# arneschneuing/DiffSBDD

Measured on AMD Instinct MI355X. Metric: sampled ligands/sec (500-step DDPM, fullatom_cond) at 1/2/4/8 MI355X, higher is better.
Workload: dtype f32

## Files before the change

diffsbdd_amd/_lib.py:

```python
from __future__ import annotations

import ctypes as C
import os

_HERE = os.path.dirname(os.path.abspath(__file__))
LIB_PATH = os.environ.get("DSBDD_LIB") or os.path.join(_HERE, "libdiffsbdd_hip.so")
ABI_VERSION = 6

OK, ERR_ARG, ERR_STATE, ERR_CAPACITY, ERR_LAUNCH = 0, -1, -2, -3, -4
STATUS_NAN, STATUS_EDGE_OVERFLOW = 1, 2

G_NAMES = ["ATOM_ENC_W0T", "ATOM_ENC_B0", "ATOM_ENC_W1T", "ATOM_ENC_B1",
           "RES_ENC_W0T", "RES_ENC_B0", "RES_ENC_W1T", "RES_ENC_B1",
           "ATOM_DEC_W0T", "ATOM_DEC_B0", "ATOM_DEC_W1T", "ATOM_DEC_B1",
           "RES_DEC_W0T", "RES_DEC_B0", "RES_DEC_W1T", "RES_DEC_B1",
           "EMB_WT", "EMB_B", "EMBOUT_WT", "EMBOUT_B"]
GCL_NAMES = ["E1_WT", "E1_WD", "E1_WD0", "E1_TAB", "E2_WT", "E2_B", "ATT_W", "ATT_B",
             "N1_WT", "N1_B", "N2_WT", "N2_B"]
EQ_NAMES = ["C1_WT", "C_WD", "C_WD0", "C_TAB", "C_W2T", "C_B2",
            "X_WD", "X_WD0", "X_TAB", "X_W2T", "X_B2", "W3"]
OPT_PRUNE, OPT_CONE, OPT_GRANULE16, OPT_EMU, OPT_SPLITK = 0, 1, 2, 3, 4
(BUF_EDGE_ROW, BUF_EDGE_COL, BUF_EDGE_D0, BUF_ROW_PTR, BUF_H, BUF_X, BUF_NODE_BATCH, BUF_DEG,
 BUF_LEVEL, BUF_LEVEL_LIST, BUF_LEVEL_COUNT, BUF_LEVEL_END, BUF_LROW_PTR, BUF_LEDGE_ROW, BUF_LEDGE_COL,
 BUF_LEDGE_D0, BUF_LEVEL_STATS) = range(17)


class Config(C.Structure):
    _fields_ = [(n, C.c_int32) for n in (
        "atom_nf", "residue_nf", "joint_nf", "hidden_nf", "n_layers", "inv_sublayers",
        "attention", "use_tanh", "update_pocket_coords", "reflection_equivariant",
        "edge_embedding_dim", "has_cutoff_ligand", "has_cutoff_pocket",
        "has_cutoff_interaction")] + [(n, C.c_float) for n in (
            "cutoff_ligand", "cutoff_pocket", "cutoff_interaction",
            "norm_constant", "normalization_factor", "coords_range")]


class TrainGraph(C.Structure):
    _fields_ = [(n, C.c_void_p) for n in ("erow", "ecol", "ed0", "row_ptr", "deg", "rev", "node_batch", "lig_off",
                                          "poc_off")] + [(n, C.c_int64) for n in ("n_lig", "n_nodes", "n_edges", "batch")]


class LossCfg(C.Structure):
    _fields_ = [(n, C.c_int32) for n in ("batch", "n_lig", "n_pocket", "atom_nf", "residue_nf", "timesteps", "remove_com",
                                         "vnode_idx")] + \
               [(n, C.c_float) for n in ("norm_value_x", "norm_value_h", "norm_bias_h")] + \
               [(n, C.c_int32) for n in ("n1_tab", "n2_tab")]


class TrainMlp(C.Structure):
    _fields_ = [("P", C.c_void_p), ("Q", C.c_void_p), ("ldpq", C.c_int32)] + \
               [(n, C.c_void_p) for n in ("wd", "wd0", "tab", "W2", "W2T", "b2", "head", "head_b")]


class TrainMlpGrad(C.Structure):
    _fields_ = [("dP", C.c_void_p), ("dQ", C.c_void_p), ("ldo", C.c_int32), ("d_vec", C.c_void_p), ("d_W2", C.c_void_p),
                ("gd0", C.c_void_p)]


class OptimCfg(C.Structure):
    _fields_ = [(n, C.c_double) for n in ("lr", "beta1", "beta2", "eps", "weight_decay")] + [("clip_grad", C.c_int32)]


_P = C.c_void_p
_I64 = C.c_int64
_I32 = C.c_int32
_F = C.c_float

SIGNATURES = {
    "dsbdd_abi_version": (C.c_int, []),
    "dsbdd_last_error": (C.c_char_p, []),
    "dsbdd_engine_create": (C.c_int, [C.POINTER(Config), C.POINTER(_P)]),
    "dsbdd_engine_destroy": (None, [_P]),
    "dsbdd_engine_weight_slots": (C.c_int, [_P]),
    "dsbdd_engine_set_weights": (C.c_int, [_P, C.POINTER(_P), C.c_int]),
    "dsbdd_engine_workspace_bytes": (C.c_size_t, [_P, _I64, _I64, _I64, _I64]),
    "dsbdd_engine_bind_workspace": (C.c_int, [_P, _P, C.c_size_t, _I64, _I64, _I64, _I64]),
    "dsbdd_engine_set_trace": (C.c_int, [_P, _P, _P]),
    "dsbdd_engine_set_pocket_frame": (C.c_int, [_P, _P, _P, _P, _P, _P, _I64, _I64, _I64, _I64, _I64, _I64]),
    "dsbdd_engine_clear_pocket_frame": (C.c_int, [_P]),
    "dsbdd_dynamics_forward": (C.c_int, [_P, _P, _P, _P, _P, _I64, _P, _P, _I64, _I64, _I64,
                                         _P, _P, _I64, _P, _P, _P]),
    "dsbdd_engine_buffer": (C.c_int, [_P, C.c_int, C.POINTER(_P)]),
    "dsbdd_engine_graph_stats": (C.c_int, [_P, C.POINTER(_I64), C.POINTER(_I64), C.POINTER(_I64)]),
    "dsbdd_engine_last_plan": (C.c_int, [_P, C.POINTER(C.c_int32), C.POINTER(C.c_int32), C.c_int32,
                                         C.POINTER(C.c_int32), C.POINTER(C.c_int32)]),
    "dsbdd_engine_set_option": (C.c_int, [_P, C.c_int, C.c_int]),
    "dsbdd_engine_get_option": (C.c_int, [_P, C.c_int]),
    "dsbdd_engine_profile": (C.c_int, [_P, C.c_int, C.c_int]),
    "dsbdd_engine_profile_read": (C.c_int, [_P, C.POINTER(C.c_double), C.POINTER(_I64)]),
    "dsbdd_cond_reverse_update": (C.c_int, [_P, _P, _P, _P, _P, _P, _P, _I64, _I64, _I64,
                                            _I32, _I32, _F, _F, _F, _I32]),
    "dsbdd_joint_reverse_update": (C.c_int, [_P, _P, _P, _P, _P, _P, _P, _P, _P, _I64, _I64, _I64,
                                             _I32, _I32, _F, _F, _F, _I32]),
    "dsbdd_segment_mean3": (C.c_int, [_P, _P, _I32, _P, _I64, _I64, _P]),
    "dsbdd_cond_affine_noise": (C.c_int, [_P, _P, _P, _P, _P, _P, _I64, _I64, _I64, _I32, _I32, _F, _F, _I32]),
    "dsbdd_joint_affine_noise": (C.c_int, [_P, _P, _P, _P, _P, _P, _P, _I64, _I64, _I64, _I32, _I32, _F, _F,
                                           _I32, _I32]),
    "dsbdd_cond_repaint_update": (C.c_int, [_P, _P, _P, _P, _P, _P, _P, _P, _P, _P, _P, _I64, _I64, _I64,
                                            _I32, _I32, _F, _F, _F, _F, _I32, _I32]),
    "dsbdd_joint_repaint_update": (C.c_int, [_P] * 15 + [_I64, _I64, _I64, _I32, _I32, _F, _F, _F, _F, _I32]),
    "dsbdd_cond_step_keyed": (C.c_int, [_P] * 10 + [_I64, _I64, _I64, _I32, _I32, _F, _F, _F, _I32, _F, _F, _F, _I32,
                                        C.c_uint64, C.c_uint64, _I64, _P, _P, _F]),
    "dsbdd_randn_keyed": (C.c_int, [_P, _P, _P, _I64, _I32, _I64, _I64, _P, C.c_uint64, C.c_uint64,
                                    C.c_uint32]),
    "dsbdd_node_linear": (C.c_int, [_P, _P, _I32, _I32, _P, _I32, _I32, _P, _I32, _P, _P, _I32,
                                    _P, _I32, _I64, _I32, _I32]),
    "dsbdd_build_edges": (C.c_int, [_P, _P, _P, _P, _I64, _I64, _I64, C.POINTER(Config),
                                    _P, _P, _P, _P, _P, _P, _P, _P, _I64, _P]),
    "dsbdd_bond_orders": (C.c_int, [_P, _P, _P, _P, _I64, _I32, _P, _P, _P, C.c_float, C.c_float,
                                    C.c_float, _I32, _P]),
    "dsbdd_pack_ligands": (C.c_int, [_P, _P, _P, _P, _I32, _I64, _P, _P, _P, _I64, _I64, _I32, _P, _P, _P, _P, _P]),
    "dsbdd_train_scratch_bytes": (C.c_size_t, [_I32, _I64, _I64]),
    "dsbdd_train_wgrad_scratch_bytes": (C.c_size_t, [_I64, _I64, _I64]),
    "dsbdd_train_wgrad_plan_bytes": (C.c_size_t, [_I64, _I64, _I64]),
    "dsbdd_train_edge_rev": (C.c_int, [_P, _P, _P]),
    "dsbdd_train_sample_mean": (C.c_int, [_P, _P, _P, _P]),
    "dsbdd_train_gcl_forward": (C.c_int, [_P, _I32, _P, _P, _P, _F, _P, _P, C.c_size_t]),
    "dsbdd_train_gcl_backward": (C.c_int, [_P, _I32, _P, _P, _P, _F, _P, _P, _P, _P, C.c_size_t]),
    "dsbdd_train_coord_forward": (C.c_int, [_P, _I32, _P, _P, _I32, _P, _P, _I64, _F, _F, _I32, _F, _P, _P,
                                            C.c_size_t]),
    "dsbdd_train_coord_backward": (C.c_int, [_P, _I32, _P, _P, _I32, _P, _P, _I64, _I64, _F, _F, _I32, _F, _P, _P, _P,
                                             _P, _P, C.c_size_t]),
    "dsbdd_train_radial_backward": (C.c_int, [_P, _P, _P, _P, _P]),
    "dsbdd_train_wgrad": (C.c_int, [_P, _P, _I32, _P, _I32, _I64, _I32, _I32, _P, _P, C.c_size_t]),
    "dsbdd_train_colsum": (C.c_int, [_P, _P, _I32, _I64, _I32, _P, _P, C.c_size_t]),
    "dsbdd_train_net_create": (C.c_int, [C.POINTER(Config), C.POINTER(_P)]),
    "dsbdd_train_net_destroy": (None, [_P]),
    "dsbdd_train_net_param_count": (C.c_int, [_P]),
    "dsbdd_train_net_pack_bytes": (C.c_size_t, [_P]),
    "dsbdd_train_net_workspace_bytes": (C.c_size_t, [_P, C.POINTER(TrainGraph)]),
    "dsbdd_train_net_forward": (C.c_int, [_P, _P, C.POINTER(TrainGraph), C.POINTER(_P), _P, C.c_size_t, _P, C.c_size_t, _P, _P,
                                          _P, _I64, _I32, _P, _P, _P]),
    "dsbdd_train_net_backward": (C.c_int, [_P, _P, C.POINTER(TrainGraph), C.POINTER(_P), C.POINTER(_P), _P, C.c_size_t, _P,
                                           C.c_size_t, _I64, _P, _P, _P, _P]),
    "dsbdd_train_net_forward_held": (C.c_int, [_P, _P, C.POINTER(TrainGraph), C.POINTER(_P), _P, C.c_size_t, _P, C.c_size_t,
                                               _P, _P, _P, _I64, _I32, _P, _P, _P, _I32]),
    "dsbdd_train_net_backward_acc": (C.c_int, [_P, _P, C.POINTER(TrainGraph), C.POINTER(_P), C.POINTER(_P), _P, _P, C.c_size_t,
                                               _P, C.c_size_t, _I64, _P, _P, _P, _P]),
    "dsbdd_edge_capacity": (C.c_int, [_P, _P, _I64, _P, _I64, _I64, _P]),
    "dsbdd_loss_rows": (C.c_int, []),
    "dsbdd_loss_out_rows": (C.c_int, []),
    "dsbdd_loss_cond_pre": (C.c_int, [_P, C.POINTER(LossCfg)] + [_P] * 17),
    "dsbdd_loss_cond_post": (C.c_int, [_P, C.POINTER(LossCfg)] + [_P] * 8),
    "dsbdd_loss_cond_post_backward": (C.c_int, [_P, C.POINTER(LossCfg)] + [_P] * 9),
    "dsbdd_loss_joint_out_rows": (C.c_int, []),
    "dsbdd_loss_joint_pre": (C.c_int, [_P, C.POINTER(LossCfg)] + [_P] * 20),
    "dsbdd_loss_joint_post": (C.c_int, [_P, C.POINTER(LossCfg)] + [_P] * 10),
    "dsbdd_loss_joint_post_backward": (C.c_int, [_P, C.POINTER(LossCfg)] + [_P] * 14),
    "dsbdd_optim_create": (C.c_int, [C.POINTER(OptimCfg), _I32, C.POINTER(_I64), C.POINTER(_P)]),
    "dsbdd_optim_destroy": (None, [_P]),
    "dsbdd_optim_state_elems": (_I64, [_P]),
    "dsbdd_optim_state_offset": (_I64, [_P, _I32]),
    "dsbdd_optim_workspace_bytes": (C.c_size_t, [_P]),
    "dsbdd_optim_bind": (C.c_int, [_P, _P, _P, _P, _P, _P, C.c_size_t]),
    "dsbdd_optim_set_params": (C.c_int, [_P, _P, C.POINTER(_P)]),
    "dsbdd_optim_step": (C.c_int, [_P, _P, C.POINTER(_P), C.POINTER(_I32), C.c_double]),
    "dsbdd_optim_state_read": (C.c_int, [_P, _P, C.POINTER(C.c_double), _I32]),
    "dsbdd_optim_state_write": (C.c_int, [_P, _P, C.POINTER(C.c_double), _I32, C.c_double, C.c_double]),
    "dsbdd_lj_potential": (C.c_int, [_P, _P, _I32, _I32, _P, _I64, _I64, _P, C.c_double, _I32, _P, _P, _P]),
}

_lib = None


class HipLibraryError(RuntimeError):
    pass


def load():
    global _lib
    if _lib is not None:
        return _lib
    import torch
    if not os.path.isfile(LIB_PATH):
        raise HipLibraryError(
            f"{LIB_PATH} not found: the HIP extension is not built. Run "
            "`python -c 'import __graft_entry__ as g; g.build()'` (needs hipcc). "
            "There is no CPU fallback for the product path.")
    try:
        lib = C.CDLL(LIB_PATH)
    except OSError as exc:
        raise HipLibraryError(f"cannot load {LIB_PATH}: {exc}") from exc
    for name, (res, args) in SIGNATURES.items():
        try:
            fn = getattr(lib, name)
        except AttributeError as exc:
            raise HipLibraryError(f"{LIB_PATH} does not export {name}") from exc
        fn.restype = res
        fn.argtypes = args
    ver = lib.dsbdd_abi_version()
    if ver != ABI_VERSION:
        raise HipLibraryError(f"ABI version mismatch: library {ver}, binding {ABI_VERSION}")
    _lib = lib
    return lib


def check(rc, what=""):
    if rc == OK:
        return
    msg = load().dsbdd_last_error()
    msg = msg.decode() if msg else ""
    raise HipLibraryError(f"{what} failed with code {rc}: {msg}")
```

diffsbdd_amd/csrc/edge_mlp.h:

```cpp
#pragma once
#include "common.h"

namespace dsbdd {

struct EdgeMlpW {
  const float* P;
  const float* Q;
  const float* wd;
  const float* wd0;
  const float* table;
  const float* W2T;
  const float* b2;
  const float* W2TP;
  const float* W2TP16;
  const void* W2E;
  const float* W2SK;
};

struct EdgeArgs {
  const int* erow; const int* ecol; const float* ed0;
  const int* e_count;
  int e_cap;
  const float* x;
  int n_lig;
  int n_nodes;
  int ldpq;
  EdgeMlpW mlp[2];
  const float* att_w; const float* att_b; int attention;
  float* agg;
  float* agg_head;
  const float* w3; const int* node_batch; const float* mean;
  float norm_constant; float coords_range; int use_tanh; int n_mlp;
  float* xagg;
  float* xagg_head;
  size_t xagg_stride;
  size_t xhead_stride;
  float norm_factor;
  int wt_base;
  int* tile_ctr;
  unsigned long long* ts;
  int pass_split;
  const int* erow_b; const int* ecol_b; const float* ed0_b; const int* e_count_b; int e_cap_b; int wt_base_b;
  float* agg_b; float* agg_head_b;
  float* z2_out;
  size_t z2_stride;
};

enum { MODE_GCL = 0, MODE_COORD = 1 };

__global__ __launch_bounds__(kThreads) void agg_complete_kernel(float* agg, const float* agg_head,
                                                                const int* row_ptr, const int* deg,
                                                                int n_rows, int H, int max_tile, int shift) {
  const int row = (blockIdx.x * kThreads + threadIdx.x) >> 6, lane = threadIdx.x & 63;
  if (row >= n_rows) return;
  const int d = deg[row], s = row_ptr[row];
  const int t0 = s >> shift, t1 = min((s + d - 1) >> shift, max_tile);
  if (d > 0 && t1 == t0) return;
  for (int k = 4 * lane; k < H; k += 256) {
    float4 v = make_float4(0.f, 0.f, 0.f, 0.f);
    if (d > 0) {
      v = ld4(agg + (size_t)row * H + k);
      for (int T = t0 + 1; T <= t1; ++T) {
        const float4 h = ld4(agg_head + (size_t)T * H + k);
        v.x += h.x; v.y += h.y; v.z += h.z; v.w += h.w;
      }
    }
    *reinterpret_cast<float4*>(agg + (size_t)row * H + k) = v;
  }
}


__global__ __launch_bounds__(kThreads) void agg_complete2_kernel(
    float* agg, const float* head_a, const int* row_ptr_a, const int* deg_a, const float* agg_b,
    const float* head_b, const int* row_ptr_b, const int* deg_b, const int* twin_local, int twin_base,
    int n_lig, int n_rows, int H, int n_ghost, int max_tile) {
  const int row = (blockIdx.x * kThreads + threadIdx.x) >> 6, lane = threadIdx.x & 63;
  if (row >= n_rows + n_ghost) return;
  const bool ghost = row >= n_rows;
  const int da = ghost ? 0 : deg_a[row], sa = ghost ? 0 : row_ptr_a[row];
  const int a0 = sa >> 5, a1 = min((sa + da - 1) >> 5, max_tile);
  int db = 0, sb = 0, tw = 0;
  if (row >= n_lig) {
    const int tl = ghost ? row - n_rows : twin_local[row - n_lig];
    db = deg_b[tl]; sb = row_ptr_b[tl]; tw = twin_base + tl;
  }
  const int b0 = sb >> 5, b1 = min((sb + db - 1) >> 5, max_tile);
  for (int k = 4 * lane; k < H; k += 256) {
    float4 v = make_float4(0.f, 0.f, 0.f, 0.f);
    if (da > 0) {
      v = ld4(agg + (size_t)row * H + k);
      for (int T = a0 + 1; T <= a1; ++T) {
        const float4 h = ld4(head_a + (size_t)T * H + k);
        v.x += h.x; v.y += h.y; v.z += h.z; v.w += h.w;
      }
    }
    if (db > 0) {
      float4 u = ld4(agg_b + (size_t)tw * H + k);
      for (int T = b0 + 1; T <= b1; ++T) {
        const float4 h = ld4(head_b + (size_t)T * H + k);
        u.x += h.x; u.y += h.y; u.z += h.z; u.w += h.w;
      }
      v.x += u.x; v.y += u.y; v.z += u.z; v.w += u.w;
    }
    *reinterpret_cast<float4*>(agg + (size_t)row * H + k) = v;
  }
}

}
```

diffsbdd_amd/csrc/edge_wave.h:

```cpp
#pragma once
#include "common.h"
#include "edge_mlp.h"
#include "graph.h"

namespace dsbdd {

template <int H, int MODE, int EMU = 0>
struct WaveLayout {
  static constexpr int BK = EMU ? 16 : 32;
  static constexpr int B_BUF = EMU ? 24 * H : BK * H;
  static constexpr int NV = (MODE == MODE_GCL) ? 1 : 2;
  static constexpr int VEC_PER = 7 * H;
  static constexpr int VEC_OFF = 0;
  static constexpr int SCR_OFF = VEC_OFF + NV * VEC_PER;
  static constexpr int SCR_PER = 32 * 3;
  static constexpr int B_OFF = (SCR_OFF + 4 * SCR_PER + 4 + 255) / 256 * 256;
  static constexpr int TOTAL = B_OFF + 2 * B_BUF;
};

__device__ __forceinline__ void wave_lds_fence() {
  __builtin_amdgcn_fence(__ATOMIC_RELEASE, "wavefront");
  __builtin_amdgcn_s_waitcnt(0xc07f);
  __builtin_amdgcn_wave_barrier();
  __builtin_amdgcn_fence(__ATOMIC_ACQUIRE, "wavefront");
}


__device__ __forceinline__ float dpp_xor1(float v) {
  return __int_as_float(__builtin_amdgcn_update_dpp(0, __float_as_int(v), 0xB1, 0xF, 0xF, true));
}
__device__ __forceinline__ float dpp_xor2(float v) {
  return __int_as_float(__builtin_amdgcn_update_dpp(0, __float_as_int(v), 0x4E, 0xF, 0xF, true));
}
__device__ __forceinline__ float dpp_half_mirror(float v) {
  return __int_as_float(__builtin_amdgcn_update_dpp(0, __float_as_int(v), 0x141, 0xF, 0xF, true));
}
__device__ __forceinline__ float dpp_ror8(float v) {
  return __int_as_float(__builtin_amdgcn_update_dpp(0, __float_as_int(v), 0x128, 0xF, 0xF, true));
}
__device__ __forceinline__ float pair_sum_rows16(float p, float q) {
  const auto r = __builtin_amdgcn_permlane16_swap(__float_as_uint(p), __float_as_uint(q), false, false);
  return __uint_as_float(r[0]) + __uint_as_float(r[1]);
}
__device__ __forceinline__ float pair_sum_halves(float p, float q) {
  const auto r = __builtin_amdgcn_permlane32_swap(__float_as_uint(p), __float_as_uint(q), false, false);
  return __uint_as_float(r[0]) + __uint_as_float(r[1]);
}

__device__ __forceinline__ float reduce16_half_wave(const float (&part)[16], int j) {
  float k8[8], k4[4], k2[2];
#pragma unroll
  for (int i = 0; i < 8; ++i) k8[i] = pair_sum_rows16(part[i], part[i + 8]);
  const bool b3 = (j >> 3) & 1, b2 = (j >> 2) & 1, b1 = (j >> 1) & 1;
#pragma unroll
  for (int i = 0; i < 4; ++i) {
    const float send = b3 ? k8[i] : k8[i + 4], keep = b3 ? k8[i + 4] : k8[i];
    k4[i] = keep + dpp_ror8(send);
  }
#pragma unroll
  for (int i = 0; i < 2; ++i) {
    const float send = b2 ? k4[i] : k4[i + 2], keep = b2 ? k4[i + 2] : k4[i];
    k2[i] = keep + dpp_half_mirror(send);
  }
  const float send = b1 ? k2[0] : k2[1], keep = b1 ? k2[1] : k2[0];
  const float k1 = keep + dpp_xor2(send);
  return k1 + dpp_xor1(k1);
}

typedef __bf16 bf16x8 __attribute__((ext_vector_type(8)));
typedef unsigned int u32x4 __attribute__((ext_vector_type(4)));

__device__ __forceinline__ float bf16_rne_f(float x) {
  unsigned u = __float_as_uint(x);
  u += 0x7FFFu + ((u >> 16) & 1u);
  return __uint_as_float(u & 0xFFFF0000u);
}

__global__ __launch_bounds__(256) void pack_w2e_kernel(const float* __restrict__ W2T, unsigned short* __restrict__ out, int H) {
  const int idx = blockIdx.x * 256 + threadIdx.x;
  if (idx >= H * H) return;
  const int CT = H / 32;
  const int i = idx & 7, l = (idx >> 3) & 63, c = (idx >> 9) % CT, ks = (idx >> 9) / CT;
  const int k = 16 * ks + 8 * (l >> 5) + i, col = 32 * c + (l & 31);
  const float w = W2T[(size_t)k * H + col];
  const float hi = bf16_rne_f(w), r1 = w - hi, mid = bf16_rne_f(r1), lo = bf16_rne_f(r1 - mid);
  const size_t base = (((size_t)(ks * CT + c) * 3) * 64 + l) * 8 + i;
  out[base] = (unsigned short)(__float_as_uint(hi) >> 16);
  out[base + 512] = (unsigned short)(__float_as_uint(mid) >> 16);
  out[base + 1024] = (unsigned short)(__float_as_uint(lo) >> 16);
}

template <int H, int MODE, bool BPERM, int EMU = 0, bool STORE = false>
__global__ __launch_bounds__(kThreads, 2) void edge_wave_kernel(EdgeArgs p) {
  using L = WaveLayout<H, MODE, EMU>;
  static_assert(!STORE || (!BPERM && EMU == 0), "z2 is stored by the plain exact kernels only");
  constexpr int BK = L::BK;
  constexpr int CT = H / 32;
  constexpr int NK = H / BK;
  constexpr int NQ = H / 4;
  constexpr int UNIT = EMU ? (((6 * H) % kThreads == 0) ? 4 : 2) : 4;
  constexpr int BI = EMU ? (24 * H) / (kThreads * UNIT) : BK * NQ / kThreads;
  constexpr int NG = EMU ? CT / 2 : BK / 8;
  constexpr int BMW = 32, BMB = 128;
  static_assert(H % 64 == 0 && H <= 256, "hidden_nf must be 64,128,192 or 256");
  static_assert(EMU || (BK * NQ) % kThreads == 0, "B slice split");
  static_assert(!EMU || (24 * H) % (kThreads * UNIT) == 0, "emulated B slice split");
  static_assert(EMU == 0 || EMU == 6 || EMU == 9, "partial products of the emulated path");
  static_assert(!EMU || !BPERM, "the emulated path has its own B layout");
  constexpr bool SETPRIO = true;
  static_assert(!BPERM || CT == 8 || CT == 4, "lane-grouped B reads need 4 or 8 column tiles");
  constexpr bool bperm = BPERM;

  __shared__ __attribute__((aligned(1024))) float smem[L::TOTAL];
  float* sB = smem + L::B_OFF;
  float* sV = smem + L::VEC_OFF;
  const int t = threadIdx.x, lane = t & 63;
  const int w = __builtin_amdgcn_readfirstlane(t >> 6);
  const int half = lane >> 5, j = lane & 31;
  float* s_phi = smem + L::SCR_OFF + w * L::SCR_PER;
  float* s_tr = s_phi;
  const bool split = MODE == MODE_COORD && p.pass_split && p.n_mlp == 2;
  const int qsel = split ? ((blockIdx.x >> 3) & 1) : 0;
  const int n_pass = (MODE == MODE_GCL || split) ? 1 : p.n_mlp;

  for (int q = 0; q < n_pass; ++q) {
    const EdgeMlpW& mw = p.mlp[qsel + q];
    float* v = sV + q * L::VEC_PER;
    for (int i = t; i < H; i += kThreads) {
      v[i] = mw.wd[i];
      v[H + i] = mw.wd0[i];
      v[2 * H + i] = mw.table[i];
      v[3 * H + i] = mw.table[H + i];
      v[4 * H + i] = mw.table[2 * H + i];
      v[5 * H + i] = mw.b2[i];
      v[6 * H + i] = (MODE == MODE_GCL) ? (p.attention ? p.att_w[i] : 0.f) : p.w3[i];
    }
  }
  const float att_b = (MODE == MODE_GCL && p.attention) ? p.att_b[0] : 0.f;
  const float inv_norm = 1.0f / p.norm_factor;

  const int swb = (bperm && CT == 8) ? ((j >> 3) & 1) : 0;
  auto feat = [&](int c) { return ((c ^ (4 * swb)) * 32) + j; };

  const int E = min(*p.e_count, p.e_cap);
  const int nt_a = (E + BMB - 1) / BMB;
  const int E_b = (MODE == MODE_GCL && p.e_count_b) ? min(*p.e_count_b, p.e_cap_b) : 0;
  const int ntiles = nt_a + (E_b + BMB - 1) / BMB;
  const int xcd = blockIdx.x & 7;
  const int kx = split ? (blockIdx.x >> 4) : (blockIdx.x >> 3);
  const int gx = split ? (gridDim.x >> 4) : (gridDim.x >> 3);
  const int tq = ntiles / 8, tr = ntiles % 8;
  const int csize = tq + (xcd < tr ? 1 : 0);
  const int cbase = (xcd < tr) ? xcd * (tq + 1) : tr * (tq + 1) + (xcd - tr) * tq;
  if (kx >= csize) return;


  constexpr int SG = EMU ? BI : (BI + 3) / 4;
  typedef float stg_t __attribute__((ext_vector_type(UNIT)));
  stg_t stg[SG];
  auto stage_lo = [](int g) { return BI * g / NG; };
  auto stage_load = [&](int q, int ks, int g) {
    const char* src = EMU ? reinterpret_cast<const char*>(p.mlp[qsel + q].W2E) + (size_t)ks * (96 * H)
                          : reinterpret_cast<const char*>((bperm ? p.mlp[qsel + q].W2TP : p.mlp[qsel + q].W2T) + (size_t)ks * BK * H);
    const unsigned toff = (unsigned)t * (4u * UNIT);
#pragma unroll
    for (int i = stage_lo(g); i < stage_lo(g + 1); ++i)
      stg[EMU ? i : i - stage_lo(g)] = *reinterpret_cast<const stg_t*>(src + (size_t)(kThreads * 4 * UNIT * i) + toff);
  };
  auto stage_store = [&](int buf, int g) {
    float* dst = sB + buf * L::B_BUF + t * UNIT;
#pragma unroll
    for (int i = stage_lo(g); i < stage_lo(g + 1); ++i)
      *reinterpret_cast<stg_t*>(dst + kThreads * UNIT * i) = stg[EMU ? i : i - stage_lo(g)];
  };

  int my_r = -1, my_c = 0, my_ty = 0;
  float my_d = 0.f, my_d0 = 0.f, xr[3] = {0.f, 0.f, 0.f}, xc[3] = {0.f, 0.f, 0.f};
  int nx_r = -1, nx_c = 0;
  int my_prev = -1, nx_prev = -1;
  int my_wt = 0, nx_wt = 0;
  bool my_lb = false, nx_lb = false;
  float nx_d0 = 0.f, nxr[3] = {0.f, 0.f, 0.f}, nxc[3] = {0.f, 0.f, 0.f};
  int vzero;
  asm volatile("v_mov_b32 %0, 0" : "=v"(vzero));
  auto fetch_idx = [&](int tile) {
    const bool lb = MODE == MODE_GCL && tile >= nt_a;
    const int tl = lb ? tile - nt_a : tile, El = lb ? E_b : E;
    const int* er = lb ? p.erow_b : p.erow;
    const int* ec = lb ? p.ecol_b : p.ecol;
    const float* ed = lb ? p.ed0_b : p.ed0;
    const int e0 = tl * BMB + w * BMW, e = e0 + j;
    nx_r = -1; nx_c = 0; nx_d0 = 0.f; nx_prev = -1; nx_wt = (lb ? p.wt_base_b : p.wt_base) + tl * 4 + w; nx_lb = lb;
    if (e < El) { nx_r = er[e]; nx_c = ec[e]; nx_d0 = ed[e]; }
    if (e0 > 0 && e0 < El) nx_prev = er[e0 - 1 + vzero];
  };
  auto fetch_x = [&]() {
    if ((unsigned)nx_r >= (unsigned)p.n_nodes || (unsigned)nx_c >= (unsigned)p.n_nodes) { nx_r = -1; nx_c = 0; }
    if (nx_r >= 0) {
#pragma unroll
      for (int k = 0; k < 3; ++k) { nxr[k] = p.x[3 * nx_r + k]; nxc[k] = p.x[3 * nx_c + k]; }
    }
  };
  auto commit_edge = [&]() {
    my_r = nx_r; my_c = nx_c; my_d0 = nx_d0; my_d = 0.f; my_ty = 0;
    my_prev = nx_prev; my_wt = nx_wt; my_lb = nx_lb;
#pragma unroll
    for (int k = 0; k < 3; ++k) { xr[k] = nxr[k]; xc[k] = nxc[k]; }
    if (my_r >= 0) {
      const float dx = xr[0] - xc[0], dy = xr[1] - xc[1], dz = xr[2] - xc[2];
      my_d = dx * dx + dy * dy + dz * dz;
      const bool rl = my_r < p.n_lig, cl = my_c < p.n_lig;
      my_ty = (rl && cl) ? 1 : ((!rl && !cl) ? 2 : 0);
    }
  };

  auto read_b = [&](const float* brow, float (&bv)[CT]) {
    if constexpr (BPERM) {
      const float4 lo = *reinterpret_cast<const float4*>(brow);
      bv[0] = lo.x; bv[1] = lo.y; bv[2] = lo.z; bv[3] = lo.w;
      if constexpr (CT == 8) {
        const float4 hi = *reinterpret_cast<const float4*>(brow + 4 - 8 * swb);
        bv[4] = hi.x; bv[5] = hi.y; bv[6] = hi.z; bv[7] = hi.w;
      }
    } else {
#pragma unroll
      for (int c = 0; c < CT; ++c) bv[c] = brow[c * 32];
    }
  };

#pragma unroll
  for (int g = 0; g < NG; ++g) { stage_load(0, 0, g); stage_store(0, g); }
  fetch_idx(cbase + kx);
  fetch_x();
  commit_edge();
  __syncthreads();
  int bslice = 0;

  constexpr int KH = EMU ? 8 : 4;
  const float* Pp = p.mlp[qsel].P + (size_t)(my_r < 0 ? 0 : my_r) * p.ldpq + KH * half;
  const float* Qp = p.mlp[qsel].Q + (size_t)my_c * p.ldpq + KH * half;
  f32x4 pc = ldv4(Pp), qc = ldv4(Qp), pn = pc, qn4 = qc;
  f32x4 pc1 = pc, qc1 = qc;
  if constexpr (EMU != 0) { pc1 = ldv4(Pp + 4); qc1 = ldv4(Qp + 4); }
  float phi0 = 0.f, phi1 = 0.f;

  bf16x8 a_h = {}, a_m = {}, a_l = {};
  (void)a_h; (void)a_m; (void)a_l;
  int li = kx, q = 0, next_li = 0;
  bool has_next = false;
#pragma unroll 1
  for (;;) {
    const float* vq = sV + q * L::VEC_PER;
    const bool tile_ends = q == n_pass - 1;
    const int qn = tile_ends ? 0 : q + 1;

    f32x16 acc[CT];
#pragma unroll
    for (int c = 0; c < CT; ++c) {
      const float bv = vq[5 * H + feat(c)];
#pragma unroll
      for (int r = 0; r < 16; ++r) acc[c][r] = bv;
    }

#pragma unroll 1
    for (int kt = 0; kt < NK; ++kt) {
      const bool more = kt + 1 < NK;
      const int st = q * NK + kt;
      if (st == 0) {
        next_li = li + gx;
        has_next = next_li < csize;
        if (has_next) fetch_idx(cbase + next_li);
      }
      if (st == 1 && has_next) fetch_x();
      const int sq = more ? q : qn, sks = more ? kt + 1 : 0;
      const f32x2 dd = splat2(my_d), dz = splat2(my_d0);
      if constexpr (EMU != 0) {
        constexpr int NG1 = (NG + 1) / 2;
        auto act8 = [&](int ks, bf16x8& o_h, bf16x8& o_m, bf16x8& o_l) {
          const float* vk = vq + ks * 16 + 8 * half;
          const float* vt = vk + (2 + my_ty) * H;
          float av[8];
#pragma unroll
          for (int hh = 0; hh < 2; ++hh) {
            const f32x4 pp = hh ? pc1 : pc, qq = hh ? qc1 : qc;
            const f32x4 wd4 = *reinterpret_cast<const f32x4*>(vk + 4 * hh);
            const f32x4 wz4 = *reinterpret_cast<const f32x4*>(vk + H + 4 * hh);
            const f32x4 tb4 = *reinterpret_cast<const f32x4*>(vt + 4 * hh);
            f32x2 alo = pk_fma(dz, wz4.xy, pk_fma(dd, wd4.xy, pp.xy + qq.xy)) + tb4.xy;
            f32x2 ahi = pk_fma(dz, wz4.zw, pk_fma(dd, wd4.zw, pp.zw + qq.zw)) + tb4.zw;
            alo = silu2(alo);
            ahi = silu2(ahi);
            av[4 * hh] = alo.x; av[4 * hh + 1] = alo.y; av[4 * hh + 2] = ahi.x; av[4 * hh + 3] = ahi.y;
          }
#pragma unroll
          for (int i = 0; i < 8; ++i) {
            const __bf16 h1 = (__bf16)av[i];
            const float r1 = av[i] - (float)h1;
            const __bf16 m1 = (__bf16)r1;
            const float r2 = r1 - (float)m1;
            o_h[i] = h1; o_m[i] = m1; o_l[i] = (__bf16)r2;
          }
        };
        auto load_pq = [&](int ks) {
          pc = ldv4(Pp + 16 * ks); pc1 = ldv4(Pp + 16 * ks + 4);
          qc = ldv4(Qp + 16 * ks); qc1 = ldv4(Qp + 16 * ks + 4);
        };
        act8(kt, a_h, a_m, a_l);
        load_pq(more ? kt + 1 : 0);
#pragma unroll
        for (int g = 0; g < NG1; ++g) stage_load(sq, sks, g);
        const float* bl = sB + (bslice & 1) * L::B_BUF + lane * 4;
        bf16x8 bh[2], bm[2], blo[2];
        auto rdb = [&](int cp, int plane, bf16x8 (&dst)[2]) {
#pragma unroll
          for (int u = 0; u < 2; ++u)
            dst[u] = __builtin_bit_cast(bf16x8, *reinterpret_cast<const u32x4*>(bl + (2 * cp + u) * 768 + plane * 256));
        };
        rdb(0, 2, blo); rdb(0, 1, bm); rdb(0, 0, bh);
#define EMU_MM(a, b) do { _Pragma("unroll") for (int u = 0; u < 2; ++u) \
          acc[2 * cp + u] = __builtin_amdgcn_mfma_f32_32x32x16_bf16(a, b[u], acc[2 * cp + u], 0, 0, 0); } while (0)
        __builtin_amdgcn_s_setprio(1);
#pragma unroll
        for (int cp = 0; cp < CT / 2; ++cp) {
          const bool nxt = cp + 1 < CT / 2;
          if constexpr (EMU == 9) { EMU_MM(a_l, blo); EMU_MM(a_m, blo); }
          EMU_MM(a_h, blo);
          if (nxt) rdb(cp + 1, 2, blo);
          if constexpr (EMU == 9) EMU_MM(a_l, bm);
          EMU_MM(a_m, bm); EMU_MM(a_h, bm);
          if (nxt) rdb(cp + 1, 1, bm);
          EMU_MM(a_l, bh); EMU_MM(a_m, bh); EMU_MM(a_h, bh);
          if (nxt) rdb(cp + 1, 0, bh);
          if (NG > 1 && cp == CT / 4 - 1) {
#pragma unroll
            for (int g = 0; g < NG1; ++g) stage_store((bslice + 1) & 1, g);
#pragma unroll
            for (int g = NG1; g < NG; ++g) stage_load(sq, sks, g);
          }
        }
#undef EMU_MM
        __builtin_amdgcn_s_setprio(0);
#pragma unroll
        for (int g = (NG > 1 ? NG1 : 0); g < NG; ++g) stage_store((bslice + 1) & 1, g);
      } else {
      const float* bcur = sB + (bslice & 1) * L::B_BUF + (4 * half) * H + (bperm ? j * CT + 4 * swb : j);
      const float* vk = vq + kt * BK + 4 * half;
      const float* vt = vk + (2 + my_ty) * H;
#pragma unroll
      for (int g = 0; g < BK / 8; ++g) {
        const int kb = kt * BK + 8 * g;
        if (g > 0) stage_store((bslice + 1) & 1, g - 1);
        stage_load(sq, sks, g);
        if (g + 1 < BK / 8 || more) {
          pn = ldv4(Pp + kb + 8);
          qn4 = ldv4(Qp + kb + 8);
        }
        const f32x4 wd4 = *reinterpret_cast<const f32x4*>(vk + 8 * g);
        const f32x4 wz4 = *reinterpret_cast<const f32x4*>(vk + H + 8 * g);
        const f32x4 tb4 = *reinterpret_cast<const f32x4*>(vt + 8 * g);
        f32x2 alo = pk_fma(dz, wz4.xy, pk_fma(dd, wd4.xy, pc.xy + qc.xy)) + tb4.xy;
        f32x2 ahi = pk_fma(dz, wz4.zw, pk_fma(dd, wd4.zw, pc.zw + qc.zw)) + tb4.zw;
        alo = silu2(alo);
        ahi = silu2(ahi);
        const float a[4] = {alo.x, alo.y, ahi.x, ahi.y};
        if (SETPRIO) __builtin_amdgcn_s_setprio(1);
#pragma unroll
        for (int i = 0; i < 4; ++i) {
          const float* brow = bcur + (8 * g + i) * H;
          float bv[CT];
          read_b(brow, bv);
#pragma unroll
          for (int c = 0; c < CT; ++c) acc[c] = mfma32(a[i], bv[c], acc[c]);
        }
        if (SETPRIO) __builtin_amdgcn_s_setprio(0);
        pc = pn; qc = qn4;
      }
      stage_store((bslice + 1) & 1, BK / 8 - 1);
      }
      ++bslice;
      __syncthreads();
    }

    const bool last_unit = tile_ends && !has_next;
    if (!last_unit) {
      const int r_n = tile_ends ? nx_r : my_r, c_n = tile_ends ? nx_c : my_c;
      Pp = p.mlp[qsel + qn].P + (size_t)(r_n < 0 ? 0 : r_n) * p.ldpq + KH * half;
      Qp = p.mlp[qsel + qn].Q + (size_t)c_n * p.ldpq + KH * half;
      pc = ldv4(Pp); qc = ldv4(Qp);
      if constexpr (EMU != 0) { pc1 = ldv4(Pp + 4); qc1 = ldv4(Qp + 4); }
    }

    if constexpr (STORE) {
      const int e0 = (my_wt - p.wt_base) * BMW;
      float* zb = p.z2_out + (MODE == MODE_COORD ? (size_t)(qsel + q) * p.z2_stride : (size_t)0) + (size_t)e0 * H + j;
#pragma unroll
      for (int r = 0; r < 16; ++r) {
        const int row = 8 * (r >> 2) + 4 * half + (r & 3);
        if (e0 + row < E) {
#pragma unroll
          for (int c = 0; c < CT; ++c) zb[(size_t)row * H + 32 * c] = acc[c][r];
        }
      }
    }
    if (MODE == MODE_GCL) {
#pragma unroll
      for (int c = 0; c < CT; ++c)
#pragma unroll
        for (int r = 0; r < 16; r += 2) {
          const f32x2 m2 = silu2(f32x2{acc[c][r], acc[c][r + 1]});
          acc[c][r] = m2.x; acc[c][r + 1] = m2.y;
        }
      if (p.attention) {
        f32x2 part2[8];
#pragma unroll
        for (int r = 0; r < 8; ++r) part2[r] = splat2(0.f);
#pragma unroll
        for (int c = 0; c < CT; ++c) {
          const f32x2 aw = splat2(vq[6 * H + feat(c)]);
#pragma unroll
          for (int r = 0; r < 8; ++r) part2[r] = pk_fma(f32x2{acc[c][2 * r], acc[c][2 * r + 1]}, aw, part2[r]);
        }
        float part[16];
#pragma unroll
        for (int r = 0; r < 8; ++r) { part[2 * r] = part2[r].x; part[2 * r + 1] = part2[r].y; }
        const float gate = sigmoidf_fast(reduce16_half_wave(part, j) + att_b);
        s_phi[16 * half + (j >> 1)] = gate;
        wave_lds_fence();
#pragma unroll
        for (int q4 = 0; q4 < 4; ++q4) {
          const float4 g4 = *reinterpret_cast<const float4*>(s_phi + 16 * half + 4 * q4);
          part[4 * q4] = g4.x; part[4 * q4 + 1] = g4.y; part[4 * q4 + 2] = g4.z; part[4 * q4 + 3] = g4.w;
        }
        wave_lds_fence();
#pragma unroll
        for (int c = 0; c < CT; ++c)
#pragma unroll
          for (int r = 0; r < 16; ++r) acc[c][r] *= part[r];
      }
      static_assert(CT % 2 == 0, "column tiles are exchanged in pairs");
      f32x2 sum2[CT];
#pragma unroll
      for (int c = 0; c < CT; ++c) sum2[c] = splat2(0.f);
      int cur = -1;
      const int row0 = __builtin_amdgcn_readlane(my_r, 0);
      bool to_head = row0 >= 0 && row0 == __builtin_amdgcn_readfirstlane(my_prev);
      auto flush = [&]() {
        if (cur >= 0) {
          float* dst = to_head ? (my_lb ? p.agg_head_b : p.agg_head) + (size_t)my_wt * H
                               : (my_lb ? p.agg_b : p.agg) + (size_t)cur * H;
#pragma unroll
          for (int c = 0; c < CT / 2; ++c) {
            const float tot = pair_sum_halves(sum2[c].x + sum2[c].y, sum2[c + CT / 2].x + sum2[c + CT / 2].y);
            dst[feat(c + half * (CT / 2))] = tot * inv_norm;
          }
          to_head = false;
        }
#pragma unroll
        for (int c = 0; c < CT; ++c) sum2[c] = splat2(0.f);
      };
#pragma unroll
      for (int gb = 0; gb < 8; ++gb) {
        const int hh = gb & 1;
#pragma unroll
        for (int ip = 0; ip < 4; ip += 2) {
          const int k = 4 * (gb >> 1) + ip;
          const int rn0 = __builtin_amdgcn_readlane(my_r, 4 * gb + ip);
          const int rn1 = __builtin_amdgcn_readlane(my_r, 4 * gb + ip + 1);
          if (rn0 != cur) {
            flush();
            cur = rn0;
          }
          if (half == hh) {
#pragma unroll
            for (int c = 0; c < CT; ++c) sum2[c].x += acc[c][k];
          }
          if (rn1 != rn0) {
            flush();
            cur = rn1;
          }
          if (half == hh) {
#pragma unroll
            for (int c = 0; c < CT; ++c) sum2[c].y += acc[c][k + 1];
          }
        }
      }
      flush();
    } else {
      f32x2 part2[8];
#pragma unroll
      for (int r = 0; r < 8; ++r) part2[r] = splat2(0.f);
#pragma unroll
      for (int c = 0; c < CT; ++c) {
        const f32x2 wv = splat2(vq[6 * H + feat(c)]);
#pragma unroll
        for (int r = 0; r < 8; ++r) part2[r] = pk_fma(silu2(f32x2{acc[c][2 * r], acc[c][2 * r + 1]}), wv, part2[r]);
      }
      float part[16];
#pragma unroll
      for (int r = 0; r < 8; ++r) { part[2 * r] = part2[r].x; part[2 * r + 1] = part2[r].y; }
      s_phi[mfma_row(j >> 1, lane)] = reduce16_half_wave(part, j);
      wave_lds_fence();
      const float ph = s_phi[j];
      wave_lds_fence();
      if (qsel + q == 0) phi0 = ph; else phi1 = ph;

      if (tile_ends) {
        float tx = 0.f, ty = 0.f, tz = 0.f;
        if (my_r >= 0) {
          const float dx = xr[0] - xc[0], dy = xr[1] - xc[1], dz = xr[2] - xc[2];
          const float den = sqrtf(my_d + 1e-8f) + p.norm_constant;
          const float ux = dx / den, uy = dy / den, uz = dz / den;
          if (split && qsel == 1) {
          } else if (p.use_tanh) {
            const float th = tanhf(phi0);
            tx = ux * th * p.coords_range; ty = uy * th * p.coords_range; tz = uz * th * p.coords_range;
          } else {
            tx = ux * phi0; ty = uy * phi0; tz = uz * phi0;
          }
          if (p.n_mlp == 2 && !(split && qsel == 0)) {
            const int b = p.node_batch[my_r];
            const float m0 = p.mean[3 * b], m1 = p.mean[3 * b + 1], m2 = p.mean[3 * b + 2];
            const float a0 = xr[0] - m0, a1 = xr[1] - m1, a2 = xr[2] - m2;
            const float b0 = xc[0] - m0, b1 = xc[1] - m1, b2 = xc[2] - m2;
            const float c0 = a1 * b2 - a2 * b1, c1 = a2 * b0 - a0 * b2, c2 = a0 * b1 - a1 * b0;
            const float cden = sqrtf(c0 * c0 + c1 * c1 + c2 * c2) + p.norm_constant;
            float phx = phi1;
            if (p.use_tanh) phx = tanhf(phx) * p.coords_range;
            tx += c0 / cden * phx; ty += c1 / cden * phx; tz += c2 / cden * phx;
          }
        }
        if (half == 0) { s_tr[3 * j] = tx; s_tr[3 * j + 1] = ty; s_tr[3 * j + 2] = tz; }
        wave_lds_fence();
        float trv[32];
#pragma unroll
        for (int e = 0; e < 32; ++e) trv[e] = s_tr[3 * e + (lane < 3 ? lane : 0)];
        if (lane < 3) {
          const int pop = split ? qsel : 0;
          float* xa = p.xagg + pop * p.xagg_stride;
          float* xh = p.xagg_head + pop * p.xhead_stride;
          const int row0 = __builtin_amdgcn_readlane(my_r, 0);
          bool to_head = row0 >= 0 && row0 == __builtin_amdgcn_readfirstlane(my_prev);
          int cur = -1;
          float sum = 0.f;
          auto put = [&]() {
            if (cur >= 0) {
              const float v = sum / p.norm_factor;
              if (to_head) xh[4 * (size_t)my_wt + lane] = v; else xa[(size_t)cur * 3 + lane] = v;
              to_head = false;
            }
          };
#pragma unroll
          for (int e = 0; e < 32; ++e) {
            const int rn = __builtin_amdgcn_readlane(my_r, e);
            if (rn != cur) {
              put();
              cur = rn;
              sum = 0.f;
            }
            sum += trv[e];
          }
          put();
        }
        wave_lds_fence();
      }
    }

    if (tile_ends) {
      if (last_unit) break;
      commit_edge();
      li = next_li;
      q = 0;
    } else {
      ++q;
    }
  }
}

}
```

diffsbdd_amd/csrc/engine.hip:

```cpp
#include "../../include/diffsbdd_hip.h"

#include <algorithm>
#include <climits>
#include <cmath>
#include <cstdio>
#include <cstdlib>
#include <cstring>
#include <string>
#include <type_traits>
#include <utility>
#include <vector>

#include "common.h"
#include "ddpm.h"
#include "edge_mlp.h"
#include "edge_wave.h"
#include "edge_wave16.h"
#include "edge_splitk.h"
#include "graph.h"
#include "lig_head.h"
#include "ligand_pack.h"
#include "molecule.h"
#include "node_chain.h"
#include "node_linear.h"
#include "train.h"
#include "train_kernels.h"

using namespace dsbdd;

#include "engine_state.h"
#include "launch.h"
#include "forward.h"
#include "graph_cache.h"
#include "capi_kernels.h"
#include "train_blocks.h"
#include "train_net.h"
#include "loss_head.h"
#include "optim.h"
#include "lj_loss.h"
#include "train_api.h"

extern "C" {

int dsbdd_abi_version(void) { return DSBDD_ABI_VERSION; }
const char* dsbdd_last_error(void) { return g_err.c_str(); }

int dsbdd_engine_create(const dsbdd_config* cfg, dsbdd_engine** out) {
  if (!cfg || !out) return fail(DSBDD_ERR_ARG, "null argument");
  if (!hidden_nf_ok(cfg->hidden_nf)) return fail(DSBDD_ERR_ARG, "hidden_nf must be one of 64, 128, 192, 256");
  if (cfg->n_layers < 1 || cfg->inv_sublayers < 1 || cfg->atom_nf < 1 || cfg->residue_nf < 1 ||
      cfg->joint_nf < 1 || cfg->edge_embedding_dim < 0)
    return fail(DSBDD_ERR_ARG, "bad layer/feature counts");
  if (!(cfg->normalization_factor > 0.f)) return fail(DSBDD_ERR_ARG, "normalization_factor must be > 0");
  dsbdd_engine* e = new dsbdd_engine();
  e->cfg = *cfg;
  e->slots.assign(n_slots(*cfg), nullptr);
  e->n_cu = device_cus();
  read_env_switches(e);
  *out = e;
  return DSBDD_OK;
}

void dsbdd_engine_destroy(dsbdd_engine* e) { delete e; }

int dsbdd_engine_weight_slots(const dsbdd_engine* e) { return e ? n_slots(e->cfg) : DSBDD_ERR_ARG; }

int dsbdd_engine_set_weights(dsbdd_engine* e, const float* const* slots_host, int n) {
  if (!e || !slots_host) return fail(DSBDD_ERR_ARG, "null argument");
  if (n != n_slots(e->cfg)) return fail(DSBDD_ERR_ARG, "wrong number of weight slots");
  const dsbdd_config& c = e->cfg;
  for (int i = 0; i < n; ++i) {
    const float* ptr = slots_host[i];
    bool optional = false;
    const int per = c.inv_sublayers * DSBDD_GCL_COUNT + DSBDD_EQ_COUNT;
    if (i >= DSBDD_G_COUNT) {
      const int r = (i - DSBDD_G_COUNT) % per;
      if (r < c.inv_sublayers * DSBDD_GCL_COUNT) {
        const int wch = r % DSBDD_GCL_COUNT;
        if (!c.attention && (wch == DSBDD_GCL_ATT_W || wch == DSBDD_GCL_ATT_B)) optional = true;
      } else {
        const int wch = r - c.inv_sublayers * DSBDD_GCL_COUNT;
        if (c.reflection_equivariant && wch >= DSBDD_EQ_X_WD && wch <= DSBDD_EQ_X_B2) optional = true;
      }
    }
    if (!ptr && !optional) return fail(DSBDD_ERR_ARG, "null weight slot " + std::to_string(i));
    if (ptr && (reinterpret_cast<uintptr_t>(ptr) & 15))
      return fail(DSBDD_ERR_ARG, "weight slot " + std::to_string(i) + " not 16-byte aligned");
    e->slots[i] = ptr;
  }
  e->drop_graphs();
  e->invalidate_derived();
  e->h0_pocket_valid = false;
  e->has_weights = true;
  return DSBDD_OK;
}

size_t dsbdd_engine_workspace_bytes(const dsbdd_engine* e, int64_t nl, int64_t np, int64_t B,
                                    int64_t E) {
  if (!e || nl < 0 || np < 0 || B < 1 || E < 0) return 0;
  return ws_carve(e->cfg, nl, np, B, E, nullptr).total;
}

int dsbdd_engine_bind_workspace(dsbdd_engine* e, void* ws, size_t bytes, int64_t nl, int64_t np,
                                int64_t B, int64_t E) {
  if (!e || !ws) return fail(DSBDD_ERR_ARG, "null argument");
  if (reinterpret_cast<uintptr_t>(ws) & 255) return fail(DSBDD_ERR_ARG, "workspace must be 256-byte aligned");
  if ((nl + np) >= (1ll << 30) || E >= (1ll << 31) - 256) return fail(DSBDD_ERR_ARG, "problem too large for int32 indices");
  if (bytes < ws_carve(e->cfg, nl, np, B, E, nullptr).total) return fail(DSBDD_ERR_CAPACITY, "workspace too small");
  e->drop_graphs();
  static_cast<Workspace&>(*e) = ws_carve(e->cfg, nl, np, B, E, static_cast<char*>(ws));
  e->ws = static_cast<char*>(ws); e->ws_bytes = bytes;
  e->cap_lig = nl; e->cap_poc = np; e->cap_batch = B; e->cap_edges = E;
  e->cap_edgesL = 2 * E + 32 * kLevels * B;
  e->cap_tiles = e->cap_edgesL / 32 + 2;
  e->cap_tiles16 = e->cap_edgesL / 16 + 2;
  e->lvl_stats_zeroed = false;
  e->frame = false;
  e->ghost_dirty = true;
  e->h0_pocket_valid = false;
  e->invalidate_derived();
  return DSBDD_OK;
}

#ifdef DSBDD_TIMESTAMPS
int dsbdd_debug_set_timestamps(dsbdd_engine* e, unsigned long long* buf, int capacity) {
  if (!e) return DSBDD_ERR_ARG;
  e->ts_buf = buf; e->ts_cap = capacity; e->ts_next = 0;
  return DSBDD_OK;
}
#endif

int dsbdd_engine_set_pocket_frame(dsbdd_engine* e, void* stream, const float* x_frame, const int64_t* mask_frame,
                                  const int32_t* frame_rows, const int32_t* twin_local, int64_t n_lig,
                                  int64_t n_pocket, int64_t batch, int64_t n_frame, int64_t batch_frame,
                                  int64_t edge_bound_frame) {
  StreamDevice stream_device_(stream);
  if (!e || !x_frame || !mask_frame || !frame_rows || !twin_local) return fail(DSBDD_ERR_ARG, "null argument");
  if (!e->ws) return fail(DSBDD_ERR_STATE, "workspace not bound");
  if (e->cfg.update_pocket_coords) return fail(DSBDD_ERR_STATE, "a pocket frame needs rigid pocket coordinates");
  if (n_lig < 0 || n_lig > e->cap_lig || n_pocket < 1 || n_pocket > e->cap_poc || batch < 1 || batch > e->cap_batch ||
      n_frame < 1 || n_frame > n_pocket || batch_frame < 1 || batch_frame > batch || edge_bound_frame < 1 ||
      edge_bound_frame > e->cap_edges)
    return fail(DSBDD_ERR_CAPACITY, "pocket frame exceeds the bound workspace");
  hipStream_t s = static_cast<hipStream_t>(stream);
  e->drop_graphs();
  e->frame = false;
  e->h0_pocket_valid = false;
  const int n3 = (int)n_frame, b3 = (int)batch_frame, N = (int)(n_lig + n_pocket);
  HIP_TRY(hipMemcpyAsync(e->xframe, x_frame, (size_t)n3 * 12, hipMemcpyDeviceToDevice, s));
  HIP_TRY(hipMemcpyAsync(e->frame_rows, frame_rows, (size_t)n3 * 4, hipMemcpyDeviceToDevice, s));
  HIP_TRY(hipMemcpyAsync(e->twin, twin_local, (size_t)n_pocket * 4, hipMemcpyDeviceToDevice, s));
  const int work = n3 > b3 + 1 ? n3 : b3 + 1;
  hipLaunchKernelGGL(prep_kernel, dim3((work + 255) / 256), dim3(256), 0, s, (const int64_t*)nullptr, 0, mask_frame,
                     n3, b3, e->node_batch3, e->lig_off3, e->poc_off3, (int*)nullptr);
  HIP_TRY(hipGetLastError());
  int rc = build_edges_impl(s, x_frame, 0, n3, b3, e->cfg, e->node_batch3, e->lig_off3, e->poc_off3, e->deg3,
                            e->row_ptr3, e->erow3, e->ecol3, e->ed03, e->cap_edges, e->tile_ctr + 24, nullptr,
                            e->scan_tmp3, e->seg_base3, nullptr, N);
  if (rc) return rc;
  e->frame_nlig = n_lig; e->frame_npoc = n_pocket; e->frame_batch = batch;
  e->frame_n3 = n3; e->frame_cap3 = edge_bound_frame;
  rc = ghost_setup(e, s);
  if (rc) return rc;
  int slots = 0;
  HIP_TRY(hipMemcpyAsync(&slots, e->row_ptr3 + n3, 4, hipMemcpyDeviceToHost, s));
  HIP_TRY(hipStreamSynchronize(s));
  if (slots < 0 || slots > e->cap_edges || (slots & (kEdgeAlign - 1)))
    return fail(DSBDD_ERR_CAPACITY, "pocket frame: pocket-pocket list exceeds the edge capacity");
  e->ghost_slots = slots;
  e->frame = true;
  return DSBDD_OK;
}

int dsbdd_engine_clear_pocket_frame(dsbdd_engine* e) {
  if (!e) return fail(DSBDD_ERR_ARG, "null argument");
  if (e->frame) e->drop_graphs();
  e->frame = false;
  e->h0_pocket_valid = false;
  return DSBDD_OK;
}

int dsbdd_engine_last_plan(const dsbdd_engine* e, int32_t* radius, int32_t* ghost, int32_t capacity,
                           int32_t* n_stages, int32_t* timed_level) {
  if (!e || !radius || !ghost || !n_stages || !timed_level) return fail(DSBDD_ERR_ARG, "null argument");
  const int n = (int)e->plan_radius.size();
  if (capacity < n) return fail(DSBDD_ERR_CAPACITY, "plan arrays too short");
  for (int i = 0; i < n; ++i) { radius[i] = e->plan_radius[i]; ghost[i] = e->plan_ghost[i]; }
  *n_stages = n; *timed_level = e->plan_timed_level;
  return DSBDD_OK;
}

int dsbdd_engine_set_option(dsbdd_engine* e, int which, int value) {
  if (!e) return fail(DSBDD_ERR_ARG, "null argument");
  switch (which) {
    case DSBDD_OPT_PRUNE: e->prune = value ? 1 : 0; break;
    case DSBDD_OPT_CONE: e->cone = value <= 0 ? 0 : (value >= 2 ? 2 : 1); break;
    case DSBDD_OPT_GRANULE16: e->granule16 = (unsigned)value; break;
    case DSBDD_OPT_SPLITK: e->splitk = (unsigned)value; break;
    case DSBDD_OPT_EMU:
      if (value != 0 && value != 6 && value != 9) return fail(DSBDD_ERR_ARG, "DSBDD_OPT_EMU takes 0, 6 or 9");
      e->emu = value; break;
    default: return fail(DSBDD_ERR_ARG, "unknown option");
  }
  e->drop_graphs();
  return DSBDD_OK;
}

int dsbdd_engine_get_option(const dsbdd_engine* e, int which) {
  if (!e) return fail(DSBDD_ERR_ARG, "null argument");
  switch (which) {
    case DSBDD_OPT_PRUNE: return e->prune;
    case DSBDD_OPT_CONE: return e->cone;
    case DSBDD_OPT_GRANULE16: return (int)e->granule16;
    case DSBDD_OPT_SPLITK: return (int)e->splitk;
    case DSBDD_OPT_EMU: return e->emu;
  }
  return fail(DSBDD_ERR_ARG, "unknown option");
}

int dsbdd_engine_set_trace(dsbdd_engine* e, float* th, float* tx) {
  if (!e) return DSBDD_ERR_ARG;
  e->trace_h = th; e->trace_x = tx;
  return DSBDD_OK;
}

int dsbdd_engine_profile(dsbdd_engine* e, int enable, int max_launches) {
  if (!e || max_launches < 0) return fail(DSBDD_ERR_ARG, "bad argument");
  e->profile = enable < 0 ? 0 : enable;
  e->prof_call = 0;
  e->ev_used = 0;
  while (e->profile && e->ev.size() < (size_t)2 * max_launches) {
    hipEvent_t a;
    HIP_TRY(hipEventCreate(&a));
    e->ev.push_back(a);
  }
  return DSBDD_OK;
}

int dsbdd_engine_profile_read(dsbdd_engine* e, double* total_ms, int64_t* launches) {
  if (!e || !total_ms || !launches) return fail(DSBDD_ERR_ARG, "null argument");
  double tot = 0.0;
  for (size_t i = 0; i + 1 < e->ev_used; i += 2) {
    HIP_TRY(hipEventSynchronize(e->ev[i + 1]));
    float ms = 0.f;
    HIP_TRY(hipEventElapsedTime(&ms, e->ev[i], e->ev[i + 1]));
    tot += ms;
  }
  *total_ms = tot;
  *launches = (int64_t)(e->ev_used / 2);
  e->ev_used = 0;
  return DSBDD_OK;
}

int dsbdd_engine_graph_stats(const dsbdd_engine* e, int64_t* replays, int64_t* captures, int64_t* eager) {
  if (!e || !replays || !captures || !eager) return fail(DSBDD_ERR_ARG, "null argument");
  *replays = e->n_replay; *captures = e->n_capture; *eager = e->n_eager;
  return DSBDD_OK;
}

int dsbdd_engine_buffer(const dsbdd_engine* e, int which, void** out) {
  if (!e || !out || !e->ws) return fail(DSBDD_ERR_STATE, "no workspace bound");
  void* const buf[] = {e->erow, e->ecol, e->ed0, e->row_ptr, e->h, e->x, e->node_batch, e->deg, e->lvl, e->lvl_list, e->lvl_cnt,
                       e->lvl_end, e->row_ptrL, e->erowL, e->ecolL, e->ed0L, e->lvl_stats};
  static_assert(DSBDD_BUF_LEVEL_STATS + 1 == sizeof(buf) / sizeof(buf[0]), "one pointer per DSBDD_BUF_* id");
  if (which < 0 || which > DSBDD_BUF_LEVEL_STATS) return fail(DSBDD_ERR_ARG, "unknown buffer id");
  *out = buf[which];
  return DSBDD_OK;
}


int dsbdd_dynamics_forward(dsbdd_engine* e, void* stream, const float* xh_lig, const float* xh_pocket,
                           const float* t, int64_t t_count, const int64_t* mask_lig,
                           const int64_t* mask_pocket, int64_t n_lig, int64_t n_pocket, int64_t batch,
                           const int32_t* ext_row, const int32_t* ext_col, int64_t ext_n_edges,
                           float* eps_lig, float* eps_pocket, int32_t* status) {
  StreamDevice stream_device_(stream);
  if (!e || !xh_lig || !xh_pocket || !t || !mask_lig || !mask_pocket || !eps_lig || !status)
    return fail(DSBDD_ERR_ARG, "null argument");
  if (!e->has_weights) return fail(DSBDD_ERR_STATE, "weights not set");
  if (!e->ws) return fail(DSBDD_ERR_STATE, "workspace not bound");
  if (n_lig > e->cap_lig || n_pocket > e->cap_poc || batch > e->cap_batch || n_lig < 0 || n_pocket < 0 ||
      batch < 1)
    return fail(DSBDD_ERR_CAPACITY, "sizes exceed the bound workspace");
  if (t_count != 1 && t_count != batch) return fail(DSBDD_ERR_ARG, "t must have 1 or batch entries");
  if (ext_row && (!ext_col || ext_n_edges < 0 || ext_n_edges > e->cap_edges))
    return fail(DSBDD_ERR_CAPACITY, "external edge list exceeds edge capacity");
  hipStream_t s = static_cast<hipStream_t>(stream);
  const ForwardArgs args{xh_lig, xh_pocket, t, t_count, mask_lig, mask_pocket, n_lig, n_pocket, batch,
                         ext_row, ext_col, ext_n_edges, eps_lig, eps_pocket, status};
  const int rc = frame_upkeep(e, s, args);
  if (rc) return rc;
  e->time_now = e->profile > 0 && (e->prof_call++ % e->profile) == 0;
  if (!e->use_graph || e->time_now || e->trace_h || e->trace_x || ext_row) {
    ++e->n_eager;
    return forward_impl(e, s, args);
  }
  return forward_cached(e, s, args);
}

}
```

diffsbdd_amd/csrc/engine_state.h:

```cpp
#pragma once

static thread_local std::string g_err;
static int fail(int code, const std::string& msg) { g_err = msg; return code; }

#define HIP_TRY(expr)                                                              \
  do {                                                                             \
    hipError_t _e = (expr);                                                        \
    if (_e != hipSuccess)                                                          \
      return fail(DSBDD_ERR_LAUNCH, std::string(#expr) + ": " + hipGetErrorString(_e)); \
  } while (0)
#define RC_TRY(expr)                       \
  do {                                     \
    const int _rc = (expr);                \
    if (_rc != DSBDD_OK) return _rc;       \
  } while (0)

struct StreamDevice {
  int prev = -1;
  bool switched = false;
  explicit StreamDevice(void* stream) {
    hipStream_t s = static_cast<hipStream_t>(stream);
    if (!s) return;
    hipDevice_t d = 0;
    int cur = 0;
    if (hipStreamGetDevice(s, &d) != hipSuccess || hipGetDevice(&cur) != hipSuccess) { (void)hipGetLastError(); return; }
    if ((int)d != cur) { prev = cur; switched = hipSetDevice((int)d) == hipSuccess; }
  }
  ~StreamDevice() { if (switched) (void)hipSetDevice(prev); }
  StreamDevice(const StreamDevice&) = delete;
  StreamDevice& operator=(const StreamDevice&) = delete;
};

static inline int pad4(int v) { return (v + 3) & ~3; }
static inline size_t al256(size_t v) { return (v + 255) & ~(size_t)255; }
struct Carver {
  char* base;
  size_t off = 0;
  char* bytes(size_t n) { char* q = base ? base + off : nullptr; off += al256(n); return q; }
  float* f(size_t floats) { return reinterpret_cast<float*>(bytes(floats * 4)); }
  float* f1(size_t floats) { return f(floats > 0 ? floats : 1); }
};

template <class F>
static hipError_t with_hidden(int H, F&& f) {
  switch (H) {
    case 64: return f(std::integral_constant<int, 64>{});
    case 128: return f(std::integral_constant<int, 128>{});
    case 192: return f(std::integral_constant<int, 192>{});
    case 256: return f(std::integral_constant<int, 256>{});
  }
  return hipErrorInvalidValue;
}
static bool hidden_nf_ok(int H) { return with_hidden(H, [](auto) { return hipSuccess; }) == hipSuccess; }

enum { W2_PERM, W2_PERM16, W2_EMU, W2_SPLITK, W2_KINDS };
struct W2Kind {
  size_t bytes;
  void (*pack)(hipStream_t s, const float* src, void* dst, int H);
};
template <class T, void (*K)(const float*, T*, int)>
static void w2_pack(hipStream_t s, const float* src, void* dst, int H) {
  hipLaunchKernelGGL(K, dim3((H * H + 255) / 256), dim3(256), 0, s, src, static_cast<T*>(dst), H);
}
static const W2Kind kW2Kinds[W2_KINDS] = {
    {4, w2_pack<float, permute_w2t_kernel>},
    {4, w2_pack<float, pack16_w2t_kernel>},
    {6, w2_pack<unsigned short, pack_w2e_kernel>},
    {4, w2_pack<float, pack_w2sk_kernel>}};
static size_t w2_bytes_before(int kind) {
  size_t b = 0;
  for (int k = 0; k < kind; ++k) b += kW2Kinds[k].bytes;
  return b;
}
struct DerivedReady { bool w2[W2_KINDS] = {}, chain = false; };

struct Workspace {
  int *node_batch, *lig_off, *poc_off, *deg, *row_ptr, *erow, *ecol;
  int *act_flag, *act_ptr, *act_list;
  float *ed0, *x, *x_in, *xagg, *mean, *h0, *enc_tmp, *h, *t1, *agg, *pq, *pqg, *hout;
  char* w2copies;
  float *agg_head, *xagg_head;
  int *scan_tmp, *seg_base, *tile_ctr;
  int *erow2, *ecol2, *row_ptr2, *deg2, *scan_tmp2, *seg_base2;
  int *erow3, *ecol3, *row_ptr3, *deg3, *scan_tmp3, *seg_base3, *node_batch3, *lig_off3, *poc_off3, *twin;
  float *ed02, *ed03, *xframe, *aggB, *agg_headB;
  int* frame_rows;
  int *lvl, *seg_rows, *seg_edges, *node_base, *edge_base, *lvl_cnt, *lvl_end, *lvl_list, *row_ptrL, *erowL, *ecolL;
  float* ed0L;
  unsigned long long* lvl_stats;
  float* wchain;
  size_t total;
};

static Workspace ws_carve(const dsbdd_config& c, int64_t nl, int64_t np, int64_t B, int64_t E, char* base) {
  const size_t N = (size_t)(nl + np), nB = (size_t)B, nE = (size_t)E;
  const size_t H = c.hidden_nf, JP = pad4(c.joint_nf + 1);
  const size_t LE = pad4(2 * (c.atom_nf > c.residue_nf ? c.atom_nf : c.residue_nf));
  const size_t PQ = (c.reflection_equivariant ? 2 : 4) * H;
  const size_t EL = 2 * nE + 32 * kLevels * nB;
  const size_t NG = N + (size_t)np;
  const size_t T = EL / 32 + 2;
  const size_t LB = kLevels * nB;
  const size_t n_w2 = (size_t)c.n_layers * (c.inv_sublayers + 2);
  Workspace w{};
  size_t off = 0;
  auto take = [&](auto*& p, size_t count) {
    using T_ = std::remove_reference_t<decltype(*p)>;
    p = base ? reinterpret_cast<T_*>(base + off) : nullptr;
    off += al256(count * sizeof(T_) + 16);
  };
  take(w.node_batch, N); take(w.lig_off, nB + 1); take(w.poc_off, nB + 1);
  take(w.deg, NG); take(w.row_ptr, N + 1);
  take(w.erow, nE); take(w.ecol, nE); take(w.ed0, nE);
  take(w.x, NG * 3); take(w.x_in, N * 3); take(w.xagg, N * 6); take(w.mean, nB * 3);
  take(w.h0, N * JP); take(w.enc_tmp, N * LE);
  take(w.h, NG * H); take(w.t1, NG * H); take(w.agg, NG * H); take(w.pq, N * PQ); take(w.hout, N * JP);
  take(w.act_flag, N); take(w.act_ptr, N + 1); take(w.act_list, N);
  take(w.pqg, NG * 2 * H);
  take(w.w2copies, n_w2 * H * H * w2_bytes_before(W2_KINDS) + 4096);
  take(w.agg_head, 2 * T * H); take(w.xagg_head, 2 * T * 2 * 4);
  take(w.scan_tmp, N + 1); take(w.seg_base, 2 * nB + 1); take(w.tile_ctr, (size_t)kTileCtrInts);
  take(w.erow2, nE); take(w.ecol2, nE); take(w.ed02, nE); take(w.row_ptr2, N + 1); take(w.deg2, N);
  take(w.scan_tmp2, N + 1); take(w.seg_base2, 2 * nB + 1);
  take(w.erow3, nE); take(w.ecol3, nE); take(w.ed03, nE); take(w.row_ptr3, N + 1); take(w.deg3, N);
  take(w.scan_tmp3, N + 1); take(w.seg_base3, 2 * nB + 1);
  take(w.node_batch3, N); take(w.lig_off3, nB + 1); take(w.poc_off3, nB + 1); take(w.twin, N);
  take(w.xframe, N * 3); take(w.aggB, NG * H); take(w.agg_headB, T * H);
  take(w.lvl, N); take(w.seg_rows, LB); take(w.seg_edges, LB);
  take(w.node_base, LB + 1); take(w.edge_base, LB + 1); take(w.lvl_cnt, 16); take(w.lvl_end, 16);
  take(w.lvl_list, NG); take(w.row_ptrL, NG + 1); take(w.erowL, EL); take(w.ecolL, EL); take(w.ed0L, EL);
  take(w.lvl_stats, 16); take(w.frame_rows, N);
  take(w.wchain, (size_t)c.n_layers * ((size_t)c.inv_sublayers * 5 * H * H + H * PQ) + 1024);
  w.total = off;
  return w;
}

struct dsbdd_engine : Workspace {
  dsbdd_config cfg;
  std::vector<const float*> slots;
  bool has_weights = false;
  char* ws = nullptr;
  size_t ws_bytes = 0;
  int64_t cap_lig = 0, cap_poc = 0, cap_batch = 0, cap_edges = 0;
  bool lvl_stats_zeroed = false;
  int64_t cap_edgesL = 0;
  int prune = 1;
  int cone = 1;
  int64_t ghost_slots = 0;
  std::vector<int> plan_radius, plan_ghost;
  int plan_timed_level = kLevels - 1;
  bool frame = false;
  int64_t frame_nlig = 0, frame_npoc = 0, frame_batch = 0, frame_n3 = 0, frame_cap3 = 0;
  bool ghost_dirty = true;
  bool h0_pocket_valid = false;
  int64_t cap_tiles = 0;
  int64_t cap_tiles16 = 0;
  unsigned granule16 = 0;
  unsigned splitk = 0;
  int emu = 0;
  DerivedReady derived;
  float *trace_h = nullptr, *trace_x = nullptr;
  int n_cu = 256;
  int chain = 1;
  int64_t chain_min_rows = 0;
  int fork_front = 0;
  hipStream_t side_stream = nullptr;
  hipEvent_t ev_fork = nullptr, ev_join = nullptr;
  int level_rows = 0;
  int fold_scan = 1;
  int lig_head = 1;
  int edge_bperm = 1;
  int profile = 0;
  int64_t prof_call = 0;
  bool time_now = false;
  std::vector<hipEvent_t> ev;
  size_t ev_used = 0;
  struct GraphEntry {
    std::vector<uint64_t> key;
    int seen = 0;
    hipGraph_t graph = nullptr;
    hipGraphExec_t exec = nullptr;
    std::vector<int> plan_radius, plan_ghost;
    int plan_timed_level = 0;
    void destroy() { if (exec) (void)hipGraphExecDestroy(exec); if (graph) (void)hipGraphDestroy(graph); }
  };
  std::vector<GraphEntry> graphs;
  int use_graph = 1;
  int coord_split = 1;
  int node_group = 1;
  int edge_max_wg = 0;
  int64_t n_replay = 0, n_capture = 0, n_eager = 0;
  unsigned long long* ts_buf = nullptr;
  int ts_cap = 0, ts_next = 0;
  hipStream_t cap_stream = nullptr;
  dsbdd_engine() : Workspace{} {}
  void drop_graphs() {
    for (GraphEntry& g : graphs) g.destroy();
    graphs.clear();
  }
  void invalidate_derived() { derived = DerivedReady{}; }
  ~dsbdd_engine() {
    for (hipEvent_t e : ev) (void)hipEventDestroy(e);
    drop_graphs();
    if (cap_stream) (void)hipStreamDestroy(cap_stream);
    if (side_stream) (void)hipStreamDestroy(side_stream);
    if (ev_fork) (void)hipEventDestroy(ev_fork);
    if (ev_join) (void)hipEventDestroy(ev_join);
  }
};

static int n_slots(const dsbdd_config& c) {
  return DSBDD_G_COUNT + c.n_layers * (c.inv_sublayers * DSBDD_GCL_COUNT + DSBDD_EQ_COUNT);
}
static int gcl_slot(const dsbdd_config& c, int block, int sub, int which) {
  return DSBDD_G_COUNT + block * (c.inv_sublayers * DSBDD_GCL_COUNT + DSBDD_EQ_COUNT) +
         sub * DSBDD_GCL_COUNT + which;
}
static int eq_slot(const dsbdd_config& c, int block, int which) {
  return DSBDD_G_COUNT + block * (c.inv_sublayers * DSBDD_GCL_COUNT + DSBDD_EQ_COUNT) +
         c.inv_sublayers * DSBDD_GCL_COUNT + which;
}

static bool w2_enabled(const dsbdd_engine* e, int kind) {
  const int H = e->cfg.hidden_nf;
  switch (kind) {
    case W2_PERM: return e->edge_bperm && (H == 256 || H == 128);
    case W2_PERM16: return e->granule16 != 0;
    case W2_EMU: return e->emu != 0;
    case W2_SPLITK: return e->splitk != 0 && H == 256 && !e->emu;
  }
  return false;
}
static void* w2_copy(const dsbdd_engine* e, int kind, int blk, int which) {
  if (!w2_enabled(e, kind)) return nullptr;
  const dsbdd_config& c = e->cfg;
  const size_t HH = (size_t)c.hidden_nf * c.hidden_nf, n_w2 = (size_t)c.n_layers * (c.inv_sublayers + 2);
  return e->w2copies + n_w2 * HH * w2_bytes_before(kind) + ((size_t)blk * (c.inv_sublayers + 2) + which) * HH * kW2Kinds[kind].bytes;
}
static int w2_pack_missing(dsbdd_engine* e, hipStream_t s) {
  const dsbdd_config& c = e->cfg;
  for (int kind = W2_KINDS - 1; kind >= 0; --kind) {
    if (!w2_enabled(e, kind) || e->derived.w2[kind]) continue;
    for (int blk = 0; blk < c.n_layers; ++blk)
      for (int which = 0; which < c.inv_sublayers + 2; ++which) {
        const float* src = which < c.inv_sublayers ? e->slots[gcl_slot(c, blk, which, DSBDD_GCL_E2_WT)]
                         : e->slots[eq_slot(c, blk, which == c.inv_sublayers ? DSBDD_EQ_C_W2T : DSBDD_EQ_X_W2T)];
        if (!src) continue;
        kW2Kinds[kind].pack(s, src, w2_copy(e, kind, blk, which), c.hidden_nf);
        HIP_TRY(hipGetLastError());
      }
    e->derived.w2[kind] = true;
  }
  return DSBDD_OK;
}

static bool env_int(const char* name, long long* v, bool mask = false) {
  const char* s = getenv(name);
  if (!s) return false;
  *v = mask ? (long long)strtoul(s, nullptr, 0) : (long long)atoi(s);
  return true;
}
static int env_int_in(const char* name, long long lo, long long hi, int dflt) {
  long long v;
  return env_int(name, &v) && v >= lo && v <= hi ? (int)v : dflt;
}
static void read_env_switches(dsbdd_engine* e) {
  long long v;
  const std::pair<const char*, int*> off_on_zero[] = {
      {"DSBDD_GRAPH", &e->use_graph}, {"DSBDD_EDGE_BPERM", &e->edge_bperm}, {"DSBDD_COORD_SPLIT", &e->coord_split},
      {"DSBDD_NODE_GROUP", &e->node_group}, {"DSBDD_PRUNE", &e->prune}, {"DSBDD_LIG_HEAD", &e->lig_head},
      {"DSBDD_NODE_CHAIN", &e->chain}};
  for (const auto& sw : off_on_zero) if (env_int(sw.first, &v) && v == 0) *sw.second = 0;
  const std::pair<const char*, int*> on_nonzero[] = {{"DSBDD_LEVEL_ROWS", &e->level_rows}, {"DSBDD_FORK", &e->fork_front}};
  for (const auto& sw : on_nonzero) if (env_int(sw.first, &v)) *sw.second = v != 0;
  if (env_int("DSBDD_FOLD_SCAN", &v)) e->fold_scan = v > 0 ? 1 : 0;
  if (env_int("DSBDD_GRANULE16", &v, true)) e->granule16 = (unsigned)v;
  if (env_int("DSBDD_SPLITK", &v, true)) e->splitk = (unsigned)v;
  if (env_int("DSBDD_EMU", &v)) e->emu = (v == 6 || v == 9) ? (int)v : 0;
  if (env_int("DSBDD_CONE", &v)) e->cone = v <= 0 ? 0 : (v >= 2 ? 2 : 1);
  if (env_int("DSBDD_NODE_CHAIN_MIN_ROWS", &v) && v >= 0) e->chain_min_rows = v;
  if (env_int("DSBDD_EDGE_MAX_WG", &v) && v > 0) e->edge_max_wg = (int)v;
}
```

diffsbdd_amd/csrc/forward.h:

```cpp
#pragma once

struct ForwardArgs {
  const float *xh_lig, *xh_pocket, *t;
  int64_t t_count;
  const int64_t *mask_lig, *mask_pocket;
  int64_t n_lig, n_pocket, batch;
  const int32_t *ext_row, *ext_col;
  int64_t ext_n_edges;
  float *eps_lig, *eps_pocket;
  int32_t* status;
};

static bool frame_applies(const dsbdd_engine* e, const ForwardArgs& a) {
  return e->frame && !e->cfg.update_pocket_coords && !a.ext_row && a.n_lig == e->frame_nlig &&
         a.n_pocket == e->frame_npoc && a.batch == e->frame_batch;
}

static Mlp2Problem residue_encoder(const dsbdd_engine* e, const ForwardArgs& a) {
  const dsbdd_config& c = e->cfg;
  const int r = c.residue_nf, J = c.joint_nf, JP = pad4(J + 1);
  const float* const* W = e->slots.data();
  return Mlp2Problem{a.xh_pocket + 3, 3 + r, r, W[DSBDD_G_RES_ENC_W0T], pad4(2 * r), W[DSBDD_G_RES_ENC_B0], 2 * r,
                     W[DSBDD_G_RES_ENC_W1T], pad4(J), W[DSBDD_G_RES_ENC_B1], J, e->h0 + (size_t)a.n_lig * JP, JP,
                     (int)a.n_pocket};
}

struct StageState {
  bool pqg_ready = false;
  bool chained_pq = false;
  bool chained_coord = false;
};

struct Forward : ForwardArgs {
  dsbdd_engine* const e;
  const hipStream_t s;
  const bool ext = ext_row != nullptr;
  const dsbdd_config& c = e->cfg;
  const int H = c.hidden_nf, J = c.joint_nf, JP = pad4(J + 1);
  const int a = c.atom_nf, r = c.residue_nf, dl = 3 + a, dp = 3 + r;
  const int LE = pad4(2 * (a > r ? a : r));
  const int nlig = (int)n_lig, N = (int)(n_lig + n_pocket), B = (int)batch;
  const int n_mlp = c.reflection_equivariant ? 1 : 2;
  const int PQ = (c.reflection_equivariant ? 2 : 4) * H;
  const float* const* W = e->slots.data();
  const bool subset = !c.update_pocket_coords;

  const bool split0 = frame_applies(e, *this);
  const bool prune = e->prune && subset && !ext && !eps_pocket && !e->trace_h && !e->trace_x && nlig > 0;
  const int G_stages = c.n_layers * c.inv_sublayers;
  const bool cone_pays = e->cone >= 2 || 5 * e->frame_n3 <= 2 * (int64_t)n_pocket;
  const bool cone = prune && split0 && e->cone && cone_pays && t_count == 1 && G_stages >= 2;
  const int n_frame_rows = split0 ? (int)e->frame_n3 : 0;
  const int n_ghost = (split0 && prune) ? n_frame_rows : 0;
  const int64_t ghost_slots = (split0 && prune) ? e->ghost_slots : 0;
  static constexpr int LV = kLevels - 1;
  const int g_ghost_last = ghost_last();
  const bool fork = e->fork_front && !ext;
  hipStream_t sa = s;
  int64_t edge_bound = e->cap_edges;
  bool mean_in_levels = false;
  const int* L_row = prune ? e->erowL : e->erow;
  const int* L_col = prune ? e->ecolL : e->ecol;
  const float* L_d0 = prune ? e->ed0L : e->ed0;
  const int* L_ptr = prune ? e->row_ptrL : e->row_ptr;
  const int L_cap = prune ? (int)e->cap_edgesL : (int)e->cap_edges;
  int64_t L_bound() const { return prune ? e->cap_edgesL : edge_bound; }
  const int* act_rows = prune ? e->lvl_list + n_ghost : e->act_list;
  const int* act_count = prune ? e->lvl_cnt + kLevels + 1 : e->act_ptr + N;
  const int n_upd = c.update_pocket_coords ? N : nlig;
  const int* e_all = prune ? e->lvl_end + kLevels + LV : e->row_ptr + N;
  const int* e_upd = prune ? e->lvl_end + kLevels : e->row_ptr + n_upd;
  const bool can_sk = w2_enabled(e, W2_SPLITK);
  const bool use_chain = e->chain && (H == 256 || H == 192 || H == 128) && N >= e->chain_min_rows;
  const size_t chain_blk = (size_t)c.inv_sublayers * 5 * H * H + (size_t)H * PQ;

  Forward(dsbdd_engine* e_, hipStream_t s_, const ForwardArgs& args) : ForwardArgs(args), e(e_), s(s_) {}

  int radius_of(int g) const {
    const int bw = G_stages - g, fw = g + 1;
    const int r = cone ? (bw < fw ? bw : fw) : bw;
    return r < LV ? r : LV;
  }
  int ghost_last() const {
    int last = -1;
    if (cone)
      for (int g = 0; g + 1 < G_stages; ++g) {
        const int rd = radius_of(g + 1) + 1 < LV ? radius_of(g + 1) + 1 : LV;
        if (rd > radius_of(g)) last = g;
      }
    return last;
  }
  void rows_of(int r, bool ghost, NodeLinearArgs& a) const {
    if (!prune || (r >= LV && !ghost && !e->level_rows)) return;
    if (r > LV) r = LV;
    a.row_idx = ghost ? e->lvl_list : e->lvl_list + n_ghost;
    a.m_count = ghost ? e->lvl_cnt + r : e->lvl_cnt + kLevels + r;
    a.M = N + n_ghost;
  }
  const float* chain_w(int blk, int sub, int which) const {
    const float* base = e->wchain + (size_t)blk * chain_blk;
    if (which == 3) return base + (size_t)c.inv_sublayers * 5 * H * H;
    return base + (size_t)sub * 5 * H * H + (which == 0 ? 0 : (which == 1 ? 2 * H * H : 3 * H * H));
  }
  NodeLinearArgs gcl_pq(int blk, int sub) const {
    NodeLinearArgs a{e->h, H, H, nullptr, 0, 0, W[gcl_slot(c, blk, sub, DSBDD_GCL_E1_WT)], 2 * H, nullptr,
                     nullptr, 0, e->pqg, 2 * H, (int)N, 2 * H, 0, nullptr, nullptr};
    const int g = blk * c.inv_sublayers + sub;
    rows_of(radius_of(g) + 1, g <= g_ghost_last && g > 0, a);
    return a;
  }
  EdgeMlpW edge_mlp(const float* P, const float* Q, const float* wd, const float* wd0, const float* tab, const float* W2T,
                    const float* b2, int blk, int which) const {
    return EdgeMlpW{P, Q, wd, wd0, tab, W2T, b2,
                    static_cast<const float*>(w2_copy(e, W2_PERM, blk, which)),
                    static_cast<const float*>(w2_copy(e, W2_PERM16, blk, which)), w2_copy(e, W2_EMU, blk, which),
                    static_cast<const float*>(w2_copy(e, W2_SPLITK, blk, which))};
  }

  void plan() {
    e->plan_radius.assign(G_stages, LV); e->plan_ghost.assign(G_stages, 0);
    e->plan_timed_level = LV;
    if (prune) {
      int rt = 0;
      for (int g = 0; g < G_stages; ++g) {
        e->plan_radius[g] = radius_of(g); e->plan_ghost[g] = g <= g_ghost_last;
        if (!(split0 && g == 0) && radius_of(g) > rt) rt = radius_of(g);
      }
      e->plan_timed_level = rt;
    }
  }

  int assemble_and_encode() {
    {
      int work = N > B + 1 ? N : B + 1;
      if (work < 2 * B) work = 2 * B;
      hipLaunchKernelGGL(prep_assemble_kernel, dim3((work + 255) / 256), dim3(256), 0, s, mask_lig, nlig, mask_pocket,
                         (int)n_pocket, B, e->node_batch, e->lig_off, e->poc_off, e->tile_ctr, xh_lig, dl, xh_pocket, dp,
                         t, (int)t_count, e->x, e->x_in, e->h0, J, JP);
      HIP_TRY(hipGetLastError());
    }
    if (fork) {
      if (!e->side_stream) HIP_TRY(hipStreamCreateWithFlags(&e->side_stream, hipStreamNonBlocking));
      if (!e->ev_fork) HIP_TRY(hipEventCreateWithFlags(&e->ev_fork, hipEventDisableTiming));
      if (!e->ev_join) HIP_TRY(hipEventCreateWithFlags(&e->ev_join, hipEventDisableTiming));
      HIP_TRY(hipEventRecord(e->ev_fork, s));
      HIP_TRY(hipStreamWaitEvent(e->side_stream, e->ev_fork, 0));
      sa = e->side_stream;
    }
    {
      Mlp2Problem enc[2] = {
          {xh_lig + 3, dl, a, W[DSBDD_G_ATOM_ENC_W0T], pad4(2 * a), W[DSBDD_G_ATOM_ENC_B0], 2 * a,
           W[DSBDD_G_ATOM_ENC_W1T], pad4(J), W[DSBDD_G_ATOM_ENC_B1], J, e->h0, JP, (int)n_lig},
          residue_encoder(e, *this)};
      if (mlp2_fits(enc[0]) && mlp2_fits(enc[1])) {
        HIP_TRY(launch_mlp2(sa, enc, (split0 && e->h0_pocket_valid) ? 1 : 2));
      } else {
        HIP_TRY(nl(sa, xh_lig + 3, dl, a, nullptr, 0, 0, W[DSBDD_G_ATOM_ENC_W0T], pad4(2 * a), W[DSBDD_G_ATOM_ENC_B0],
                   nullptr, 0, e->enc_tmp, LE, n_lig, 2 * a, 1));
        HIP_TRY(nl(sa, e->enc_tmp, LE, 2 * a, nullptr, 0, 0, W[DSBDD_G_ATOM_ENC_W1T], pad4(J),
                   W[DSBDD_G_ATOM_ENC_B1], nullptr, 0, e->h0, JP, n_lig, J, 0));
        float* tmp_p = e->enc_tmp + (size_t)n_lig * LE;
        HIP_TRY(nl(sa, xh_pocket + 3, dp, r, nullptr, 0, 0, W[DSBDD_G_RES_ENC_W0T], pad4(2 * r), W[DSBDD_G_RES_ENC_B0],
                   nullptr, 0, tmp_p, LE, n_pocket, 2 * r, 1));
        HIP_TRY(nl(sa, tmp_p, LE, 2 * r, nullptr, 0, 0, W[DSBDD_G_RES_ENC_W1T], pad4(J), W[DSBDD_G_RES_ENC_B1],
                   nullptr, 0, e->h0 + (size_t)n_lig * JP, JP, n_pocket, J, 0));
      }
    }
    HIP_TRY(nl(sa, e->h0, JP, JP, nullptr, 0, 0, W[DSBDD_G_EMB_WT], H, W[DSBDD_G_EMB_B], nullptr, 0, e->h, H, N, H, 0));
    if (split0) {
      hipLaunchKernelGGL(gather_rows_kernel, dim3((e->frame_n3 + 3) / 4), dim3(kThreads), 0, sa, e->h + (size_t)N * H,
                         (const float*)(e->h + (size_t)nlig * H), (const int*)e->frame_rows, (int)e->frame_n3, H);
      HIP_TRY(hipGetLastError());
    }
    if (fork) HIP_TRY(hipEventRecord(e->ev_join, sa));
    return DSBDD_OK;
  }

  int edge_list() {
    if (ext) {
      HIP_TRY(zero_async(e->deg, (size_t)N * 4, s));
      if (ext_n_edges > 0) {
        hipLaunchKernelGGL(ext_edges_kernel, dim3((int)((ext_n_edges + 255) / 256)), dim3(256), 0, s, ext_row,
                           ext_col, (int)ext_n_edges, (const float*)e->x, e->erow, e->ecol, e->ed0, e->deg);
        HIP_TRY(hipGetLastError());
      }
      hipLaunchKernelGGL(scan_kernel, dim3(1), dim3(1024), 0, s, (const int*)e->deg, e->row_ptr, N, SegAlign{},
                         (const int*)nullptr, (int*)nullptr, SegAlign{});
      HIP_TRY(hipGetLastError());
      edge_bound = ext_n_edges > 0 ? ext_n_edges : 1;
      if (subset) {
        hipLaunchKernelGGL(ext_flags_init_kernel, dim3((N + 255) / 256), dim3(256), 0, s, e->act_flag, nlig, N);
        HIP_TRY(hipGetLastError());
        if (ext_n_edges > 0) {
          hipLaunchKernelGGL(ext_flags_kernel, dim3((int)((ext_n_edges + 255) / 256)), dim3(256), 0, s, ext_row,
                             ext_col, (int)ext_n_edges, nlig, e->act_flag);
          HIP_TRY(hipGetLastError());
        }
      }
    } else {
      EdgeList2 l2{e->deg2, e->row_ptr2, e->erow2, e->ecol2, e->ed02, (int)e->cap_edges,
                   SegAlign{e->node_batch, e->lig_off, e->poc_off, nlig, B, e->scan_tmp2, e->seg_base2}};
      int rc = build_edges_impl(s, e->x, nlig, N, B, c, e->node_batch, e->lig_off, e->poc_off, e->deg,
                                e->row_ptr, e->erow, e->ecol, e->ed0, e->cap_edges, status,
                                subset ? e->act_flag : nullptr, e->scan_tmp, e->seg_base,
                                split0 ? &l2 : nullptr, 0, prune ? e->lvl : nullptr);
      if (rc) return rc;
      if (prune) {
        LevelArgs la{e->node_batch, e->lig_off, e->poc_off, nlig, B, e->lvl, e->deg, e->row_ptr, e->erow, e->ecol,
                     e->ed0, e->seg_rows, e->seg_edges, e->node_base, e->edge_base, e->lvl_cnt, e->lvl_end,
                     e->lvl_list, e->row_ptrL, e->erowL, e->ecolL, e->ed0L, (int)e->cap_edgesL, e->lvl_stats,
                     n_ghost, (int)ghost_slots, (int)e->cap_edges, nullptr, nullptr};
        mean_in_levels = e->fold_scan && n_mlp == 2;
        if (mean_in_levels) { la.mean_x = e->x; la.mean_out = e->mean; }
        if (!e->lvl_stats_zeroed) {
          HIP_TRY(zero_async(e->lvl_stats, 128, s));
          e->lvl_stats_zeroed = true;
        }
        hipLaunchKernelGGL(levels_kernel, dim3(B), dim3(kThreads), 0, s, la);
        HIP_TRY(hipGetLastError());
        if (!e->fold_scan) {
          hipLaunchKernelGGL(level_scan_kernel, dim3(1), dim3(1024), 0, s, la, N);
          HIP_TRY(hipGetLastError());
        }
        hipLaunchKernelGGL(level_place_kernel, dim3(B), dim3(kThreads), 0, s, la, e->fold_scan ? 1 : 0);
        HIP_TRY(hipGetLastError());
        int64_t cb = (e->cap_edges + 255) / 256;
        if (cb > 2048) cb = 2048;
        if (cb < 1) cb = 1;
        hipLaunchKernelGGL(level_copy_kernel, dim3((int)cb), dim3(256), 0, s, la, N);
        HIP_TRY(hipGetLastError());
      }
    }
    if (subset && !prune) {
      hipLaunchKernelGGL(scan_kernel, dim3(1), dim3(1024), 0, s, (const int*)e->act_flag, e->act_ptr, N, SegAlign{},
                         (const int*)nullptr, (int*)nullptr, SegAlign{});
      HIP_TRY(hipGetLastError());
      hipLaunchKernelGGL(compact_kernel, dim3((N + 255) / 256), dim3(256), 0, s, (const int*)e->act_flag,
                         (const int*)e->act_ptr, e->act_list, N);
      HIP_TRY(hipGetLastError());
    }
    if (fork) HIP_TRY(hipStreamWaitEvent(s, e->ev_join, 0));
    return DSBDD_OK;
  }

  int derived_weights() {
    const int rc = w2_pack_missing(e, s);
    if (rc) return rc;
    if (use_chain && !e->derived.chain) {
      auto pack = [&](const float* WT, int ldw, int K, int Ncols, const float* dst) {
        hipLaunchKernelGGL(pack_b16_kernel, dim3((K * Ncols + 255) / 256), dim3(256), 0, s, WT, ldw, K, Ncols,
                           const_cast<float*>(dst));
      };
      for (int blk = 0; blk < c.n_layers; ++blk) {
        for (int sub = 0; sub < c.inv_sublayers; ++sub) {
          pack(W[gcl_slot(c, blk, sub, DSBDD_GCL_N1_WT)], H, 2 * H, H, chain_w(blk, sub, 0));
          pack(W[gcl_slot(c, blk, sub, DSBDD_GCL_N2_WT)], H, H, H, chain_w(blk, sub, 1));
          pack(W[gcl_slot(c, blk, sub, DSBDD_GCL_E1_WT)], 2 * H, H, 2 * H, chain_w(blk, sub, 2));
        }
        pack(W[eq_slot(c, blk, DSBDD_EQ_C1_WT)], PQ, H, PQ, chain_w(blk, 0, 3));
      }
      HIP_TRY(hipGetLastError());
      e->derived.chain = true;
    }
    return DSBDD_OK;
  }

  int message_stage(int blk, int sub, StageState& st) {
    auto G = [&](int which) { return W[gcl_slot(c, blk, sub, which)]; };
    const bool first_split = split0 && blk == 0 && sub == 0;
    if (sub > 0 && st.chained_pq) st.pqg_ready = true;
    if (!st.pqg_ready) {
      NodeLinearArgs grp0[2];
      if (first_split) {
        grp0[0] = gcl_pq(blk, sub);
        grp0[0].row_idx = act_rows; grp0[0].m_count = act_count; grp0[0].M = N;
        grp0[1] = gcl_pq(blk, sub);
        grp0[1].A1 = e->h + (size_t)N * H; grp0[1].C = e->pqg + (size_t)N * 2 * H; grp0[1].M = n_frame_rows;
        grp0[1].row_idx = nullptr; grp0[1].m_count = nullptr;
      }
      if (!(first_split && launch_node_group(s, grp0, 2) == hipSuccess)) {
        (void)hipGetLastError();
        HIP_TRY(launch_node_linear(s, gcl_pq(blk, sub)));
        if (first_split) HIP_TRY(launch_node_linear(s, grp0[1]));
      }
    }
    st.pqg_ready = false;
    const int g = blk * c.inv_sublayers + sub;
    const int radius = radius_of(g);
    const bool ghost = g <= g_ghost_last;
    const bool all_rows = !prune || radius >= LV;
    const int64_t begin = ghost ? 0 : ghost_slots;
    EdgeArgs ea{};
    ea.erow = L_row + begin; ea.ecol = L_col + begin; ea.ed0 = L_d0 + begin;
    ea.e_count = !prune ? e_all : (ghost ? e->lvl_end + radius : e->lvl_end + kLevels + radius);
    ea.e_cap = L_cap - (int)begin; ea.wt_base = (int)(begin / 32); ea.x = e->x;
    ea.n_lig = nlig; ea.n_nodes = N + n_frame_rows; ea.ldpq = 2 * H;
    ea.mlp[0] = edge_mlp(e->pqg, e->pqg + H, G(DSBDD_GCL_E1_WD), G(DSBDD_GCL_E1_WD0), G(DSBDD_GCL_E1_TAB),
                         G(DSBDD_GCL_E2_WT), G(DSBDD_GCL_E2_B), blk, sub);
    ea.mlp[1] = ea.mlp[0];
    const bool g16 = ((e->granule16 >> (g & 15)) & 1u) && !first_split && !e->emu;
    const bool gsk = ((e->splitk >> (g & 15)) & 1u) && can_sk;
    ea.att_w = G(DSBDD_GCL_ATT_W); ea.att_b = G(DSBDD_GCL_ATT_B); ea.attention = c.attention;
    ea.agg = e->agg; ea.agg_head = e->agg_head; ea.tile_ctr = e->tile_ctr;
    ea.norm_factor = c.normalization_factor;
    if (first_split) {
      EdgeArgs a2 = ea;
      a2.erow = e->erow2; a2.ecol = e->ecol2; a2.ed0 = e->ed02; a2.e_count = e->row_ptr2 + N;
      a2.e_cap = (int)e->cap_edges; a2.wt_base = 0;
      EdgeArgs a3 = ea;
      a3.erow = e->erow3; a3.ecol = e->ecol3; a3.ed0 = e->ed03; a3.e_count = e->row_ptr3 + e->frame_n3;
      a3.agg = e->aggB; a3.agg_head = e->agg_headB; a3.e_cap = (int)e->cap_edges; a3.wt_base = 0;
      a2.erow_b = a3.erow; a2.ecol_b = a3.ecol; a2.ed0_b = a3.ed0; a2.e_count_b = a3.e_count; a2.e_cap_b = a3.e_cap;
      a2.wt_base_b = a3.wt_base; a2.agg_b = a3.agg; a2.agg_head_b = a3.agg_head;
      HIP_TRY(launch_edge(e, s, MODE_GCL, a2, edge_bound + ((e->frame_cap3 + 127) / 128) * 128, false, gsk));
      hipLaunchKernelGGL(agg_complete2_kernel, dim3((N + n_ghost + 3) / 4), dim3(kThreads), 0, s, e->agg,
                         (const float*)e->agg_head, (const int*)e->row_ptr2, (const int*)e->deg2,
                         (const float*)e->aggB, (const float*)e->agg_headB, (const int*)e->row_ptr3,
                         (const int*)e->deg3, (const int*)e->twin, N, nlig, N, H, cone ? n_ghost : 0, (int)e->cap_tiles - 1);
      HIP_TRY(hipGetLastError());
    } else {
      const bool timed = e->time_now && (all_rows || radius == e->plan_timed_level) && e->ev_used + 2 <= e->ev.size();
      if (timed) HIP_TRY(hipEventRecord(e->ev[e->ev_used], s));
      HIP_TRY(launch_edge(e, s, MODE_GCL, ea, L_bound(), g16 && !gsk, gsk));
      if (timed) {
        HIP_TRY(hipEventRecord(e->ev[e->ev_used + 1], s));
        e->ev_used += 2;
      }
      const int n_rows = N + (ghost ? n_ghost : 0);
      hipLaunchKernelGGL(agg_complete_kernel, dim3((n_rows + 3) / 4), dim3(kThreads), 0, s, e->agg,
                         (const float*)e->agg_head, L_ptr, (const int*)e->deg, n_rows, H,
                         (int)((g16 && !gsk) ? e->cap_tiles16 : e->cap_tiles) - 1, (g16 && !gsk) ? 4 : 5);
      HIP_TRY(hipGetLastError());
    }
    return node_phase(blk, sub, radius, ghost, st);
  }

  int node_phase(int blk, int sub, int radius, bool ghost, StageState& st) {
    auto G = [&](int which) { return W[gcl_slot(c, blk, sub, which)]; };
    const int g = blk * c.inv_sublayers + sub;
    NodeLinearArgs n1{e->h, H, H, e->agg, H, H, G(DSBDD_GCL_N1_WT), H, G(DSBDD_GCL_N1_B), nullptr, 0, e->t1, H,
                      (int)N, H, 1, nullptr, nullptr};
    NodeLinearArgs n2{e->t1, H, H, nullptr, 0, 0, G(DSBDD_GCL_N2_WT), H, G(DSBDD_GCL_N2_B), e->h, H, e->h, H,
                      (int)N, H, 0, nullptr, nullptr};
    rows_of(radius, ghost, n1); rows_of(radius, ghost, n2);
    st.chained_pq = false; st.chained_coord = false;
    bool fill_pq = false;
    if (use_chain) {
      NodeChainArgs ca{};
      ca.row_idx = n1.row_idx; ca.m_count = n1.m_count; ca.M = n1.M; ca.do_mlp = 1;
      ca.h = e->h; ca.agg = e->agg;
      ca.W1p = chain_w(blk, sub, 0); ca.b1 = G(DSBDD_GCL_N1_B);
      ca.W2p = chain_w(blk, sub, 1); ca.b2 = G(DSBDD_GCL_N2_B);
      const bool last_sub = sub + 1 == c.inv_sublayers;
      const int first = ghost ? n_ghost : 0;
      if (last_sub) {
        const int QW = n_mlp * H;
        const float* wc = chain_w(blk, 0, 3);
        if (!subset) {
          ca.proj[ca.n_proj++] = ChainProj{wc, e->pq, PQ, PQ, nullptr, 0};
          st.chained_coord = true;
        } else if (prune && n1.row_idx) {
          ca.proj[ca.n_proj++] = ChainProj{wc, e->pq, PQ, QW, act_count, first};
          ca.proj[ca.n_proj++] = ChainProj{wc + (size_t)(QW / 16) * (H / 16) * 256, e->pq + QW, PQ, QW,
                                           e->lvl_cnt + kLevels, first};
          st.chained_coord = true;
        }
      }
      const bool has_next = !last_sub || blk + 1 < c.n_layers;
      if (has_next) {
        const int nb = last_sub ? blk + 1 : blk, ns = last_sub ? 0 : sub + 1;
        const NodeLinearArgs nx = gcl_pq(nb, ns);
        const bool same_rows = nx.row_idx == n1.row_idx && nx.m_count == n1.m_count && nx.M == n1.M;
        if (same_rows || ghost) {
          ca.proj[ca.n_proj++] = ChainProj{chain_w(nb, ns, 2), e->pqg, 2 * H, 2 * H, nullptr, 0};
          st.chained_pq = true;
          fill_pq = ghost && !same_rows;
        }
      }
      HIP_TRY(launch_node_chain(s, ca, H, e->n_cu));
    } else {
      HIP_TRY(launch_node_linear(s, n1));
      HIP_TRY(launch_node_linear(s, n2));
    }
    if (ghost) {
      const int hi = radius_of(g + 1) + 1 < LV ? radius_of(g + 1) + 1 : LV;
      if (hi > radius) {
        hipLaunchKernelGGL(canon_fill_kernel, dim3((N - nlig + 3) / 4), dim3(kThreads), 0, s, e->h,
                           (const int*)e->lvl, (const int*)e->twin, nlig, N, N, radius, hi, H,
                           fill_pq ? e->pqg : (float*)nullptr, 2 * H);
        HIP_TRY(hipGetLastError());
      }
    }
    return DSBDD_OK;
  }

  int coord_stage(int blk, StageState& st) {
    auto Q = [&](int which) { return W[eq_slot(c, blk, which)]; };
    const int QW = n_mlp * H;
    NodeLinearArgs grp[kMaxGroup];
    int ng = 0;
    if (!st.chained_coord) {
      if (subset) {
        grp[ng++] = NodeLinearArgs{e->h, H, H, nullptr, 0, 0, Q(DSBDD_EQ_C1_WT), PQ, nullptr, nullptr, 0, e->pq, PQ,
                                   (int)N, QW, 0, act_rows, act_count};
        grp[ng++] = NodeLinearArgs{e->h, H, H, nullptr, 0, 0, Q(DSBDD_EQ_C1_WT) + QW, PQ, nullptr, nullptr, 0,
                                   e->pq + QW, PQ, (int)n_lig, QW, 0, nullptr, nullptr};
      } else {
        grp[ng++] = NodeLinearArgs{e->h, H, H, nullptr, 0, 0, Q(DSBDD_EQ_C1_WT), PQ, nullptr, nullptr, 0, e->pq, PQ,
                                   (int)N, PQ, 0, nullptr, nullptr};
      }
    }
    const int n_coord = ng;
    const bool want_next = blk + 1 < c.n_layers && !st.chained_pq;
    if (st.chained_pq && blk + 1 < c.n_layers) st.pqg_ready = true;
    if (want_next && use_chain) {
      const NodeLinearArgs nx = gcl_pq(blk + 1, 0);
      NodeChainArgs ca{};
      ca.row_idx = nx.row_idx; ca.m_count = nx.m_count; ca.M = nx.M; ca.do_mlp = 0; ca.h = e->h;
      ca.n_proj = 1;
      ca.proj[0] = ChainProj{chain_w(blk + 1, 0, 2), e->pqg, 2 * H, 2 * H, nullptr, 0};
      HIP_TRY(launch_node_chain(s, ca, H, e->n_cu));
      st.pqg_ready = true;
    } else if (want_next) {
      grp[ng++] = gcl_pq(blk + 1, 0);
    }
    if (ng > 0) {
      if (e->node_group && launch_node_group(s, grp, ng) == hipSuccess) {
        if (ng > n_coord) st.pqg_ready = true;
      } else {
        (void)hipGetLastError();
        for (int i = 0; i < n_coord; ++i) HIP_TRY(launch_node_linear(s, grp[i]));
      }
    }
    st.chained_pq = false;
    const int S = c.inv_sublayers;
    EdgeArgs ea{};
    ea.erow = L_row + ghost_slots; ea.ecol = L_col + ghost_slots; ea.ed0 = L_d0 + ghost_slots; ea.e_count = e_upd;
    ea.e_cap = L_cap - (int)ghost_slots; ea.wt_base = (int)(ghost_slots / 32); ea.x = e->x;
    ea.n_lig = nlig; ea.n_nodes = N + n_frame_rows; ea.ldpq = PQ;
    ea.mlp[0] = edge_mlp(e->pq + QW, e->pq, Q(DSBDD_EQ_C_WD), Q(DSBDD_EQ_C_WD0), Q(DSBDD_EQ_C_TAB),
                         Q(DSBDD_EQ_C_W2T), Q(DSBDD_EQ_C_B2), blk, S);
    if (n_mlp == 2)
      ea.mlp[1] = edge_mlp(e->pq + QW + H, e->pq + H, Q(DSBDD_EQ_X_WD), Q(DSBDD_EQ_X_WD0), Q(DSBDD_EQ_X_TAB),
                           Q(DSBDD_EQ_X_W2T), Q(DSBDD_EQ_X_B2), blk, S + 1);
    else
      ea.mlp[1] = ea.mlp[0];
    ea.w3 = Q(DSBDD_EQ_W3); ea.node_batch = e->node_batch; ea.mean = e->mean;
    ea.norm_constant = c.norm_constant; ea.coords_range = c.coords_range; ea.use_tanh = c.use_tanh;
    ea.n_mlp = n_mlp; ea.xagg = e->xagg; ea.xagg_head = e->xagg_head;
    const bool csk = ((e->splitk >> (16 + (blk & 15))) & 1u) && can_sk;
    const bool c16 = ((e->granule16 >> (16 + (blk & 15))) & 1u) && !e->emu && !csk;
    ea.xagg_stride = (size_t)N * 3; ea.xhead_stride = (size_t)(c16 ? e->cap_tiles16 : e->cap_tiles) * 4;
    ea.tile_ctr = e->tile_ctr; ea.norm_factor = c.normalization_factor;
    ea.pass_split = (c16 || csk) ? 1 : e->coord_split;
    if (e->ts_buf && e->ts_next < e->ts_cap) ea.ts = e->ts_buf + (size_t)(e->ts_next++) * 1024;
    HIP_TRY(launch_edge(e, s, MODE_COORD, ea, L_bound(), c16, csk));
    const int n_q = ((e->coord_split || c16 || csk) && n_mlp == 2) ? 2 : 1;
    const int c_shift = c16 ? 4 : 5, c_max = (int)(c16 ? e->cap_tiles16 : e->cap_tiles) - 1;
    const bool next_mean = subset && n_mlp == 2 && blk + 1 < c.n_layers;
    if (!subset) {
      if (n_upd > 0) {
        hipLaunchKernelGGL(coord_update_kernel, dim3((3 * n_upd + 255) / 256), dim3(256), 0, s, e->x,
                           (const float*)e->xagg, (const float*)e->xagg_head, n_q, ea.xagg_stride, ea.xhead_stride,
                           L_ptr, (const int*)e->deg, 3 * n_upd, c_max, c_shift);
        HIP_TRY(hipGetLastError());
      }
    } else if (n_upd > 0 || next_mean) {
      hipLaunchKernelGGL(coord_update_mean_kernel, dim3(B), dim3(kThreads), 0, s, e->x, (const float*)e->xagg,
                         (const float*)e->xagg_head, n_q, ea.xagg_stride, ea.xhead_stride, L_ptr,
                         (const int*)e->deg, n_upd, (const int*)e->lig_off, (const int*)e->poc_off, nlig,
                         next_mean ? e->mean : (float*)nullptr, c_max, c_shift);
      HIP_TRY(hipGetLastError());
    }
    return DSBDD_OK;
  }

  int output_head() {
    LigHeadArgs lh{e->h, H, W[DSBDD_G_EMBOUT_WT], JP, W[DSBDD_G_EMBOUT_B], J,
                   W[DSBDD_G_ATOM_DEC_W0T], pad4(2 * a), W[DSBDD_G_ATOM_DEC_B0], 2 * a,
                   W[DSBDD_G_ATOM_DEC_W1T], pad4(a), W[DSBDD_G_ATOM_DEC_B1], a,
                   e->x, e->x_in, nlig, N, eps_lig, dl, status};
    if (e->lig_head && !eps_pocket && !c.update_pocket_coords && lig_head_fits(lh)) {
      HIP_TRY(launch_lig_head(s, lh));
      return DSBDD_OK;
    }
    HIP_TRY(nl(s, e->h, H, H, nullptr, 0, 0, W[DSBDD_G_EMBOUT_WT], JP, W[DSBDD_G_EMBOUT_B], nullptr, 0, e->hout, JP,
               eps_pocket ? N : n_lig, JP, 0));
    {
      Mlp2Problem dec[2] = {
          {e->hout, JP, J, W[DSBDD_G_ATOM_DEC_W0T], pad4(2 * a), W[DSBDD_G_ATOM_DEC_B0], 2 * a,
           W[DSBDD_G_ATOM_DEC_W1T], pad4(a), W[DSBDD_G_ATOM_DEC_B1], a, eps_lig + 3, dl, (int)n_lig},
          {e->hout + (size_t)n_lig * JP, JP, J, W[DSBDD_G_RES_DEC_W0T], pad4(2 * r), W[DSBDD_G_RES_DEC_B0], 2 * r,
           W[DSBDD_G_RES_DEC_W1T], pad4(r), W[DSBDD_G_RES_DEC_B1], r, eps_pocket ? eps_pocket + 3 : nullptr, dp,
           (int)n_pocket}};
      if (mlp2_fits(dec[0]) && mlp2_fits(dec[1])) {
        HIP_TRY(launch_mlp2(s, dec, eps_pocket ? 2 : 1));
      } else {
        HIP_TRY(nl(s, e->hout, JP, J, nullptr, 0, 0, W[DSBDD_G_ATOM_DEC_W0T], pad4(2 * a), W[DSBDD_G_ATOM_DEC_B0], nullptr, 0,
                   e->enc_tmp, LE, n_lig, 2 * a, 1));
        HIP_TRY(nl(s, e->enc_tmp, LE, 2 * a, nullptr, 0, 0, W[DSBDD_G_ATOM_DEC_W1T], pad4(a), W[DSBDD_G_ATOM_DEC_B1], nullptr, 0,
                   eps_lig + 3, dl, n_lig, a, 0));
        if (eps_pocket) {
          float* tmp_p = e->enc_tmp + (size_t)n_lig * LE;
          HIP_TRY(nl(s, e->hout + (size_t)n_lig * JP, JP, J, nullptr, 0, 0, W[DSBDD_G_RES_DEC_W0T], pad4(2 * r),
                     W[DSBDD_G_RES_DEC_B0], nullptr, 0, tmp_p, LE, n_pocket, 2 * r, 1));
          HIP_TRY(nl(s, tmp_p, LE, 2 * r, nullptr, 0, 0, W[DSBDD_G_RES_DEC_W1T], pad4(r), W[DSBDD_G_RES_DEC_B1], nullptr, 0,
                     eps_pocket + 3, dp, n_pocket, r, 0));
        }
      }
    }
    hipLaunchKernelGGL(finalize_kernel, dim3(B), dim3(kThreads), 0, s, (const float*)e->x, (const float*)e->x_in,
                       (const int*)e->lig_off, (const int*)e->poc_off, nlig, c.update_pocket_coords, eps_lig, dl,
                       eps_pocket, dp, status);
    HIP_TRY(hipGetLastError());
    return DSBDD_OK;
  }

  int run() {
    if (N == 0) return DSBDD_OK;
    plan();
    int rc = assemble_and_encode();
    if (rc == DSBDD_OK) rc = edge_list();
    if (rc == DSBDD_OK) rc = derived_weights();
    StageState st;
    for (int blk = 0; blk < c.n_layers && rc == DSBDD_OK; ++blk) {
      if (n_mlp == 2 && (blk == 0 || !subset) && !(blk == 0 && mean_in_levels)) {
        hipLaunchKernelGGL(sample_mean_kernel, dim3(B), dim3(kThreads), 0, s, (const float*)e->x,
                           (const int*)e->lig_off, (const int*)e->poc_off, nlig, e->mean);
        HIP_TRY(hipGetLastError());
      }
      for (int sub = 0; sub < c.inv_sublayers && rc == DSBDD_OK; ++sub) rc = message_stage(blk, sub, st);
      if (rc == DSBDD_OK) rc = coord_stage(blk, st);
      if (rc != DSBDD_OK) break;
      if (e->trace_h)
        HIP_TRY(hipMemcpyAsync(e->trace_h + (size_t)blk * N * H, e->h, (size_t)N * H * 4, hipMemcpyDeviceToDevice, s));
      if (e->trace_x)
        HIP_TRY(hipMemcpyAsync(e->trace_x + (size_t)blk * N * 3, e->x, (size_t)N * 12, hipMemcpyDeviceToDevice, s));
    }
    return rc == DSBDD_OK ? output_head() : rc;
  }
};

static int forward_impl(dsbdd_engine* e, hipStream_t s, const ForwardArgs& args) { return Forward(e, s, args).run(); }
```

diffsbdd_amd/csrc/graph.h:

```cpp
#pragma once
#include "common.h"

namespace dsbdd {

constexpr int kTileCtrInts = 32;
constexpr int kEdgeAlign = 32;
constexpr int kLevels = 5;

struct Cutoffs {
  int has_l, has_p, has_i;
  float cl, cp, ci;
};

__device__ __forceinline__ int lower_bound_i64(const int64_t* a, int n, int64_t v) {
  int lo = 0, hi = n;
  while (lo < hi) {
    const int mid = (lo + hi) >> 1;
    if (a[mid] < v) lo = mid + 1; else hi = mid;
  }
  return lo;
}

__global__ void prep_kernel(const int64_t* mask_lig, int n_lig, const int64_t* mask_poc, int n_poc,
                            int B, int* node_batch, int* lig_off, int* poc_off, int* tile_ctr) {
  const int i = blockIdx.x * blockDim.x + threadIdx.x;
  if (tile_ctr && i < kTileCtrInts) tile_ctr[i] = 0;
  if (i < n_lig) node_batch[i] = (int)mask_lig[i];
  else if (i < n_lig + n_poc) node_batch[i] = (int)mask_poc[i - n_lig];
  if (i <= B) {
    lig_off[i] = lower_bound_i64(mask_lig, n_lig, i);
    poc_off[i] = lower_bound_i64(mask_poc, n_poc, i);
  }
}

struct SegAlign {
  const int* node_batch; const int* lig_off; const int* poc_off;
  int n_lig; int B;
  int* scan_tmp;
  int* seg_base;
};

__device__ __forceinline__ int wave_sum_i(int v) {
#pragma unroll
  for (int o = 32; o > 0; o >>= 1) v += __shfl_xor(v, o);
  return v;
}

struct EdgeList2 {
  int* deg; int* row_ptr; int* erow; int* ecol; float* ed0; int e_cap;
  SegAlign seg;
};

template <bool FILL>
__global__ __launch_bounds__(kThreads) void edges_kernel(
    const float* __restrict__ x, const int* __restrict__ node_batch,
    const int* __restrict__ lig_off, const int* __restrict__ poc_off, int n_lig, int n_nodes,
    Cutoffs cut, int* __restrict__ deg, const int* __restrict__ row_ptr, int* __restrict__ erow,
    int* __restrict__ ecol, float* __restrict__ ed0, int e_cap, int* __restrict__ status,
    int* __restrict__ act_flag, SegAlign seg, int* __restrict__ row_ptr_out, EdgeList2 l2, int id_offset,
    int* __restrict__ lvl = nullptr) {
  const int lane = threadIdx.x & 63;
  const int wave = (blockIdx.x * blockDim.x + threadIdx.x) >> 6;
  const int nwaves = (gridDim.x * blockDim.x) >> 6;
  for (int i = wave; i < n_nodes; i += nwaves) {
    const int b = node_batch[i];
    const bool il = i < n_lig;
    const float xi = x[3 * i], yi = x[3 * i + 1], zi = x[3 * i + 2];
    int base = 0;
    int base2 = 0;
    if (FILL) {
      if (seg.seg_base) {
        const int k = il ? b : seg.B + b;
        const int first = il ? lig_off[b] : n_lig + poc_off[b];
        base = seg.seg_base[k] + seg.scan_tmp[i] - seg.scan_tmp[first];
        if (lane == 0) row_ptr_out[i] = base;
      } else {
        base = row_ptr[i];
      }
    }
    if (FILL && l2.deg) {
      const int k = il ? b : l2.seg.B + b;
      const int first = il ? lig_off[b] : n_lig + poc_off[b];
      base2 = l2.seg.seg_base[k] + l2.seg.scan_tmp[i] - l2.seg.scan_tmp[first];
      if (lane == 0) l2.row_ptr[i] = base2;
    }
    int cnt = 0, cnt_lig = 0;
#pragma unroll 1
    for (int seg = 0; seg < 2; ++seg) {
      const int j_begin = seg == 0 ? lig_off[b] : n_lig + poc_off[b];
      const int j_end = seg == 0 ? lig_off[b + 1] : n_lig + poc_off[b + 1];
      const bool jl = seg == 0;
      const int has = (il && jl) ? cut.has_l : ((!il && !jl) ? cut.has_p : cut.has_i);
      const float c = (il && jl) ? cut.cl : ((!il && !jl) ? cut.cp : cut.ci);
      for (int j0 = j_begin; j0 < j_end; j0 += 64) {
        const int j = j0 + lane;
        const bool valid = j < j_end;
        float d2 = 0.f;
        if (valid) {
          const float dx = xi - x[3 * j], dy = yi - x[3 * j + 1], dz = zi - x[3 * j + 2];
          d2 = dx * dx + dy * dy + dz * dz;
        }
        const bool pass = valid && (!has || __fsqrt_rn(d2) <= c);
        const unsigned long long m = __ballot(pass);
        if (FILL && pass) {
          const int pos = base + cnt + __popcll(m & ((1ull << lane) - 1ull));
          if (pos >= 0 && pos < e_cap) {
            erow[pos] = i + id_offset; ecol[pos] = j + id_offset; ed0[pos] = d2;
          }
          if (l2.deg && (il || jl)) {
            const int pos2 = base2 + cnt + __popcll(m & ((1ull << lane) - 1ull));
            if (pos2 >= 0 && pos2 < l2.e_cap) { l2.erow[pos2] = i; l2.ecol[pos2] = j; l2.ed0[pos2] = d2; }
          }
        }
        cnt += __popcll(m);
      }
      if (seg == 0) cnt_lig = cnt;
    }
    if (!FILL && lane == 0) {
      deg[i] = cnt;
      if (l2.deg) l2.deg[i] = il ? cnt : cnt_lig;
      if (act_flag) act_flag[i] = (il || cnt_lig > 0) ? 1 : 0;
      if (lvl) lvl[i] = il ? 0 : (cnt_lig > 0 ? 1 : kLevels - 1);
    }
    if (FILL && lane == 0 && base + cnt > e_cap) atomicOr(status, 2);
    if (FILL && seg.seg_base) {
      const int seg_last = (il ? lig_off[b + 1] : n_lig + poc_off[b + 1]) - 1;
      if (i == seg_last) {
        const int from = base + cnt, to = (from + kEdgeAlign - 1) & ~(kEdgeAlign - 1);
        const int pos = from + lane;
        if (pos >= 0 && pos < to && pos < e_cap) { erow[pos] = -1; ecol[pos] = 0; ed0[pos] = 0.f; }
        if (l2.deg) {
          const int from2 = base2 + (il ? cnt : cnt_lig), to2 = (from2 + kEdgeAlign - 1) & ~(kEdgeAlign - 1);
          const int p2 = from2 + lane;
          if (p2 >= 0 && p2 < to2 && p2 < l2.e_cap) { l2.erow[p2] = -1; l2.ecol[p2] = 0; l2.ed0[p2] = 0.f; }
        }
      }
    }
  }
}

__device__ __forceinline__ int block_scan_1024(int mine, int* s_wave, int* s_total) {
  const int t = threadIdx.x, lane = t & 63, w = t >> 6;
  int incl = mine;
#pragma unroll
  for (int o = 1; o < 64; o <<= 1) {
    const int u = __shfl_up(incl, o);
    if (lane >= o) incl += u;
  }
  if (lane == 63) s_wave[w] = incl;
  __syncthreads();
  if (w == 0) {
    int tot = lane < 16 ? s_wave[lane] : 0;
    int inc = tot;
#pragma unroll
    for (int o = 1; o < 16; o <<= 1) {
      const int u = __shfl_up(inc, o);
      if (lane >= o) inc += u;
    }
    if (lane < 16) s_wave[lane] = inc - tot;
    if (lane == 15) *s_total = inc;
  }
  __syncthreads();
  const int r = s_wave[w] + incl - mine;
  return r;
}

__device__ void scan_one(const int* deg, int* row_ptr, int n, SegAlign seg, int* s_wave, int* s_carry_p);

__global__ __launch_bounds__(1024) void scan_kernel(const int* deg, int* row_ptr, int n, SegAlign seg,
                                                    const int* deg_b, int* row_ptr_b, SegAlign seg_b) {
  __shared__ int s_wave[16];
  __shared__ int s_carry;
  scan_one(deg, row_ptr, n, seg, s_wave, &s_carry);
  if (deg_b) {
    __syncthreads();
    scan_one(deg_b, row_ptr_b, n, seg_b, s_wave, &s_carry);
  }
}

__device__ void scan_one(const int* deg, int* row_ptr, int n, SegAlign seg, int* s_wave, int* s_carry_p) {
  int& s_carry = *s_carry_p;
  const int t = threadIdx.x;
  int* out = seg.seg_base ? seg.scan_tmp : row_ptr;
  const bool vec = ((reinterpret_cast<uintptr_t>(deg) | reinterpret_cast<uintptr_t>(out)) & 15) == 0;
  int carry = 0;
  for (int base = 0; base < n; base += 4096) {
    const int i0 = base + 4 * t;
    int v[4] = {0, 0, 0, 0};
    if (vec && i0 + 3 < n) {
      const int4 q = *reinterpret_cast<const int4*>(deg + i0);
      v[0] = q.x; v[1] = q.y; v[2] = q.z; v[3] = q.w;
    } else {
#pragma unroll
      for (int k = 0; k < 4; ++k) if (i0 + k < n) v[k] = deg[i0 + k];
    }
    const int mine = v[0] + v[1] + v[2] + v[3];
    int run = carry + block_scan_1024(mine, s_wave, s_carry_p);
    const int tile_total = s_carry;
    if (vec && i0 + 3 < n) {
      int4 o4;
      o4.x = run; o4.y = run + v[0]; o4.z = o4.y + v[1]; o4.w = o4.z + v[2];
      *reinterpret_cast<int4*>(out + i0) = o4;
    } else {
#pragma unroll
      for (int k = 0; k < 4; ++k) if (i0 + k < n) { out[i0 + k] = run; run += v[k]; }
    }
    carry += tile_total;
    __syncthreads();
  }
  if (t == 0) out[n] = carry;
  if (!seg.seg_base) return;
  __syncthreads();
  const int S = 2 * seg.B;
  auto seg_begin = [&](int k) { return k < seg.B ? seg.lig_off[k] : seg.n_lig + seg.poc_off[k - seg.B]; };
  auto seg_end = [&](int k) { return k < seg.B ? seg.lig_off[k + 1] : seg.n_lig + seg.poc_off[k - seg.B + 1]; };
  carry = 0;
  for (int base = 0; base < S; base += 1024) {
    const int k = base + t;
    int len = 0;
    if (k < S) len = (max(out[seg_end(k)] - out[seg_begin(k)], 0) + kEdgeAlign - 1) & ~(kEdgeAlign - 1);
    const int ex = carry + block_scan_1024(len, s_wave, s_carry_p);
    if (k < S) seg.seg_base[k] = ex;
    carry += s_carry;
    __syncthreads();
  }
  if (t == 0) {
    seg.seg_base[S] = carry;
    row_ptr[n] = carry;
  }
}

__device__ __forceinline__ void sample_mean_body(const float* x, const int* lig_off, const int* poc_off, int n_lig,
                                                 float* mean, float (*red)[kThreads]) {
  const int b = blockIdx.x, t = threadIdx.x;
  const int l0 = lig_off[b], l1 = lig_off[b + 1], p0 = n_lig + poc_off[b], p1 = n_lig + poc_off[b + 1];
  float s0 = 0.f, s1 = 0.f, s2 = 0.f;
  for (int i = l0 + t; i < l1; i += kThreads) { s0 += x[3 * i]; s1 += x[3 * i + 1]; s2 += x[3 * i + 2]; }
  for (int i = p0 + t; i < p1; i += kThreads) { s0 += x[3 * i]; s1 += x[3 * i + 1]; s2 += x[3 * i + 2]; }
  red[0][t] = s0; red[1][t] = s1; red[2][t] = s2;
  __syncthreads();
  for (int o = kThreads / 2; o > 0; o >>= 1) {
    if (t < o) { red[0][t] += red[0][t + o]; red[1][t] += red[1][t + o]; red[2][t] += red[2][t + o]; }
    __syncthreads();
  }
  if (t < 3) {
    int cnt = (l1 - l0) + (p1 - p0);
    if (cnt == 0) cnt = 1;
    mean[3 * b + t] = red[t][0] / (float)cnt;
  }
  __syncthreads();
}

struct LevelArgs {
  const int* node_batch; const int* lig_off; const int* poc_off; int n_lig; int B;
  int* lvl;
  const int* deg;
  const int* row_ptr_nat;
  const int* erow_nat; const int* ecol_nat; const float* ed0_nat;
  int* seg_rows;
  int* seg_edges;
  int* node_base;
  int* edge_base;
  int* lvl_cnt;
  int* lvl_end;
  int* lvl_list;
  int* row_ptr;
  int* erow; int* ecol; float* ed0; int e_cap;
  unsigned long long* stats;
  int node_off; int edge_off;
  int e_cap_nat;
  const float* mean_x; float* mean_out;
};

__global__ __launch_bounds__(kThreads) void levels_kernel(LevelArgs a) {
  __shared__ int s_rows[kLevels], s_edges[kLevels];
  __shared__ float s_red[3][kThreads];
  if (a.mean_out) sample_mean_body(a.mean_x, a.lig_off, a.poc_off, a.n_lig, a.mean_out, s_red);
  const int b = blockIdx.x, t = threadIdx.x;
  const int p0 = a.n_lig + a.poc_off[b], p1 = a.n_lig + a.poc_off[b + 1];
  const int l0 = a.lig_off[b], l1 = a.lig_off[b + 1];
  if (t < kLevels) { s_rows[t] = 0; s_edges[t] = 0; }
  for (int k = 2; k < kLevels - 1; ++k) {
    __syncthreads();
    for (int i = p0 + t; i < p1; i += kThreads) {
      if (a.lvl[i] != kLevels - 1) continue;
      const int s = a.row_ptr_nat[i], d = a.deg[i];
      bool hit = false;
      for (int e = max(s, 0); e < min(s + d, a.e_cap_nat) && !hit; ++e) {
        const int j = a.ecol_nat[e];
        hit = j >= a.n_lig && a.lvl[j] == k - 1;
      }
      if (hit) a.lvl[i] = k;
    }
  }
  __syncthreads();
  for (int i = p0 + t; i < p1; i += kThreads) {
    const int L = a.lvl[i];
    atomicAdd(&s_rows[L], 1);
    atomicAdd(&s_edges[L], a.deg[i]);
  }
  int le = 0;
  for (int i = l0 + t; i < l1; i += kThreads) le += a.deg[i];
  if (le) atomicAdd(&s_edges[0], le);
  __syncthreads();
  if (t < kLevels) {
    a.seg_rows[t * a.B + b] = t == 0 ? (l1 - l0) : s_rows[t];
    a.seg_edges[t * a.B + b] = s_edges[t];
  }
}

__global__ __launch_bounds__(1024) void level_scan_kernel(LevelArgs a, int n_nodes) {
  __shared__ int s_wave[16];
  __shared__ int s_tot;
  const int t = threadIdx.x, S = kLevels * a.B;
  int carry_n = 0, carry_e = 0;
  for (int base = 0; base < S; base += 1024) {
    const int k = base + t;
    const int r = k < S ? a.seg_rows[k] : 0;
    const int e = k < S ? ((a.seg_edges[k] + kEdgeAlign - 1) & ~(kEdgeAlign - 1)) : 0;
    const int xn = carry_n + block_scan_1024(r, s_wave, &s_tot);
    carry_n += s_tot;
    __syncthreads();
    const int xe = carry_e + block_scan_1024(e, s_wave, &s_tot);
    carry_e += s_tot;
    __syncthreads();
    if (k < S) { a.node_base[k] = a.node_off + xn; a.edge_base[k] = a.edge_off + xe; }
  }
  if (t == 0) { a.node_base[S] = a.node_off + carry_n; a.edge_base[S] = a.edge_off + carry_e; }
  __syncthreads();
  if (t < kLevels) {
    const int cn = t == kLevels - 1 ? a.node_off + carry_n : a.node_base[(t + 1) * a.B];
    const int ce = t == kLevels - 1 ? a.edge_off + carry_e : a.edge_base[(t + 1) * a.B];
    a.lvl_cnt[t] = cn; a.lvl_cnt[kLevels + t] = cn - a.node_off;
    a.lvl_end[t] = ce; a.lvl_end[kLevels + t] = ce - a.edge_off;
    if (a.stats) {
      int own = 0;
      for (int k = t * a.B; k < (t + 1) * a.B; ++k) own += a.seg_edges[k];
      s_wave[t] = own;
      __threadfence_block();
      __builtin_amdgcn_wave_barrier();
      unsigned long long ed = 0;
      for (int k = 0; k <= t; ++k) ed += (unsigned long long)s_wave[k];
      a.stats[t] += (unsigned long long)(cn - a.node_off);
      a.stats[kLevels + t] += (unsigned long long)(ce - a.edge_off);
      a.stats[2 * kLevels + t] += ed;
      if (t == 0) a.stats[3 * kLevels] += 1ull;
    }
  }
}

__device__ __forceinline__ void level_bases(const LevelArgs& a, int k, int lane, int& nb, int& eb) {
  int sn = 0, se = 0;
  for (int k0 = 0; k0 < k; k0 += 64) {
    const int kk = k0 + lane;
    if (kk < k) { sn += a.seg_rows[kk]; se += (a.seg_edges[kk] + kEdgeAlign - 1) & ~(kEdgeAlign - 1); }
  }
  nb = a.node_off + wave_sum_i(sn);
  eb = a.edge_off + wave_sum_i(se);
}

__global__ __launch_bounds__(kThreads) void level_place_kernel(LevelArgs a, int fold_scan = 0) {
  static_assert(kThreads / 64 >= kLevels - 1, "one wave per pocket level");
  const int b = blockIdx.x, lane = threadIdx.x & 63, w = threadIdx.x >> 6;
  if (fold_scan && b == 0 && w == kThreads / 64 - 1) {
    unsigned long long ed_run = 0;
    for (int t = 0; t < kLevels; ++t) {
      int cn, ce;
      level_bases(a, (t + 1) * a.B, lane, cn, ce);
      int own = 0;
      for (int k0 = t * a.B; k0 < (t + 1) * a.B; k0 += 64) { const int kk = k0 + lane; if (kk < (t + 1) * a.B) own += a.seg_edges[kk]; }
      ed_run += (unsigned long long)wave_sum_i(own);
      if (lane == 0) {
        a.lvl_cnt[t] = cn; a.lvl_cnt[kLevels + t] = cn - a.node_off;
        a.lvl_end[t] = ce; a.lvl_end[kLevels + t] = ce - a.edge_off;
        if (a.stats) {
          a.stats[t] += (unsigned long long)(cn - a.node_off);
          a.stats[kLevels + t] += (unsigned long long)(ce - a.edge_off);
          a.stats[2 * kLevels + t] += ed_run;
          if (t == 0) a.stats[3 * kLevels] += 1ull;
        }
      }
    }
  }
  auto pads = [&](int from) {
    const int to = (from + kEdgeAlign - 1) & ~(kEdgeAlign - 1), pos = from + lane;
    if (pos < to && pos < a.e_cap) { a.erow[pos] = -1; a.ecol[pos] = 0; a.ed0[pos] = 0.f; }
  };
  if (w == 0) {
    const int l0 = a.lig_off[b], l1 = a.lig_off[b + 1];
    int nb, eb;
    if (fold_scan) level_bases(a, b, lane, nb, eb); else { nb = a.node_base[b]; eb = a.edge_base[b]; }
    const int s0 = l0 < l1 ? a.row_ptr_nat[l0] : 0;
    for (int i = l0 + lane; i < l1; i += 64) {
      a.lvl_list[nb + (i - l0)] = i;
      a.row_ptr[i] = eb + (a.row_ptr_nat[i] - s0);
    }
    pads(eb + a.seg_edges[b]);
  }
  const int L = w + 1;
  if (L >= kLevels) return;
  const int p0 = a.n_lig + a.poc_off[b], p1 = a.n_lig + a.poc_off[b + 1];
  int n_run, e_run;
  if (fold_scan) level_bases(a, L * a.B + b, lane, n_run, e_run);
  else { n_run = a.node_base[L * a.B + b]; e_run = a.edge_base[L * a.B + b]; }
  for (int i0 = p0; i0 < p1; i0 += 64) {
    const int i = i0 + lane;
    const bool mine = i < p1 && a.lvl[i] == L;
    const int d = mine ? a.deg[i] : 0;
    const unsigned long long m = __ballot(mine);
    int incl = d;
#pragma unroll
    for (int o = 1; o < 64; o <<= 1) {
      const int u = __shfl_up(incl, o);
      if (lane >= o) incl += u;
    }
    if (mine) {
      a.lvl_list[n_run + __popcll(m & ((1ull << lane) - 1ull))] = i;
      a.row_ptr[i] = e_run + incl - d;
    }
    n_run += __popcll(m);
    e_run += __shfl(incl, 63);
  }
  pads(e_run);
}

__global__ void ghost_setup_kernel(const int* erow3, const int* ecol3, const float* ed03, const int* row_ptr3,
                                   const int* deg3, int n3, int id_src, int id_dst, int* erow, int* ecol,
                                   float* ed0, int e_cap, int* deg, int* row_ptr, int* lvl_list,
                                   const float* xframe, float* x) {
  const int total = min(row_ptr3[n3], e_cap);
  for (int p = blockIdx.x * blockDim.x + threadIdx.x; p < total; p += gridDim.x * blockDim.x) {
    const int r = erow3[p];
    erow[p] = r < 0 ? -1 : r - id_src + id_dst;
    ecol[p] = r < 0 ? 0 : ecol3[p] - id_src + id_dst;
    ed0[p] = ed03[p];
  }
  for (int i = blockIdx.x * blockDim.x + threadIdx.x; i < n3; i += gridDim.x * blockDim.x) {
    deg[id_dst + i] = deg3[i];
    row_ptr[id_dst + i] = row_ptr3[i];
    lvl_list[i] = id_dst + i;
    x[3 * (id_dst + i)] = xframe[3 * i]; x[3 * (id_dst + i) + 1] = xframe[3 * i + 1];
    x[3 * (id_dst + i) + 2] = xframe[3 * i + 2];
  }
}

__global__ __launch_bounds__(kThreads) void gather_rows_kernel(float* dst, const float* src, const int* rows, int n,
                                                               int H) {
  const int i = (blockIdx.x * kThreads + threadIdx.x) >> 6, lane = threadIdx.x & 63;
  if (i >= n) return;
  const float* a = src + (size_t)rows[i] * H;
  float* b = dst + (size_t)i * H;
  for (int k = 4 * lane; k < H; k += 256) *reinterpret_cast<float4*>(b + k) = ld4(a + k);
}

__global__ __launch_bounds__(kThreads) void canon_fill_kernel(float* h, const int* lvl, const int* twin_local,
                                                              int n_lig, int n_nodes, int ghost_base, int lo,
                                                              int hi, int H, float* pq = nullptr, int ldpq = 0) {
  const int i = n_lig + ((blockIdx.x * kThreads + threadIdx.x) >> 6), lane = threadIdx.x & 63;
  if (i >= n_nodes) return;
  const int L = lvl[i];
  if (L <= lo || L > hi) return;
  const int g = ghost_base + twin_local[i - n_lig];
  const float* src = h + (size_t)g * H;
  float* dst = h + (size_t)i * H;
  for (int k = 4 * lane; k < H; k += 256) *reinterpret_cast<float4*>(dst + k) = ld4(src + k);
  if (pq)
    for (int k = 4 * lane; k < ldpq; k += 256)
      *reinterpret_cast<float4*>(pq + (size_t)i * ldpq + k) = ld4(pq + (size_t)g * ldpq + k);
}

__global__ void level_copy_kernel(LevelArgs a, int n_nodes) {
  const int total = min(a.row_ptr_nat[n_nodes], a.e_cap_nat);
  for (int e = blockIdx.x * blockDim.x + threadIdx.x; e < total; e += gridDim.x * blockDim.x) {
    const int i = a.erow_nat[e];
    if (i < 0 || i >= n_nodes) continue;
    const int pos = a.row_ptr[i] + (e - a.row_ptr_nat[i]);
    if (pos >= 0 && pos < a.e_cap) { a.erow[pos] = i; a.ecol[pos] = a.ecol_nat[e]; a.ed0[pos] = a.ed0_nat[e]; }
  }
}

__global__ void zero_kernel(uint4* p, size_t n16, unsigned char* tail, int n_tail) {
  const uint4 z = make_uint4(0u, 0u, 0u, 0u);
  for (size_t i = blockIdx.x * (size_t)blockDim.x + threadIdx.x; i < n16; i += (size_t)gridDim.x * blockDim.x)
    p[i] = z;
  if (blockIdx.x == 0 && (int)threadIdx.x < n_tail) tail[threadIdx.x] = 0;
}

__global__ void copy16_kernel(uint4* dst, const uint4* src, size_t n16) {
  const size_t i = blockIdx.x * (size_t)blockDim.x + threadIdx.x;
  if (i < n16) dst[i] = src[i];
}

inline hipError_t zero_async(void* ptr, size_t bytes, hipStream_t s) {
  if (bytes == 0) return hipSuccess;
  const size_t n16 = bytes / 16;
  const int n_tail = (int)(bytes % 16);
  size_t blocks = (n16 + 255) / 256;
  if (blocks > 2048) blocks = 2048;
  if (blocks < 1) blocks = 1;
  hipLaunchKernelGGL(zero_kernel, dim3((unsigned)blocks), dim3(256), 0, s, static_cast<uint4*>(ptr), n16,
                     static_cast<unsigned char*>(ptr) + n16 * 16, n_tail);
  return hipGetLastError();
}

__global__ void permute_w2t_kernel(const float* src, float* dst, int H) {
  const int i = blockIdx.x * blockDim.x + threadIdx.x;
  if (i >= H * H) return;
  const int k = i / H, o = i % H, ct = H / 32;
  const int j = o / ct, c = o % ct;
  dst[i] = src[k * H + c * 32 + j];
}

__global__ void ext_edges_kernel(const int* row, const int* col, int E, const float* x, int* erow,
                                 int* ecol, float* ed0, int* deg) {
  const int e = blockIdx.x * blockDim.x + threadIdx.x;
  if (e >= E) return;
  const int r = row[e], c = col[e];
  erow[e] = r; ecol[e] = c;
  const float dx = x[3 * r] - x[3 * c], dy = x[3 * r + 1] - x[3 * c + 1], dz = x[3 * r + 2] - x[3 * c + 2];
  ed0[e] = dx * dx + dy * dy + dz * dz;
  atomicAdd(&deg[r], 1);
}

__global__ void ext_flags_init_kernel(int* flag, int n_lig, int n_nodes) {
  const int i = blockIdx.x * blockDim.x + threadIdx.x;
  if (i < n_nodes) flag[i] = i < n_lig ? 1 : 0;
}
__global__ void ext_flags_kernel(const int* row, const int* col, int E, int n_lig, int* flag) {
  const int e = blockIdx.x * blockDim.x + threadIdx.x;
  if (e < E && row[e] < n_lig) flag[col[e]] = 1;
}
__global__ void compact_kernel(const int* flag, const int* ptr, int* list, int n) {
  const int i = blockIdx.x * blockDim.x + threadIdx.x;
  if (i < n && flag[i]) list[ptr[i]] = i;
}

__global__ void assemble_kernel(const float* xh_lig, int dl, const float* xh_poc, int dp, int n_lig,
                                int n_nodes, const int* node_batch, const float* t, int t_count,
                                float* x, float* x_in, float* h0, int J, int JP) {
  const int i = blockIdx.x * blockDim.x + threadIdx.x;
  if (i >= n_nodes) return;
  const float* src = i < n_lig ? xh_lig + (size_t)i * dl : xh_poc + (size_t)(i - n_lig) * dp;
  const float a = src[0], b = src[1], c = src[2];
  x[3 * i] = a; x[3 * i + 1] = b; x[3 * i + 2] = c;
  x_in[3 * i] = a; x_in[3 * i + 1] = b; x_in[3 * i + 2] = c;
  h0[(size_t)i * JP + J] = t[t_count == 1 ? 0 : node_batch[i]];
  for (int k = J + 1; k < JP; ++k) h0[(size_t)i * JP + k] = 0.f;
}

__global__ void prep_assemble_kernel(const int64_t* mask_lig, int n_lig, const int64_t* mask_poc, int n_poc, int B,
                                     int* node_batch, int* lig_off, int* poc_off, int* tile_ctr, const float* xh_lig,
                                     int dl, const float* xh_poc, int dp, const float* t, int t_count, float* x,
                                     float* x_in, float* h0, int J, int JP) {
  const int i = blockIdx.x * blockDim.x + threadIdx.x;
  if (tile_ctr && i < kTileCtrInts) tile_ctr[i] = 0;
  if (i <= B) {
    lig_off[i] = lower_bound_i64(mask_lig, n_lig, i);
    poc_off[i] = lower_bound_i64(mask_poc, n_poc, i);
  }
  if (i >= n_lig + n_poc) return;
  const int b = (int)(i < n_lig ? mask_lig[i] : mask_poc[i - n_lig]);
  node_batch[i] = b;
  const float* src = i < n_lig ? xh_lig + (size_t)i * dl : xh_poc + (size_t)(i - n_lig) * dp;
  const float a0 = src[0], a1 = src[1], a2 = src[2];
  x[3 * i] = a0; x[3 * i + 1] = a1; x[3 * i + 2] = a2;
  x_in[3 * i] = a0; x_in[3 * i + 1] = a1; x_in[3 * i + 2] = a2;
  h0[(size_t)i * JP + J] = t[t_count == 1 ? 0 : b];
  for (int k = J + 1; k < JP; ++k) h0[(size_t)i * JP + k] = 0.f;
}

__global__ __launch_bounds__(kThreads) void sample_mean_kernel(const float* x, const int* lig_off,
                                                               const int* poc_off, int n_lig,
                                                               float* mean) {
  __shared__ float red[3][kThreads];
  sample_mean_body(x, lig_off, poc_off, n_lig, mean, red);
}

__global__ void coord_update_kernel(float* x, const float* xagg, const float* xhead, int n_q,
                                    size_t xagg_stride, size_t xhead_stride, const int* row_ptr,
                                    const int* deg, int n_upd3, int max_tile, int shift) {
  const int idx = blockIdx.x * blockDim.x + threadIdx.x;
  if (idx >= n_upd3) return;
  const int i = idx / 3, c = idx - 3 * i;
  const int d = deg[i];
  if (d == 0) return;
  const int s = row_ptr[i], t0 = s >> shift, t1 = min((s + d - 1) >> shift, max_tile);
  float tot = 0.f;
  for (int q = 0; q < n_q; ++q) {
    float a = xagg[q * xagg_stride + idx];
    for (int T = t0 + 1; T <= t1; ++T) a += xhead[q * xhead_stride + 4 * (size_t)T + c];
    tot += a;
  }
  x[idx] += tot;
}

__global__ __launch_bounds__(kThreads) void coord_update_mean_kernel(
    float* x, const float* xagg, const float* xhead, int n_q, size_t xagg_stride, size_t xhead_stride,
    const int* row_ptr, const int* deg, int n_upd, const int* lig_off, const int* poc_off, int n_lig, float* mean,
    int max_tile, int shift) {
  __shared__ float red[3][kThreads];
  const int b = blockIdx.x, t = threadIdx.x;
  const int l0 = lig_off[b], l1 = lig_off[b + 1], p0 = n_lig + poc_off[b], p1 = n_lig + poc_off[b + 1];
  for (int seg = 0; seg < 2; ++seg) {
    const int a = seg ? p0 : l0, e = min(seg ? p1 : l1, n_upd);
    for (int k = 3 * a + t; k < 3 * e; k += kThreads) {
      const int i = k / 3, c = k - 3 * i;
      const int d = deg[i];
      if (d == 0) continue;
      const int s = row_ptr[i], t0 = s >> shift, t1 = min((s + d - 1) >> shift, max_tile);
      float tot = 0.f;
      for (int q = 0; q < n_q; ++q) {
        float v = xagg[q * xagg_stride + k];
        for (int T = t0 + 1; T <= t1; ++T) v += xhead[q * xhead_stride + 4 * (size_t)T + c];
        tot += v;
      }
      x[k] += tot;
    }
  }
  if (!mean) return;
  __syncthreads();
  float s0 = 0.f, s1 = 0.f, s2 = 0.f;
  for (int i = l0 + t; i < l1; i += kThreads) { s0 += x[3 * i]; s1 += x[3 * i + 1]; s2 += x[3 * i + 2]; }
  for (int i = p0 + t; i < p1; i += kThreads) { s0 += x[3 * i]; s1 += x[3 * i + 1]; s2 += x[3 * i + 2]; }
  red[0][t] = s0; red[1][t] = s1; red[2][t] = s2;
  __syncthreads();
  for (int o = kThreads / 2; o > 0; o >>= 1) {
    if (t < o) { red[0][t] += red[0][t + o]; red[1][t] += red[1][t + o]; red[2][t] += red[2][t + o]; }
    __syncthreads();
  }
  if (t < 3) {
    int cnt = (l1 - l0) + (p1 - p0);
    if (cnt == 0) cnt = 1;
    mean[3 * b + t] = red[t][0] / (float)cnt;
  }
}

__global__ __launch_bounds__(kThreads) void finalize_kernel(
    const float* x, const float* x_in, const int* lig_off, const int* poc_off, int n_lig,
    int remove_mean, float* eps_lig, int dl, float* eps_poc, int dp, int* status) {
  __shared__ float red[3][kThreads];
  const int b = blockIdx.x, t = threadIdx.x;
  const int l0 = lig_off[b], l1 = lig_off[b + 1], p0 = n_lig + poc_off[b], p1 = n_lig + poc_off[b + 1];
  float m0 = 0.f, m1 = 0.f, m2 = 0.f;
  bool nan = false;
  if (remove_mean) {
    float s0 = 0.f, s1 = 0.f, s2 = 0.f;
    for (int seg = 0; seg < 2; ++seg) {
      const int a = seg ? p0 : l0, e = seg ? p1 : l1;
      for (int i = a + t; i < e; i += kThreads) {
        s0 += x[3 * i] - x_in[3 * i]; s1 += x[3 * i + 1] - x_in[3 * i + 1]; s2 += x[3 * i + 2] - x_in[3 * i + 2];
      }
    }
    red[0][t] = s0; red[1][t] = s1; red[2][t] = s2;
    __syncthreads();
    for (int o = kThreads / 2; o > 0; o >>= 1) {
      if (t < o) { red[0][t] += red[0][t + o]; red[1][t] += red[1][t + o]; red[2][t] += red[2][t + o]; }
      __syncthreads();
    }
    int cnt = (l1 - l0) + (p1 - p0);
    if (cnt == 0) cnt = 1;
    m0 = red[0][0] / (float)cnt; m1 = red[1][0] / (float)cnt; m2 = red[2][0] / (float)cnt;
  }
  for (int seg = 0; seg < 2; ++seg) {
    const int a = seg ? p0 : l0, e = seg ? p1 : l1;
    for (int i = a + t; i < e; i += kThreads) {
      const float v0 = x[3 * i] - x_in[3 * i], v1 = x[3 * i + 1] - x_in[3 * i + 1],
                  v2 = x[3 * i + 2] - x_in[3 * i + 2];
      nan = nan || (v0 != v0) || (v1 != v1) || (v2 != v2);
      float* dst = nullptr;
      if (seg == 0) dst = eps_lig + (size_t)i * dl;
      else if (eps_poc) dst = eps_poc + (size_t)(i - n_lig) * dp;
      if (dst) { dst[0] = v0 - m0; dst[1] = v1 - m1; dst[2] = v2 - m2; }
    }
  }
  if (nan) atomicOr(status, 1);
}

}
```

diffsbdd_amd/csrc/graph_cache.h:

```cpp
#pragma once

static int ghost_setup(dsbdd_engine* e, hipStream_t s) {
  const int n3 = (int)e->frame_n3, N = (int)(e->frame_nlig + e->frame_npoc);
  int64_t gb = (e->frame_cap3 + 255) / 256;
  if (gb > 1024) gb = 1024;
  hipLaunchKernelGGL(ghost_setup_kernel, dim3((int)gb), dim3(256), 0, s, (const int*)e->erow3, (const int*)e->ecol3,
                     (const float*)e->ed03, (const int*)e->row_ptr3, (const int*)e->deg3, n3, N, N, e->erowL,
                     e->ecolL, e->ed0L, (int)e->cap_edgesL, e->deg, e->row_ptrL, e->lvl_list,
                     (const float*)e->xframe, e->x);
  HIP_TRY(hipGetLastError());
  e->ghost_dirty = false;
  return DSBDD_OK;
}

static int frame_upkeep(dsbdd_engine* e, hipStream_t s, const ForwardArgs& a) {
  if (!frame_applies(e, a)) {
    e->ghost_dirty = true;
    e->h0_pocket_valid = false;
    return DSBDD_OK;
  }
  if (e->ghost_dirty) {
    int rc = ghost_setup(e, s);
    if (rc) return rc;
  }
  if (!e->h0_pocket_valid) {
    Mlp2Problem enc = residue_encoder(e, a);
    if (mlp2_fits(enc)) {
      HIP_TRY(launch_mlp2(s, &enc, 1));
      e->h0_pocket_valid = true;
    }
  }
  return DSBDD_OK;
}

static dsbdd_engine::GraphEntry* graph_entry(dsbdd_engine* e, hipStream_t s, const ForwardArgs& a) {
  std::vector<uint64_t> key = {(uint64_t)(uintptr_t)a.xh_lig, (uint64_t)(uintptr_t)a.xh_pocket, (uint64_t)(uintptr_t)a.t,
                               (uint64_t)a.t_count, (uint64_t)(uintptr_t)a.mask_lig, (uint64_t)(uintptr_t)a.mask_pocket,
                               (uint64_t)a.n_lig, (uint64_t)a.n_pocket, (uint64_t)a.batch, (uint64_t)(uintptr_t)a.eps_lig,
                               (uint64_t)(uintptr_t)a.eps_pocket, (uint64_t)(uintptr_t)a.status,
                               (uint64_t)(uintptr_t)e->ws, (uint64_t)(uintptr_t)e->slots.data()[0],
                               (uint64_t)(uintptr_t)s, (uint64_t)e->frame};
  for (auto& ge : e->graphs)
    if (ge.key == key) return &ge;
  if (e->graphs.size() >= 8) {
    e->graphs.front().destroy();
    e->graphs.erase(e->graphs.begin());
  }
  e->graphs.emplace_back();
  e->graphs.back().key = std::move(key);
  return &e->graphs.back();
}

static int graph_capture(dsbdd_engine* e, const ForwardArgs& a, dsbdd_engine::GraphEntry* g) {
  const DerivedReady before = e->derived;
  HIP_TRY(hipStreamBeginCapture(e->cap_stream, hipStreamCaptureModeThreadLocal));
  const int rc = forward_impl(e, e->cap_stream, a);
  hipGraph_t graph = nullptr;
  hipGraphExec_t exec = nullptr;
  const hipError_t ec = hipStreamEndCapture(e->cap_stream, &graph);
  const bool ok = rc == DSBDD_OK && ec == hipSuccess && graph &&
                  hipGraphInstantiate(&exec, graph, nullptr, nullptr, 0) == hipSuccess && exec;
  if (!ok) {
    if (graph) (void)hipGraphDestroy(graph);
    e->use_graph = 0;
    e->derived = before;
    return rc;
  }
  g->graph = graph;
  g->exec = exec;
  g->plan_radius = e->plan_radius; g->plan_ghost = e->plan_ghost; g->plan_timed_level = e->plan_timed_level;
  return DSBDD_OK;
}

static int forward_cached(dsbdd_engine* e, hipStream_t s, const ForwardArgs& a) {
  dsbdd_engine::GraphEntry* g = graph_entry(e, s, a);
  if (g->exec) {
    ++e->n_replay;
    HIP_TRY(hipGraphLaunch(g->exec, s));
    e->plan_radius = g->plan_radius; e->plan_ghost = g->plan_ghost; e->plan_timed_level = g->plan_timed_level;
    return DSBDD_OK;
  }
  ++e->n_eager;
  if (g->seen++ == 0) return forward_impl(e, s, a);
  if (!e->cap_stream) HIP_TRY(hipStreamCreateWithFlags(&e->cap_stream, hipStreamNonBlocking));
  const int rc = graph_capture(e, a, g);
  if (rc != DSBDD_OK) return rc;
  if (!g->exec) return forward_impl(e, s, a);
  ++e->n_capture;
  HIP_TRY(hipGraphLaunch(g->exec, s));
  return DSBDD_OK;
}
```

diffsbdd_amd/csrc/launch.h:

```cpp
#pragma once

static hipError_t nl(hipStream_t s, const float* A1, int lda1, int K1, const float* A2, int lda2, int K2,
                     const float* WT, int ldw, const float* bias, const float* R, int ldr, float* C,
                     int ldc, int64_t M, int N, int act) {
  NodeLinearArgs a{A1, lda1, K1, A2, lda2, K2, WT, ldw, bias, R, ldr, C, ldc, (int)M, N, act, nullptr, nullptr};
  return launch_node_linear(s, a);
}

template <class... P, class... A>
static int launch_1d(void (*kernel)(P...), size_t n_items, hipStream_t s, A... args) {
  hipLaunchKernelGGL(kernel, dim3((unsigned)((n_items + 255) / 256)), dim3(256), 0, s, static_cast<P>(args)...);
  HIP_TRY(hipGetLastError());
  return DSBDD_OK;
}

static int device_cus() {
  static int cache[64] = {0};
  int dev = 0;
  if (hipGetDevice(&dev) != hipSuccess || dev < 0 || dev >= 64) return 256;
  if (cache[dev] == 0) {
    hipDeviceProp_t pr;
    int n = 0;
    if (hipGetDeviceProperties(&pr, dev) == hipSuccess) n = pr.multiProcessorCount;
    cache[dev] = n > 0 ? n : 256;
  }
  return cache[dev];
}

static int persistent_grid(int64_t items, int n_cu, int per_cu, int max_wg, int quantum) {
  int64_t resident = (int64_t)per_cu * n_cu;
  if (max_wg > 0 && max_wg < resident) resident = max_wg;
  if (items > resident) items = resident;
  const int grid = (int)((items + quantum - 1) / quantum * quantum);
  return grid < quantum ? quantum : grid;
}

template <int H>
static hipError_t launch_wave_emu_t(hipStream_t s, int mode, const EdgeArgs& a, int grid, int emu) {
  if (emu == 9) {
    if (mode == MODE_GCL) hipLaunchKernelGGL((edge_wave_kernel<H, MODE_GCL, false, 9>), dim3(grid), dim3(kThreads), 0, s, a);
    else hipLaunchKernelGGL((edge_wave_kernel<H, MODE_COORD, false, 9>), dim3(grid), dim3(kThreads), 0, s, a);
  } else {
    if (mode == MODE_GCL) hipLaunchKernelGGL((edge_wave_kernel<H, MODE_GCL, false, 6>), dim3(grid), dim3(kThreads), 0, s, a);
    else hipLaunchKernelGGL((edge_wave_kernel<H, MODE_COORD, false, 6>), dim3(grid), dim3(kThreads), 0, s, a);
  }
  return hipGetLastError();
}

template <int H>
static hipError_t launch_wave_t(hipStream_t s, int mode, const EdgeArgs& a, int grid) {
  constexpr bool can_perm = (H == 256 || H == 128);
  if constexpr (can_perm) {
    if (a.mlp[0].W2TP && a.mlp[1].W2TP) {
      if (mode == MODE_GCL)
        hipLaunchKernelGGL((edge_wave_kernel<H, MODE_GCL, true>), dim3(grid), dim3(kThreads), 0, s, a);
      else
        hipLaunchKernelGGL((edge_wave_kernel<H, MODE_COORD, true>), dim3(grid), dim3(kThreads), 0, s, a);
      return hipGetLastError();
    }
  }
  if (mode == MODE_GCL)
    hipLaunchKernelGGL((edge_wave_kernel<H, MODE_GCL, false>), dim3(grid), dim3(kThreads), 0, s, a);
  else
    hipLaunchKernelGGL((edge_wave_kernel<H, MODE_COORD, false>), dim3(grid), dim3(kThreads), 0, s, a);
  return hipGetLastError();
}

template <int H>
static hipError_t launch_wave_store_t(hipStream_t s, int mode, const EdgeArgs& a, int grid) {
  if (mode == MODE_GCL) hipLaunchKernelGGL((edge_wave_kernel<H, MODE_GCL, false, 0, true>), dim3(grid), dim3(kThreads), 0, s, a);
  else hipLaunchKernelGGL((edge_wave_kernel<H, MODE_COORD, false, 0, true>), dim3(grid), dim3(kThreads), 0, s, a);
  return hipGetLastError();
}

template <int H>
static hipError_t launch_wave16_t(hipStream_t s, int mode, const EdgeArgs& a, int grid) {
  if (mode == MODE_GCL) hipLaunchKernelGGL((edge_wave16_kernel<H, MODE_GCL>), dim3(grid), dim3(kThreads), 0, s, a);
  else hipLaunchKernelGGL((edge_wave16_kernel<H, MODE_COORD>), dim3(grid), dim3(kThreads), 0, s, a);
  return hipGetLastError();
}

static hipError_t launch_edge16(const dsbdd_engine* e, hipStream_t s, int mode, const EdgeArgs& a, int64_t edge_bound) {
  const int64_t items = (edge_bound + 63) / 64 * (mode == MODE_COORD ? a.n_mlp : 1);
  const int grid = persistent_grid(items, e->n_cu, 2, e->edge_max_wg, 1);
  return with_hidden(e->cfg.hidden_nf, [&](auto h) { return launch_wave16_t<decltype(h)::value>(s, mode, a, grid); });
}

static hipError_t launch_edge_sk(const dsbdd_engine* e, hipStream_t s, int mode, const EdgeArgs& a, int64_t edge_bound) {
  const bool two = mode == MODE_COORD && a.n_mlp == 2;
  const int64_t items = (edge_bound + 31) / 32 * (two ? 2 : 1);
  const int grid = persistent_grid(items, e->n_cu, 2, e->edge_max_wg, two ? 16 : 8);
  if (e->cfg.hidden_nf != 256) return hipErrorInvalidValue;
  if (mode == MODE_GCL) hipLaunchKernelGGL((edge_splitk_kernel<256, MODE_GCL>), dim3(grid), dim3(kThreads), 0, s, a);
  else hipLaunchKernelGGL((edge_splitk_kernel<256, MODE_COORD>), dim3(grid), dim3(kThreads), 0, s, a);
  return hipGetLastError();
}

static int edge_wave_grid(int mode, const EdgeArgs& a, int64_t edge_bound, int n_cu, int max_wg) {
  const int64_t tiles = (edge_bound + 127) / 128;
  const bool split = mode == MODE_COORD && a.pass_split && a.n_mlp == 2;
  return persistent_grid(split ? 2 * tiles : tiles, n_cu, 2, max_wg, split ? 16 : 8);
}

static hipError_t launch_edge(const dsbdd_engine* e, hipStream_t s, int mode, const EdgeArgs& a,
                              int64_t edge_bound, bool g16 = false, bool sk = false) {
  if (sk && a.mlp[0].W2SK) return launch_edge_sk(e, s, mode, a, edge_bound);
  if (g16) return launch_edge16(e, s, mode, a, edge_bound);
  const int grid = edge_wave_grid(mode, a, edge_bound, e->n_cu, e->edge_max_wg);
  const int emu = (e->emu && a.mlp[0].W2E && a.mlp[1].W2E) ? e->emu : 0;
  return with_hidden(e->cfg.hidden_nf, [&](auto h) {
    constexpr int H = decltype(h)::value;
    return emu ? launch_wave_emu_t<H>(s, mode, a, grid, emu) : launch_wave_t<H>(s, mode, a, grid);
  });
}

static hipError_t launch_edge_plain(int H, hipStream_t s, int mode, const EdgeArgs& a, int64_t edge_bound) {
  const int grid = edge_wave_grid(mode, a, edge_bound, device_cus(), 0);
  if (a.z2_out && (a.e_count_b || a.wt_base)) return hipErrorInvalidValue;
  return with_hidden(H, [&](auto h) {
    constexpr int HH = decltype(h)::value;
    return a.z2_out ? launch_wave_store_t<HH>(s, mode, a, grid) : launch_wave_t<HH>(s, mode, a, grid);
  });
}

static Cutoffs cutoffs_of(const dsbdd_config& c) {
  return Cutoffs{c.has_cutoff_ligand, c.has_cutoff_pocket, c.has_cutoff_interaction,
                 c.cutoff_ligand, c.cutoff_pocket, c.cutoff_interaction};
}

static int build_edges_impl(hipStream_t s, const float* x, int n_lig, int N, int B, const dsbdd_config& c,
                            const int* node_batch, const int* lig_off, const int* poc_off, int* deg,
                            int* row_ptr, int* erow, int* ecol, float* ed0, int64_t cap, int* status,
                            int* act_flag = nullptr, int* scan_tmp = nullptr, int* seg_base = nullptr,
                            const EdgeList2* list2 = nullptr, int id_offset = 0, int* lvl = nullptr) {
  const int waves_per_block = kThreads / 64;
  int blocks = (N + waves_per_block - 1) / waves_per_block;
  if (blocks > 4096) blocks = 4096;
  if (blocks < 1) blocks = 1;
  const Cutoffs cut = cutoffs_of(c);
  const int aligned = scan_tmp && seg_base;
  SegAlign sg{node_batch, lig_off, poc_off, n_lig, B, scan_tmp, aligned ? seg_base : nullptr};
  EdgeList2 l2{};
  if (list2 && aligned) l2 = *list2;
  hipLaunchKernelGGL((edges_kernel<false>), dim3(blocks), dim3(kThreads), 0, s, x, node_batch, lig_off,
                     poc_off, n_lig, N, cut, deg, (const int*)nullptr, (int*)nullptr, (int*)nullptr,
                     (float*)nullptr, 0, status, act_flag, SegAlign{}, (int*)nullptr, l2, 0, lvl);
  HIP_TRY(hipGetLastError());
  hipLaunchKernelGGL(scan_kernel, dim3(1), dim3(1024), 0, s, (const int*)deg, row_ptr, N, sg,
                     (const int*)l2.deg, l2.row_ptr, l2.seg);
  HIP_TRY(hipGetLastError());
  hipLaunchKernelGGL((edges_kernel<true>), dim3(blocks), dim3(kThreads), 0, s, x, node_batch, lig_off,
                     poc_off, n_lig, N, cut, deg, (const int*)row_ptr, erow, ecol, ed0, (int)cap, status,
                     (int*)nullptr, sg, row_ptr, l2, id_offset, (int*)nullptr);
  HIP_TRY(hipGetLastError());
  return DSBDD_OK;
}
```

include/diffsbdd_hip.h:

```cpp
#ifndef DIFFSBDD_HIP_H
#define DIFFSBDD_HIP_H

#include <stddef.h>
#include <stdint.h>

#ifdef __cplusplus
extern "C" {
#endif

#define DSBDD_ABI_VERSION 6

enum {
  DSBDD_OK = 0,
  DSBDD_ERR_ARG = -1,
  DSBDD_ERR_STATE = -2,
  DSBDD_ERR_CAPACITY = -3,
  DSBDD_ERR_LAUNCH = -4
};

enum {
  DSBDD_STATUS_NAN = 1,
  DSBDD_STATUS_EDGE_OVERFLOW = 2
};

typedef struct dsbdd_config {
  int32_t atom_nf, residue_nf, joint_nf, hidden_nf;
  int32_t n_layers, inv_sublayers;
  int32_t attention, use_tanh, update_pocket_coords, reflection_equivariant;
  int32_t edge_embedding_dim;
  int32_t has_cutoff_ligand, has_cutoff_pocket, has_cutoff_interaction;
  float cutoff_ligand, cutoff_pocket, cutoff_interaction;
  float norm_constant, normalization_factor, coords_range;
} dsbdd_config;

typedef struct dsbdd_engine dsbdd_engine;

enum {
  DSBDD_G_ATOM_ENC_W0T = 0, DSBDD_G_ATOM_ENC_B0, DSBDD_G_ATOM_ENC_W1T, DSBDD_G_ATOM_ENC_B1,
  DSBDD_G_RES_ENC_W0T, DSBDD_G_RES_ENC_B0, DSBDD_G_RES_ENC_W1T, DSBDD_G_RES_ENC_B1,
  DSBDD_G_ATOM_DEC_W0T, DSBDD_G_ATOM_DEC_B0, DSBDD_G_ATOM_DEC_W1T, DSBDD_G_ATOM_DEC_B1,
  DSBDD_G_RES_DEC_W0T, DSBDD_G_RES_DEC_B0, DSBDD_G_RES_DEC_W1T, DSBDD_G_RES_DEC_B1,
  DSBDD_G_EMB_WT,
  DSBDD_G_EMB_B,
  DSBDD_G_EMBOUT_WT,
  DSBDD_G_EMBOUT_B,
  DSBDD_G_COUNT
};
enum {
  DSBDD_GCL_E1_WT = 0,
  DSBDD_GCL_E1_WD,
  DSBDD_GCL_E1_WD0,
  DSBDD_GCL_E1_TAB,
  DSBDD_GCL_E2_WT,
  DSBDD_GCL_E2_B,
  DSBDD_GCL_ATT_W,
  DSBDD_GCL_ATT_B,
  DSBDD_GCL_N1_WT,
  DSBDD_GCL_N1_B,
  DSBDD_GCL_N2_WT,
  DSBDD_GCL_N2_B,
  DSBDD_GCL_COUNT
};
enum {
  DSBDD_EQ_C1_WT = 0,
  DSBDD_EQ_C_WD,
  DSBDD_EQ_C_WD0, DSBDD_EQ_C_TAB, DSBDD_EQ_C_W2T, DSBDD_EQ_C_B2,
  DSBDD_EQ_X_WD,
  DSBDD_EQ_X_WD0, DSBDD_EQ_X_TAB, DSBDD_EQ_X_W2T, DSBDD_EQ_X_B2,
  DSBDD_EQ_W3,
  DSBDD_EQ_COUNT
};

int dsbdd_abi_version(void);
const char* dsbdd_last_error(void);

int dsbdd_engine_create(const dsbdd_config* cfg, dsbdd_engine** out);
void dsbdd_engine_destroy(dsbdd_engine* e);
int dsbdd_engine_weight_slots(const dsbdd_engine* e);
int dsbdd_engine_set_weights(dsbdd_engine* e, const float* const* slots_host, int n_slots);

size_t dsbdd_engine_workspace_bytes(const dsbdd_engine* e, int64_t n_lig, int64_t n_pocket,
                                    int64_t batch, int64_t edge_capacity);
int dsbdd_engine_bind_workspace(dsbdd_engine* e, void* workspace, size_t bytes, int64_t n_lig,
                                int64_t n_pocket, int64_t batch, int64_t edge_capacity);

int dsbdd_engine_set_pocket_frame(dsbdd_engine* e, void* stream, const float* x_frame, const int64_t* mask_frame,
                                  const int32_t* frame_rows, const int32_t* twin_local, int64_t n_lig,
                                  int64_t n_pocket, int64_t batch, int64_t n_frame, int64_t batch_frame,
                                  int64_t edge_bound_frame);
int dsbdd_engine_clear_pocket_frame(dsbdd_engine* e);

int dsbdd_engine_set_trace(dsbdd_engine* e, float* trace_h, float* trace_x);

int dsbdd_dynamics_forward(dsbdd_engine* e, void* stream, const float* xh_lig,
                           const float* xh_pocket, const float* t, int64_t t_count,
                           const int64_t* mask_lig, const int64_t* mask_pocket, int64_t n_lig,
                           int64_t n_pocket, int64_t batch, const int32_t* ext_row,
                           const int32_t* ext_col, int64_t ext_n_edges, float* eps_lig,
                           float* eps_pocket, int32_t* status);

int dsbdd_engine_profile(dsbdd_engine* e, int enable, int max_launches);
int dsbdd_engine_profile_read(dsbdd_engine* e, double* total_ms, int64_t* launches);

int dsbdd_engine_graph_stats(const dsbdd_engine* e, int64_t* replays, int64_t* captures, int64_t* eager);

int dsbdd_engine_last_plan(const dsbdd_engine* e, int32_t* radius, int32_t* ghost, int32_t capacity,
                           int32_t* n_stages, int32_t* timed_level);

enum { DSBDD_OPT_PRUNE = 0, DSBDD_OPT_CONE = 1, DSBDD_OPT_GRANULE16 = 2, DSBDD_OPT_EMU = 3, DSBDD_OPT_SPLITK = 4 };
int dsbdd_engine_set_option(dsbdd_engine* e, int which, int value);
int dsbdd_engine_get_option(const dsbdd_engine* e, int which);

enum {
  DSBDD_BUF_EDGE_ROW = 0, DSBDD_BUF_EDGE_COL, DSBDD_BUF_EDGE_D0, DSBDD_BUF_ROW_PTR,
  DSBDD_BUF_H, DSBDD_BUF_X, DSBDD_BUF_NODE_BATCH, DSBDD_BUF_DEG,
  DSBDD_BUF_LEVEL, DSBDD_BUF_LEVEL_LIST, DSBDD_BUF_LEVEL_COUNT, DSBDD_BUF_LEVEL_END,
  DSBDD_BUF_LROW_PTR, DSBDD_BUF_LEDGE_ROW, DSBDD_BUF_LEDGE_COL, DSBDD_BUF_LEDGE_D0,
  DSBDD_BUF_LEVEL_STATS
};
int dsbdd_engine_buffer(const dsbdd_engine* e, int which, void** ptr_out);

int dsbdd_cond_reverse_update(void* stream, float* z_lig, float* xh_pocket, const float* eps_lig,
                              const float* noise, const int64_t* mask_lig,
                              const int64_t* mask_pocket, int64_t n_lig, int64_t n_pocket,
                              int64_t batch, int32_t atom_nf, int32_t residue_nf, float alpha_ts,
                              float c_eps, float sigma, int32_t remove_com);

int dsbdd_joint_reverse_update(void* stream, float* z_lig, float* z_pocket, const float* eps_lig,
                               const float* eps_pocket, const float* noise_lig,
                               const float* noise_pocket, const int64_t* mask_lig,
                               const int64_t* mask_pocket, int64_t n_lig, int64_t n_pocket,
                               int64_t batch, int32_t atom_nf, int32_t residue_nf, float alpha_ts,
                               float c_eps, float sigma, int32_t center_noise);

int dsbdd_segment_mean3(void* stream, const float* x, int32_t ld, const int64_t* mask, int64_t n_rows,
                        int64_t batch, float* out);

int dsbdd_cond_affine_noise(void* stream, float* z_lig, float* xh_pocket, const float* noise,
                            const int64_t* mask_lig, const int64_t* mask_pocket, int64_t n_lig,
                            int64_t n_pocket, int64_t batch, int32_t atom_nf, int32_t residue_nf, float a,
                            float sigma, int32_t remove_com);

int dsbdd_joint_affine_noise(void* stream, float* z_lig, float* z_pocket, const float* noise_lig,
                             const float* noise_pocket, const int64_t* mask_lig, const int64_t* mask_pocket,
                             int64_t n_lig, int64_t n_pocket, int64_t batch, int32_t atom_nf,
                             int32_t residue_nf, float a, float sigma, int32_t center_noise,
                             int32_t remove_com);

int dsbdd_cond_repaint_update(void* stream, float* z_lig, float* xh_pocket, float* scratch_lig,
                              const float* xh0_lig, const float* com_pocket0, const float* fixed,
                              const float* noise_known, const float* noise_resample, const int64_t* mask_lig,
                              const int64_t* mask_pocket, int64_t n_lig, int64_t n_pocket, int64_t batch,
                              int32_t atom_nf, int32_t residue_nf, float alpha_s, float sigma_s,
                              float alpha_ts, float sigma_ts, int32_t resample, int32_t remove_com);

int dsbdd_cond_step_keyed(void* stream, float* z_lig, float* xh_pocket, const float* eps_lig, float* scratch_lig,
                          const float* xh0_lig, const float* com_pocket0, const float* fixed, const int64_t* mask_lig,
                          const int64_t* mask_pocket, int64_t n_lig, int64_t n_pocket, int64_t batch, int32_t atom_nf,
                          int32_t residue_nf, float alpha_ts, float c_eps, float sigma, int32_t repaint, float alpha_s,
                          float sigma_s, float sigma_ts, int32_t remove_com, uint64_t seed, uint64_t draw_index,
                          int64_t sample_offset, const int64_t* sample_ids, float* t_word, float t_next);

int dsbdd_joint_repaint_update(void* stream, float* z_lig, float* z_pocket, float* scratch_lig,
                               float* scratch_pocket, const float* xh0_lig, const float* xh0_pocket,
                               const float* fixed_lig, const float* fixed_pocket, const float* noise_known_lig,
                               const float* noise_known_pocket, const float* noise_jump_lig,
                               const float* noise_jump_pocket, const int64_t* mask_lig,
                               const int64_t* mask_pocket, int64_t n_lig, int64_t n_pocket, int64_t batch,
                               int32_t atom_nf, int32_t residue_nf, float alpha_s, float sigma_s,
                               float alpha_ts, float sigma_ts, int32_t jump);

int dsbdd_randn_keyed(void* stream, float* out, const int64_t* mask, int64_t n_rows,
                      int32_t n_cols, int64_t batch, int64_t sample_offset,
                      const int64_t* sample_ids, uint64_t seed, uint64_t draw_index,
                      uint32_t stream_id);

int dsbdd_node_linear(void* stream, const float* A1, int32_t lda1, int32_t K1, const float* A2,
                      int32_t lda2, int32_t K2, const float* WT, int32_t ldw, const float* bias,
                      const float* R, int32_t ldr, float* C, int32_t ldc, int64_t M, int32_t N,
                      int32_t act);

int dsbdd_build_edges(void* stream, const float* x, const int64_t* mask_lig,
                      const int64_t* mask_pocket, int64_t n_lig, int64_t n_pocket, int64_t batch,
                      const dsbdd_config* cfg, int32_t* node_batch, int32_t* lig_off,
                      int32_t* poc_off, int32_t* deg, int32_t* row_ptr, int32_t* edge_row,
                      int32_t* edge_col, float* edge_d0, int64_t edge_capacity, int32_t* status);

typedef struct dsbdd_train_graph {
  const int32_t *erow, *ecol; const float* ed0;
  const int32_t *row_ptr, *deg;
  const int32_t* rev;
  const int32_t *node_batch, *lig_off, *poc_off;
  int64_t n_lig, n_nodes, n_edges, batch;
} dsbdd_train_graph;

typedef struct dsbdd_train_mlp {
  const float *P, *Q; int32_t ldpq;
  const float *wd, *wd0, *tab;
  const float *W2, *W2T, *b2;
  const float *head, *head_b;
} dsbdd_train_mlp;

typedef struct dsbdd_train_mlp_grad {
  float *dP, *dQ; int32_t ldo;
  float* d_vec;
  float* d_W2;
  float* gd0;
} dsbdd_train_mlp_grad;

size_t dsbdd_train_scratch_bytes(int32_t H, int64_t n_nodes, int64_t n_edges);
size_t dsbdd_train_wgrad_scratch_bytes(int64_t K, int64_t M, int64_t N);
size_t dsbdd_train_wgrad_plan_bytes(int64_t K, int64_t M, int64_t N);
int dsbdd_train_edge_rev(void* stream, const dsbdd_train_graph* g, int32_t* rev);
int dsbdd_train_sample_mean(void* stream, const float* x, const dsbdd_train_graph* g, float* mean);

int dsbdd_train_gcl_forward(void* stream, int32_t H, const dsbdd_train_graph* g, const dsbdd_train_mlp* m,
                            const float* x, float norm_factor, float* agg, void* scratch, size_t scratch_bytes);
int dsbdd_train_gcl_backward(void* stream, int32_t H, const dsbdd_train_graph* g, const dsbdd_train_mlp* m,
                             const float* x, float norm_factor, const float* d_agg,
                             const dsbdd_train_mlp_grad* out, float* d_x, void* scratch, size_t scratch_bytes);

int dsbdd_train_coord_forward(void* stream, int32_t H, const dsbdd_train_graph* g, const dsbdd_train_mlp* m,
                              int32_t n_mlp, const float* x, const float* mean, int64_t n_upd, float norm_constant,
                              float coords_range, int32_t use_tanh, float norm_factor, float* x_out, void* scratch,
                              size_t scratch_bytes);
int dsbdd_train_coord_backward(void* stream, int32_t H, const dsbdd_train_graph* g, const dsbdd_train_mlp* m,
                               int32_t n_mlp, const float* x, const float* mean, int64_t n_upd, int64_t e_upd,
                               float norm_constant, float coords_range, int32_t use_tanh, float norm_factor,
                               const float* d_xout, const dsbdd_train_mlp_grad* out, float* d_x, float* d_mean,
                               void* scratch, size_t scratch_bytes);

int dsbdd_train_radial_backward(void* stream, const dsbdd_train_graph* g, const float* x, const float* gd, float* d_x);

int dsbdd_train_wgrad(void* stream, const float* A, int32_t lda, const float* B, int32_t ldb, int64_t K, int32_t M,
                      int32_t N, float* C, void* scratch, size_t scratch_bytes);
int dsbdd_train_colsum(void* stream, const float* A, int32_t lda, int64_t M, int32_t N, float* out, void* scratch,
                       size_t scratch_bytes);

typedef struct dsbdd_train_net dsbdd_train_net;
int dsbdd_train_net_create(const dsbdd_config* cfg, dsbdd_train_net** out);
void dsbdd_train_net_destroy(dsbdd_train_net* net);
int dsbdd_train_net_param_count(const dsbdd_train_net* net);
size_t dsbdd_train_net_pack_bytes(const dsbdd_train_net* net);
size_t dsbdd_train_net_workspace_bytes(const dsbdd_train_net* net, const dsbdd_train_graph* g);
int dsbdd_train_net_forward(dsbdd_train_net* net, void* stream, const dsbdd_train_graph* g, const float* const* params,
                            void* pack, size_t pack_bytes, void* ws, size_t ws_bytes, const float* xh_lig,
                            const float* xh_pocket, const float* t, int64_t t_count, int32_t zero_nan, float* eps_lig,
                            float* eps_pocket, int32_t* status);
int dsbdd_train_net_backward(dsbdd_train_net* net, void* stream, const dsbdd_train_graph* g, const float* const* params,
                             float* const* grads, void* pack, size_t pack_bytes, void* ws, size_t ws_bytes,
                             int64_t e_upd, const float* d_eps_lig, const float* d_eps_pocket, float* d_xh_lig,
                             float* d_xh_pocket);
int dsbdd_train_net_forward_held(dsbdd_train_net* net, void* stream, const dsbdd_train_graph* g, const float* const* params,
                                 void* pack, size_t pack_bytes, void* ws, size_t ws_bytes, const float* xh_lig,
                                 const float* xh_pocket, const float* t, int64_t t_count, int32_t zero_nan, float* eps_lig,
                                 float* eps_pocket, int32_t* status, int32_t pack_is_current);
int dsbdd_train_net_backward_acc(dsbdd_train_net* net, void* stream, const dsbdd_train_graph* g, const float* const* params,
                                 float* const* grads, const uint8_t* accumulate, void* pack, size_t pack_bytes, void* ws,
                                 size_t ws_bytes, int64_t e_upd, const float* d_eps_lig, const float* d_eps_pocket,
                                 float* d_xh_lig, float* d_xh_pocket);

typedef struct {
  int32_t batch, n_lig, n_pocket, atom_nf, residue_nf, timesteps;
  int32_t remove_com;
  int32_t vnode_idx;
  float norm_value_x, norm_value_h, norm_bias_h;
  int32_t n1_tab, n2_tab;
} dsbdd_loss_cfg;
int dsbdd_edge_capacity(void* stream, const int64_t* lig_mask, int64_t n_lig, const int64_t* pocket_mask, int64_t n_pocket,
                        int64_t batch, int64_t* out);
int dsbdd_loss_rows(void);
int dsbdd_loss_out_rows(void);
int dsbdd_loss_cond_pre(void* stream, const dsbdd_loss_cfg* cfg, const float* lig_x, const float* lig_h, const int64_t* lig_mask,
                        const float* pocket_x, const float* pocket_h, const int64_t* pocket_mask, const float* eps,
                        const float* t_int, const float* gamma_table, const float* logpn_table, float* z_t, float* xh_pocket,
                        float* per_sample, float* lig_x_norm, float* lig_h_norm, float* pocket_x_norm, float* pocket_h_norm);
int dsbdd_loss_cond_post(void* stream, const dsbdd_loss_cfg* cfg, const float* net, const float* eps, const float* z_t,
                         const float* lig_h, const int64_t* lig_mask, const float* per_sample, float* xh_hat, float* out);
int dsbdd_loss_cond_post_backward(void* stream, const dsbdd_loss_cfg* cfg, const float* net, const float* eps, const float* lig_h,
                                  const int64_t* lig_mask, const float* per_sample, const float* g_err, const float* g_l0x,
                                  const float* g_hat, float* d_net);

int dsbdd_loss_joint_out_rows(void);
int dsbdd_loss_joint_pre(void* stream, const dsbdd_loss_cfg* cfg, const float* lig_x, const float* lig_h, const int64_t* lig_mask,
                         const float* pocket_x, const float* pocket_h, const int64_t* pocket_mask, const float* noise_lig,
                         const float* noise_pocket, const float* t_int, const float* gamma_table, const float* logpn_table,
                         float* eps_lig, float* eps_pocket, float* z_lig, float* z_pocket, float* per_sample, float* lig_x_norm,
                         float* lig_h_norm, float* pocket_x_norm, float* pocket_h_norm);
int dsbdd_loss_joint_post(void* stream, const dsbdd_loss_cfg* cfg, const float* net_lig, const float* net_pocket,
                          const float* eps_lig, const float* eps_pocket, const float* z_lig, const int64_t* lig_mask,
                          const int64_t* pocket_mask, const float* per_sample, float* xh_lig_hat, float* out);
int dsbdd_loss_joint_post_backward(void* stream, const dsbdd_loss_cfg* cfg, const float* net_lig, const float* net_pocket,
                                   const float* eps_lig, const float* eps_pocket, const int64_t* lig_mask,
                                   const int64_t* pocket_mask, const float* per_sample, const float* g_err_lig,
                                   const float* g_err_pocket, const float* g_l0x_lig, const float* g_l0x_pocket,
                                   const float* g_xh_lig_hat, float* d_net_lig, float* d_net_pocket);

typedef struct {
  double lr, beta1, beta2, eps, weight_decay;
  int32_t clip_grad;
} dsbdd_optim_cfg;
typedef struct dsbdd_optim dsbdd_optim;
int dsbdd_optim_create(const dsbdd_optim_cfg* cfg, int32_t n_tensors, const int64_t* numel, dsbdd_optim** out);
void dsbdd_optim_destroy(dsbdd_optim* o);
int64_t dsbdd_optim_state_elems(const dsbdd_optim* o);
int64_t dsbdd_optim_state_offset(const dsbdd_optim* o, int32_t tensor);
size_t dsbdd_optim_workspace_bytes(const dsbdd_optim* o);
int dsbdd_optim_bind(dsbdd_optim* o, void* stream, float* m, float* v, float* vmax, void* ws, size_t ws_bytes);
int dsbdd_optim_set_params(dsbdd_optim* o, void* stream, float* const* params);
int dsbdd_optim_step(dsbdd_optim* o, void* stream, const float* const* grads, const int32_t* steps, double lr);
int dsbdd_optim_state_read(dsbdd_optim* o, void* stream, double* out, int32_t capacity);
int dsbdd_optim_state_write(dsbdd_optim* o, void* stream, const double* items, int32_t n_items, double clips, double steps);

int dsbdd_lj_potential(void* stream, const float* xh, int32_t ld, int32_t n_types, const int64_t* mask, int64_t n, int64_t batch,
                       const double* sigma, double clamp, int32_t has_clamp, int32_t* type_scratch, float* u, float* dx);

int dsbdd_bond_orders(void* stream, const float* x, const int32_t* atom_type,
                      const int32_t* mol_off, int64_t batch, int32_t n_types,
                      const float* bonds1, const float* bonds2, const float* bonds3,
                      float margin1, float margin2, float margin3, int32_t n_max,
                      int8_t* order);

int dsbdd_pack_ligands(void* stream, const float* tmpl_x, const int32_t* tmpl_type,
                       const int32_t* tmpl_ptr, int32_t n_tmpl, int64_t tmpl_rows,
                       const int32_t* slot_tmpl, const int32_t* slot_size,
                       const int32_t* slot_off, int64_t batch, int64_t n_rows,
                       int32_t atom_nf, float* x, float* one_hot, int64_t* lig_fixed,
                       int64_t* mask, int64_t* size);

#ifdef __cplusplus
}
#endif
#endif
```

Before: 38.47.

## Add shell stage reusing ghost-pass edge messages for boundary-level pocket nodes

Adds a 'shell' path for cone stages where the radius equals g+1. The ghost edge pass now stores its per-edge messages to a buffer. Nodes at the shell level then recompute only the edges toward lower levels or ligand nodes, and take the remaining contributions from the stored messages in a new aggregation kernel. The level-building kernels gain shell degree counting, prefix sums and edge-list fills, and there is a new memory carve-out and debug read API. This is meant to skip redundant edge-MLP work for boundary nodes. In exchange it adds message-buffer writes, quadratic rank counting during the edge fill, and extra bookkeeping.

Result: faster. 40.56 (median of 6 runs) (+5.4%).

```diff
diff --git a/diffsbdd_amd/_lib.py b/diffsbdd_amd/_lib.py
--- a/diffsbdd_amd/_lib.py
+++ b/diffsbdd_amd/_lib.py
@@ -19,7 +19,7 @@
              "N1_WT", "N1_B", "N2_WT", "N2_B"]
 EQ_NAMES = ["C1_WT", "C_WD", "C_WD0", "C_TAB", "C_W2T", "C_B2",
             "X_WD", "X_WD0", "X_TAB", "X_W2T", "X_B2", "W3"]
-OPT_PRUNE, OPT_CONE, OPT_GRANULE16, OPT_EMU, OPT_SPLITK = 0, 1, 2, 3, 4
+OPT_PRUNE, OPT_CONE, OPT_GRANULE16, OPT_EMU, OPT_SPLITK, OPT_SHELL = 0, 1, 2, 3, 4, 5
 (BUF_EDGE_ROW, BUF_EDGE_COL, BUF_EDGE_D0, BUF_ROW_PTR, BUF_H, BUF_X, BUF_NODE_BATCH, BUF_DEG,
  BUF_LEVEL, BUF_LEVEL_LIST, BUF_LEVEL_COUNT, BUF_LEVEL_END, BUF_LROW_PTR, BUF_LEDGE_ROW, BUF_LEDGE_COL,
  BUF_LEDGE_D0, BUF_LEVEL_STATS) = range(17)
@@ -81,6 +81,7 @@
     "dsbdd_dynamics_forward": (C.c_int, [_P, _P, _P, _P, _P, _I64, _P, _P, _I64, _I64, _I64,
                                          _P, _P, _I64, _P, _P, _P]),
     "dsbdd_engine_buffer": (C.c_int, [_P, C.c_int, C.POINTER(_P)]),
+    "dsbdd_engine_shell_read": (C.c_int, [_P, C.c_int, C.c_int, _P, C.c_int64]),
     "dsbdd_engine_graph_stats": (C.c_int, [_P, C.POINTER(_I64), C.POINTER(_I64), C.POINTER(_I64)]),
     "dsbdd_engine_last_plan": (C.c_int, [_P, C.POINTER(C.c_int32), C.POINTER(C.c_int32), C.c_int32,
                                          C.POINTER(C.c_int32), C.POINTER(C.c_int32)]),
diff --git a/diffsbdd_amd/csrc/edge_mlp.h b/diffsbdd_amd/csrc/edge_mlp.h
--- a/diffsbdd_amd/csrc/edge_mlp.h
+++ b/diffsbdd_amd/csrc/edge_mlp.h
@@ -44,6 +44,8 @@
   float* agg_b; float* agg_head_b;
   float* z2_out;
   size_t z2_stride;
+  float* msg_out;
+  int msg_tiles;
 };
 
 enum { MODE_GCL = 0, MODE_COORD = 1 };
@@ -106,4 +108,76 @@
   }
 }
 
+
+__global__ __launch_bounds__(kThreads) void agg_complete_shell_kernel(
+    float* agg, const float* agg_head, const int* row_ptr, const int* deg, int n_rows, int H, int max_tile,
+    const int* lvl, int shell_level, int n_lig, int n_nodes, const float* head_s, const int* sh_ptr, const int* sh_deg,
+    const int* row_ptr_nat, const int* ecol_nat, int e_cap_nat, const int* twin_local, const int* row_ptr_ghost,
+    const float* msg, int msg_slots, float inv_norm) {
+  const int row = (blockIdx.x * kThreads + threadIdx.x) >> 6, lane = threadIdx.x & 63;
+  if (row >= n_rows) return;
+  const int L = (row >= n_lig && row < n_nodes) ? lvl[row] : 0;
+  if (L > shell_level) return;
+  if (L < shell_level) {
+    const int d = deg[row], s = row_ptr[row];
+    const int t0 = s >> 5, t1 = min((s + d - 1) >> 5, max_tile);
+    if (d > 0 && t1 == t0) return;
+    for (int k = 4 * lane; k < H; k += 256) {
+      float4 v = make_float4(0.f, 0.f, 0.f, 0.f);
+      if (d > 0) {
+        v = ld4(agg + (size_t)row * H + k);
+        for (int T = t0 + 1; T <= t1; ++T) {
+          const float4 h = ld4(agg_head + (size_t)T * H + k);
+          v.x += h.x; v.y += h.y; v.z += h.z; v.w += h.w;
+        }
+      }
+      *reinterpret_cast<float4*>(agg + (size_t)row * H + k) = v;
+    }
+    return;
+  }
+  const int d = sh_deg[row], s = sh_ptr[row];
+  const int t0 = s >> 5, t1 = min((s + d - 1) >> 5, max_tile);
+  const int dn = deg[row], sn = row_ptr_nat[row];
+  const int e_lo = max(sn, 0), e_hi = min(sn + dn, e_cap_nat);
+  const int base = row_ptr_ghost[twin_local[row - n_lig]] - sn;
+  const int k = min(4 * lane, H - 4);
+  const bool on = 4 * lane < H;
+  float4 v = make_float4(0.f, 0.f, 0.f, 0.f);
+  if (d > 0 && on) {
+    v = ld4(agg + (size_t)row * H + k);
+    for (int T = t0 + 1; T <= t1; ++T) {
+      const float4 h = ld4(head_s + (size_t)T * H + k);
+      v.x += h.x; v.y += h.y; v.z += h.z; v.w += h.w;
+    }
+  }
+  float4 c = make_float4(0.f, 0.f, 0.f, 0.f);
+  for (int e0 = e_lo; e0 < e_hi; e0 += 64) {
+    const int e = e0 + lane;
+    bool take = false;
+    if (e < e_hi) {
+      const int j = ecol_nat[e];
+      take = (unsigned)j < (unsigned)n_nodes && j >= n_lig && lvl[j] >= shell_level &&
+             (unsigned)(base + e) < (unsigned)msg_slots;
+    }
+    unsigned long long mk = __ballot(take);
+    while (mk) {
+      const float* src[4];
+      int n = 0;
+#pragma unroll
+      for (int u = 0; u < 4; ++u)
+        if (mk) {
+          src[n++] = msg + (size_t)(base + e0 + (__ffsll((long long)mk) - 1)) * H + k;
+          mk &= mk - 1;
+        }
+      float4 m[4];
+#pragma unroll
+      for (int u = 0; u < 4; ++u) if (u < n) m[u] = ld4(src[u]);
+#pragma unroll
+      for (int u = 0; u < 4; ++u) if (u < n) { c.x += m[u].x; c.y += m[u].y; c.z += m[u].z; c.w += m[u].w; }
+    }
+  }
+  v.x += c.x * inv_norm; v.y += c.y * inv_norm; v.z += c.z * inv_norm; v.w += c.w * inv_norm;
+  if (on) *reinterpret_cast<float4*>(agg + (size_t)row * H + k) = v;
 }
+
+}
diff --git a/diffsbdd_amd/csrc/edge_wave.h b/diffsbdd_amd/csrc/edge_wave.h
--- a/diffsbdd_amd/csrc/edge_wave.h
+++ b/diffsbdd_amd/csrc/edge_wave.h
@@ -90,10 +90,11 @@
   out[base + 1024] = (unsigned short)(__float_as_uint(lo) >> 16);
 }
 
-template <int H, int MODE, bool BPERM, int EMU = 0, bool STORE = false>
+template <int H, int MODE, bool BPERM, int EMU = 0, bool STORE = false, bool MSG = false>
 __global__ __launch_bounds__(kThreads, 2) void edge_wave_kernel(EdgeArgs p) {
   using L = WaveLayout<H, MODE, EMU>;
   static_assert(!STORE || (!BPERM && EMU == 0), "z2 is stored by the plain exact kernels only");
+  static_assert(!MSG || (MODE == MODE_GCL && EMU == 0 && !STORE), "messages are kept by the exact message kernel only");
   constexpr int BK = L::BK;
   constexpr int CT = H / 32;
   constexpr int NK = H / BK;
@@ -437,6 +438,24 @@
 #pragma unroll
           for (int r = 0; r < 16; ++r) acc[c][r] *= part[r];
       }
+      if constexpr (MSG) {
+        const int wt = __builtin_amdgcn_readfirstlane(my_wt);
+        if (!my_lb && wt < p.msg_tiles) {
+          const int e0 = wt * BMW;
+          float* mb = p.msg_out + (size_t)e0 * H + (4 * half) * H + j;
+          float* const mlo = mb + 128 * swb;
+          float* const mhi = mb - 128 * swb;
+#pragma unroll
+          for (int r = 0; r < 16; ++r) {
+            const int row = 8 * (r >> 2) + 4 * half + (r & 3);
+            if (e0 + row < E) {
+#pragma unroll
+              for (int c = 0; c < CT; ++c)
+                (c < 4 ? mlo : mhi)[(8 * (r >> 2) + (r & 3)) * H + 32 * c] = acc[c][r];
+            }
+          }
+        }
+      }
       static_assert(CT % 2 == 0, "column tiles are exchanged in pairs");
       f32x2 sum2[CT];
 #pragma unroll
diff --git a/diffsbdd_amd/csrc/engine.hip b/diffsbdd_amd/csrc/engine.hip
--- a/diffsbdd_amd/csrc/engine.hip
+++ b/diffsbdd_amd/csrc/engine.hip
@@ -113,6 +113,7 @@
   e->cap_lig = nl; e->cap_poc = np; e->cap_batch = B; e->cap_edges = E;
   e->cap_edgesL = 2 * E + 32 * kLevels * B;
   e->cap_tiles = e->cap_edgesL / 32 + 2;
+  e->cap_shell = E + 32 * B;
   e->cap_tiles16 = e->cap_edgesL / 16 + 2;
   e->lvl_stats_zeroed = false;
   e->frame = false;
@@ -200,6 +201,7 @@
     case DSBDD_OPT_EMU:
       if (value != 0 && value != 6 && value != 9) return fail(DSBDD_ERR_ARG, "DSBDD_OPT_EMU takes 0, 6 or 9");
       e->emu = value; break;
+    case DSBDD_OPT_SHELL: e->shell = value ? 1 : 0; break;
     default: return fail(DSBDD_ERR_ARG, "unknown option");
   }
   e->drop_graphs();
@@ -214,6 +216,7 @@
     case DSBDD_OPT_GRANULE16: return (int)e->granule16;
     case DSBDD_OPT_SPLITK: return (int)e->splitk;
     case DSBDD_OPT_EMU: return e->emu;
+    case DSBDD_OPT_SHELL: return e->shell;
   }
   return fail(DSBDD_ERR_ARG, "unknown option");
 }
@@ -268,6 +271,27 @@
   return DSBDD_OK;
 }
 
+int dsbdd_engine_shell_read(const dsbdd_engine* e, int which, int list, void* dst, int64_t count) {
+  if (!e || !dst || count < 0) return fail(DSBDD_ERR_ARG, "bad argument");
+  if (!e->shell_mem) return fail(DSBDD_ERR_STATE, "no shell stage has run on this engine");
+  const int64_t N = e->shell_key[0], SL = e->shell_key[2];
+  const void* src = nullptr;
+  int64_t have = 0, size = 4;
+  const bool lst = list >= 0 && list < kShellLists;
+  switch (which) {
+    case DSBDD_SHELL_STATS: src = e->sh_stats; have = 8; size = 8; break;
+    case DSBDD_SHELL_COUNT: src = e->sh_cnt; have = kShellLists; break;
+    case DSBDD_SHELL_ROW: if (lst) { src = e->sh_row + (size_t)list * SL; have = SL; } break;
+    case DSBDD_SHELL_COL: if (lst) { src = e->sh_col + (size_t)list * SL; have = SL; } break;
+    case DSBDD_SHELL_PTR: src = e->sh_ptr; have = N; break;
+    case DSBDD_SHELL_DEG: src = e->sh_deg; have = N; break;
+  }
+  if (!src) return fail(DSBDD_ERR_ARG, "unknown shell buffer");
+  if (count > have) return fail(DSBDD_ERR_CAPACITY, "shell read past the buffer");
+  HIP_TRY(hipDeviceSynchronize());
+  HIP_TRY(hipMemcpy(dst, src, (size_t)(count * size), hipMemcpyDeviceToHost));
+  return DSBDD_OK;
+}
 
 int dsbdd_dynamics_forward(dsbdd_engine* e, void* stream, const float* xh_lig, const float* xh_pocket,
                            const float* t, int64_t t_count, const int64_t* mask_lig,
diff --git a/diffsbdd_amd/csrc/engine_state.h b/diffsbdd_amd/csrc/engine_state.h
--- a/diffsbdd_amd/csrc/engine_state.h
+++ b/diffsbdd_amd/csrc/engine_state.h
@@ -147,6 +147,15 @@
   int prune = 1;
   int cone = 1;
   int64_t ghost_slots = 0;
+  int shell = 1;
+  int64_t cap_shell = 0;
+  char* shell_mem = nullptr;
+  int64_t shell_key[3] = {0, 0, 0};
+  int *sh_seg = nullptr, *sh_deg = nullptr, *sh_ptr = nullptr, *sh_row = nullptr, *sh_col = nullptr, *sh_cnt = nullptr;
+  float* sh_d0 = nullptr;
+  unsigned long long* sh_stats = nullptr;
+  float* msg_buf = nullptr;
+  int64_t msg_cap = 0;
   std::vector<int> plan_radius, plan_ghost;
   int plan_timed_level = kLevels - 1;
   bool frame = false;
@@ -206,6 +215,7 @@
     if (side_stream) (void)hipStreamDestroy(side_stream);
     if (ev_fork) (void)hipEventDestroy(ev_fork);
     if (ev_join) (void)hipEventDestroy(ev_join);
+    if (shell_mem) (void)hipFree(shell_mem);
   }
 };
 
diff --git a/diffsbdd_amd/csrc/forward.h b/diffsbdd_amd/csrc/forward.h
--- a/diffsbdd_amd/csrc/forward.h
+++ b/diffsbdd_amd/csrc/forward.h
@@ -90,6 +90,15 @@
       }
     return last;
   }
+  bool shell_stage(int g) const {
+    return cone && e->shell && g > 0 && g <= g_ghost_last && radius_of(g) == g + 1 && g + 1 < LV && g <= kShellLists &&
+           H == 256 && !e->emu && w2_enabled(e, W2_PERM);
+  }
+  int n_shell() const {
+    int n = 0;
+    for (int g = 1; g <= kShellLists && g < G_stages; ++g) if (shell_stage(g)) n = g;
+    return n;
+  }
   void rows_of(int r, bool ghost, NodeLinearArgs& a) const {
     if (!prune || (r >= LV && !ghost && !e->level_rows)) return;
     if (r > LV) r = LV;
@@ -212,6 +221,9 @@
                      n_ghost, (int)ghost_slots, (int)e->cap_edges, nullptr, nullptr};
         mean_in_levels = e->fold_scan && n_mlp == 2;
         if (mean_in_levels) { la.mean_x = e->x; la.mean_out = e->mean; }
+        la.n_shell = e->shell_mem ? n_shell() : 0;
+        la.sh_seg = e->sh_seg; la.sh_deg = e->sh_deg; la.sh_ptr = e->sh_ptr; la.sh_row = e->sh_row; la.sh_col = e->sh_col;
+        la.sh_d0 = e->sh_d0; la.sh_cap = (int)e->cap_shell; la.sh_cnt = e->sh_cnt; la.sh_stats = e->sh_stats;
         if (!e->lvl_stats_zeroed) {
           HIP_TRY(zero_async(e->lvl_stats, 128, s));
           e->lvl_stats_zeroed = true;
@@ -318,8 +330,26 @@
                          (const float*)e->aggB, (const float*)e->agg_headB, (const int*)e->row_ptr3,
                          (const int*)e->deg3, (const int*)e->twin, N, nlig, N, H, cone ? n_ghost : 0, (int)e->cap_tiles - 1);
       HIP_TRY(hipGetLastError());
+    } else if (shell_stage(g) && !g16 && !gsk) {
+      const int sl = g - 1;
+      if (!e->msg_buf || e->msg_cap < ghost_slots) return fail(DSBDD_ERR_STATE, "shell stage without a message buffer");
+      ea.e_count = e->lvl_end + (radius - 1);
+      ea.erow_b = e->sh_row + (size_t)sl * e->cap_shell; ea.ecol_b = e->sh_col + (size_t)sl * e->cap_shell;
+      ea.ed0_b = e->sh_d0 + (size_t)sl * e->cap_shell; ea.e_count_b = e->sh_cnt + sl; ea.e_cap_b = (int)e->cap_shell;
+      ea.wt_base_b = 0; ea.agg_b = e->agg; ea.agg_head_b = e->agg_headB;
+      ea.msg_out = e->msg_buf; ea.msg_tiles = (int)(ghost_slots / 32);
+      HIP_TRY(launch_edge(e, s, MODE_GCL, ea, L_bound() + 128));
+      const int n_rows = N + n_ghost;
+      hipLaunchKernelGGL(agg_complete_shell_kernel, dim3((n_rows + 3) / 4), dim3(kThreads), 0, s, e->agg,
+                         (const float*)e->agg_head, L_ptr, (const int*)e->deg, n_rows, H, (int)e->cap_tiles - 1,
+                         (const int*)e->lvl, radius, nlig, N, (const float*)e->agg_headB, (const int*)e->sh_ptr,
+                         (const int*)e->sh_deg, (const int*)e->row_ptr, (const int*)e->ecol, (int)e->cap_edges,
+                         (const int*)e->twin, (const int*)(e->row_ptrL + N), (const float*)e->msg_buf, (int)ghost_slots,
+                         1.0f / c.normalization_factor);
+      HIP_TRY(hipGetLastError());
     } else {
-      const bool timed = e->time_now && (all_rows || radius == e->plan_timed_level) && e->ev_used + 2 <= e->ev.size();
+      const bool timed = e->time_now && (all_rows || radius == e->plan_timed_level) && !shell_stage(g) &&
+                         e->ev_used + 2 <= e->ev.size();
       if (timed) HIP_TRY(hipEventRecord(e->ev[e->ev_used], s));
       HIP_TRY(launch_edge(e, s, MODE_GCL, ea, L_bound(), g16 && !gsk, gsk));
       if (timed) {
diff --git a/diffsbdd_amd/csrc/graph.h b/diffsbdd_amd/csrc/graph.h
--- a/diffsbdd_amd/csrc/graph.h
+++ b/diffsbdd_amd/csrc/graph.h
@@ -6,6 +6,7 @@
 constexpr int kTileCtrInts = 32;
 constexpr int kEdgeAlign = 32;
 constexpr int kLevels = 5;
+constexpr int kShellLists = 2;
 
 struct Cutoffs {
   int has_l, has_p, has_i;
@@ -270,16 +271,23 @@
   int node_off; int edge_off;
   int e_cap_nat;
   const float* mean_x; float* mean_out;
+  int n_shell;
+  int* sh_seg;
+  int* sh_deg; int* sh_ptr;
+  int* sh_row; int* sh_col; float* sh_d0; int sh_cap;
+  int* sh_cnt;
+  unsigned long long* sh_stats;
 };
 
 __global__ __launch_bounds__(kThreads) void levels_kernel(LevelArgs a) {
-  __shared__ int s_rows[kLevels], s_edges[kLevels];
+  __shared__ int s_rows[kLevels], s_edges[kLevels], s_shell[kShellLists];
   __shared__ float s_red[3][kThreads];
   if (a.mean_out) sample_mean_body(a.mean_x, a.lig_off, a.poc_off, a.n_lig, a.mean_out, s_red);
   const int b = blockIdx.x, t = threadIdx.x;
   const int p0 = a.n_lig + a.poc_off[b], p1 = a.n_lig + a.poc_off[b + 1];
   const int l0 = a.lig_off[b], l1 = a.lig_off[b + 1];
   if (t < kLevels) { s_rows[t] = 0; s_edges[t] = 0; }
+  if (t < kShellLists) s_shell[t] = 0;
   for (int k = 2; k < kLevels - 1; ++k) {
     __syncthreads();
     for (int i = p0 + t; i < p1; i += kThreads) {
@@ -298,6 +306,16 @@
     const int L = a.lvl[i];
     atomicAdd(&s_rows[L], 1);
     atomicAdd(&s_edges[L], a.deg[i]);
+    if (L >= 2 && L - 2 < a.n_shell) {
+      const int s = a.row_ptr_nat[i], d = a.deg[i];
+      int d2 = 0;
+      for (int e = max(s, 0); e < min(s + d, a.e_cap_nat); ++e) {
+        const int j = a.ecol_nat[e];
+        d2 += (j < a.n_lig || a.lvl[j] < L) ? 1 : 0;
+      }
+      a.sh_deg[i] = d2;
+      atomicAdd(&s_shell[L - 2], d2);
+    }
   }
   int le = 0;
   for (int i = l0 + t; i < l1; i += kThreads) le += a.deg[i];
@@ -307,6 +325,7 @@
     a.seg_rows[t * a.B + b] = t == 0 ? (l1 - l0) : s_rows[t];
     a.seg_edges[t * a.B + b] = s_edges[t];
   }
+  if (t < a.n_shell) a.sh_seg[t * a.B + b] = s_shell[t];
 }
 
 __global__ __launch_bounds__(1024) void level_scan_kernel(LevelArgs a, int n_nodes) {
@@ -403,6 +422,18 @@
   int n_run, e_run;
   if (fold_scan) level_bases(a, L * a.B + b, lane, n_run, e_run);
   else { n_run = a.node_base[L * a.B + b]; e_run = a.edge_base[L * a.B + b]; }
+  const int sl = L - 2;
+  const bool shell = sl >= 0 && sl < a.n_shell;
+  int s_run = 0;
+  if (shell) {
+    int sp = 0;
+    for (int k0 = 0; k0 < b; k0 += 64) {
+      const int kk = k0 + lane;
+      if (kk < b) sp += (a.sh_seg[sl * a.B + kk] + kEdgeAlign - 1) & ~(kEdgeAlign - 1);
+    }
+    s_run = wave_sum_i(sp);
+  }
+  const int s_begin = s_run;
   for (int i0 = p0; i0 < p1; i0 += 64) {
     const int i = i0 + lane;
     const bool mine = i < p1 && a.lvl[i] == L;
@@ -420,8 +451,36 @@
     }
     n_run += __popcll(m);
     e_run += __shfl(incl, 63);
+    if (shell) {
+      const int d2 = mine ? a.sh_deg[i] : 0;
+      int incl2 = d2;
+#pragma unroll
+      for (int o = 1; o < 64; o <<= 1) {
+        const int u = __shfl_up(incl2, o);
+        if (lane >= o) incl2 += u;
+      }
+      if (mine) a.sh_ptr[i] = s_run + incl2 - d2;
+      s_run += __shfl(incl2, 63);
+    }
   }
   pads(e_run);
+  if (shell) {
+    const int to = (s_run + kEdgeAlign - 1) & ~(kEdgeAlign - 1), pos = s_run + lane;
+    if (pos < to && pos < a.sh_cap) {
+      a.sh_row[(size_t)sl * a.sh_cap + pos] = -1; a.sh_col[(size_t)sl * a.sh_cap + pos] = 0;
+      a.sh_d0[(size_t)sl * a.sh_cap + pos] = 0.f;
+    }
+    if (lane == 0) {
+      if (b == a.B - 1) a.sh_cnt[sl] = to;
+      if (a.sh_stats) {
+        const int own = s_run - s_begin;
+        atomicAdd(&a.sh_stats[3 * sl], (unsigned long long)own);
+        atomicAdd(&a.sh_stats[3 * sl + 1], (unsigned long long)(to - s_begin));
+        atomicAdd(&a.sh_stats[3 * sl + 2], (unsigned long long)(a.seg_edges[L * a.B + b] - own));
+        if (b == 0 && sl == 0) atomicAdd(&a.sh_stats[3 * kShellLists], 1ull);
+      }
+    }
+  }
 }
 
 __global__ void ghost_setup_kernel(const int* erow3, const int* ecol3, const float* ed03, const int* row_ptr3,
@@ -476,6 +535,20 @@
     if (i < 0 || i >= n_nodes) continue;
     const int pos = a.row_ptr[i] + (e - a.row_ptr_nat[i]);
     if (pos >= 0 && pos < a.e_cap) { a.erow[pos] = i; a.ecol[pos] = a.ecol_nat[e]; a.ed0[pos] = a.ed0_nat[e]; }
+    const int L = i >= a.n_lig ? a.lvl[i] : 0;
+    if (L >= 2 && L - 2 < a.n_shell) {
+      const int j = a.ecol_nat[e];
+      if (j < a.n_lig || a.lvl[j] < L) {
+        int rank = 0;
+        for (int q = max(a.row_ptr_nat[i], 0); q < e; ++q) {
+          const int jq = a.ecol_nat[q];
+          rank += (jq < a.n_lig || a.lvl[jq] < L) ? 1 : 0;
+        }
+        const int ps = a.sh_ptr[i] + rank;
+        const size_t o = (size_t)(L - 2) * a.sh_cap;
+        if (ps >= 0 && ps < a.sh_cap) { a.sh_row[o + ps] = i; a.sh_col[o + ps] = j; a.sh_d0[o + ps] = a.ed0_nat[e]; }
+      }
+    }
   }
 }
 
diff --git a/diffsbdd_amd/csrc/graph_cache.h b/diffsbdd_amd/csrc/graph_cache.h
--- a/diffsbdd_amd/csrc/graph_cache.h
+++ b/diffsbdd_amd/csrc/graph_cache.h
@@ -13,6 +13,30 @@
   return DSBDD_OK;
 }
 
+static int shell_memory(dsbdd_engine* e, hipStream_t s) {
+  const int64_t N = e->cap_lig + e->cap_poc, B = e->cap_batch, SL = e->cap_shell;
+  if (e->shell_mem && e->shell_key[0] == N && e->shell_key[1] == B && e->shell_key[2] == SL && e->msg_cap >= e->ghost_slots)
+    return DSBDD_OK;
+  HIP_TRY(hipStreamSynchronize(s));
+  e->drop_graphs();
+  if (e->shell_mem) (void)hipFree(e->shell_mem);
+  e->shell_mem = nullptr; e->msg_cap = 0;
+  auto lay = [&](Carver c) {
+    auto ints = [&](size_t n) { return reinterpret_cast<int*>(c.bytes(n * 4)); };
+    e->sh_seg = ints((size_t)kShellLists * B); e->sh_deg = ints((size_t)N); e->sh_ptr = ints((size_t)N); e->sh_cnt = ints(4);
+    e->sh_stats = reinterpret_cast<unsigned long long*>(c.bytes(64));
+    e->sh_row = ints((size_t)kShellLists * SL); e->sh_col = ints((size_t)kShellLists * SL); e->sh_d0 = c.f((size_t)kShellLists * SL);
+    e->msg_buf = c.f1((size_t)e->ghost_slots * e->cfg.hidden_nf);
+    return c.off;
+  };
+  const size_t total = lay(Carver{nullptr});
+  HIP_TRY(hipMalloc(reinterpret_cast<void**>(&e->shell_mem), total));
+  HIP_TRY(hipMemset(e->shell_mem, 0, total));
+  lay(Carver{e->shell_mem});
+  e->shell_key[0] = N; e->shell_key[1] = B; e->shell_key[2] = SL; e->msg_cap = e->ghost_slots;
+  return DSBDD_OK;
+}
+
 static int frame_upkeep(dsbdd_engine* e, hipStream_t s, const ForwardArgs& a) {
   if (!frame_applies(e, a)) {
     e->ghost_dirty = true;
@@ -23,6 +47,7 @@
     int rc = ghost_setup(e, s);
     if (rc) return rc;
   }
+  if (Forward(e, s, a).n_shell() > 0) RC_TRY(shell_memory(e, s));
   if (!e->h0_pocket_valid) {
     Mlp2Problem enc = residue_encoder(e, a);
     if (mlp2_fits(enc)) {
diff --git a/diffsbdd_amd/csrc/launch.h b/diffsbdd_amd/csrc/launch.h
--- a/diffsbdd_amd/csrc/launch.h
+++ b/diffsbdd_amd/csrc/launch.h
@@ -107,6 +107,11 @@
   if (sk && a.mlp[0].W2SK) return launch_edge_sk(e, s, mode, a, edge_bound);
   if (g16) return launch_edge16(e, s, mode, a, edge_bound);
   const int grid = edge_wave_grid(mode, a, edge_bound, e->n_cu, e->edge_max_wg);
+  if (a.msg_out) {
+    if (mode != MODE_GCL || e->cfg.hidden_nf != 256 || e->emu || !a.mlp[0].W2TP || a.wt_base) return hipErrorInvalidValue;
+    hipLaunchKernelGGL((edge_wave_kernel<256, MODE_GCL, true, 0, false, true>), dim3(grid), dim3(kThreads), 0, s, a);
+    return hipGetLastError();
+  }
   const int emu = (e->emu && a.mlp[0].W2E && a.mlp[1].W2E) ? e->emu : 0;
   return with_hidden(e->cfg.hidden_nf, [&](auto h) {
     constexpr int H = decltype(h)::value;
diff --git a/include/diffsbdd_hip.h b/include/diffsbdd_hip.h
--- a/include/diffsbdd_hip.h
+++ b/include/diffsbdd_hip.h
@@ -107,7 +107,8 @@
 int dsbdd_engine_last_plan(const dsbdd_engine* e, int32_t* radius, int32_t* ghost, int32_t capacity,
                            int32_t* n_stages, int32_t* timed_level);
 
-enum { DSBDD_OPT_PRUNE = 0, DSBDD_OPT_CONE = 1, DSBDD_OPT_GRANULE16 = 2, DSBDD_OPT_EMU = 3, DSBDD_OPT_SPLITK = 4 };
+enum { DSBDD_OPT_PRUNE = 0, DSBDD_OPT_CONE = 1, DSBDD_OPT_GRANULE16 = 2, DSBDD_OPT_EMU = 3, DSBDD_OPT_SPLITK = 4,
+       DSBDD_OPT_SHELL = 5 };
 int dsbdd_engine_set_option(dsbdd_engine* e, int which, int value);
 int dsbdd_engine_get_option(const dsbdd_engine* e, int which);
 
@@ -119,6 +120,9 @@
   DSBDD_BUF_LEVEL_STATS
 };
 int dsbdd_engine_buffer(const dsbdd_engine* e, int which, void** ptr_out);
+
+enum { DSBDD_SHELL_STATS = 0, DSBDD_SHELL_COUNT, DSBDD_SHELL_ROW, DSBDD_SHELL_COL, DSBDD_SHELL_PTR, DSBDD_SHELL_DEG };
+int dsbdd_engine_shell_read(const dsbdd_engine* e, int which, int list, void* dst, int64_t count);
 
 int dsbdd_cond_reverse_update(void* stream, float* z_lig, float* xh_pocket, const float* eps_lig,
                               const float* noise, const int64_t* mask_lig,
```
